# pangenome/impg

Hardware: AMD Instinct MI355X
Metric: projected ranges/sec, 1M-PAF 100k-BED -x depth 3; CPU coitrees baseline (higher is better)
Workload: dtype int32

## Files before the change

### impg_amd/csrc/capi.cpp

```cpp
#include <sys/stat.h>
#include <unistd.h>

#include <atomic>
#include <cerrno>
#include <functional>
#include <thread>
#include <chrono>
#include <cmath>
#include <cstdlib>
#include <memory>
#include <new>

#include "engine.hpp"
#include "partition.hpp"

namespace impg {
thread_local std::string g_error;
void set_error(const std::string &msg) { g_error = msg; }
void render_paf(const impg_gpu_results &res, const impg_gpu_index &ix, const char *const *range_names,
                const impg_gpu_params_t &p, int32_t merge_distance, bool bedpe, std::vector<std::string> &parts);
void render_bed(const impg_gpu_results &res, const impg_gpu_index &ix, const char *const *range_names,
                const impg_gpu_params_t &p, int32_t merge_distance, std::vector<std::string> &parts);
char *join_parts(std::vector<std::string> &parts, size_t *len);
}

using namespace impg;


namespace impg {
static void engine_options(impg_gpu_index &ix, Engine *e) {
  e->pair_budget = ix.opt_pair_budget;
  e->chunk_ranges = ix.opt_chunk_ranges;
  e->locality_min = ix.opt_locality_min;
  e->free_slots_allowed = ix.opt_free_slots;
  e->regroup_pairs = ix.opt_regroup;
  e->fuse_allowed = ix.opt_fuse_final;
  e->filter_covered = ix.opt_filter_covered;
  e->walk_allowed = ix.opt_walk != 0 && !getenv("IMPG_NO_WALK");
  e->walk_bfs = ix.opt_walk == 2;
  e->walk_members = ix.opt_walk_members;
  e->seg_group = ix.opt_seg_group;
  e->seg_parts_force = ix.opt_seg_parts;
  e->seg_stats = ix.seg_stats;
  e->proj_stats = ix.proj_stats;
  e->update_stats = ix.opt_update_stats;
  e->upd_stats = ix.upd_stats;
  e->wide_emit = WideEmit{ix.opt_wide_cap, ix.opt_wide_bins, ix.opt_lookup_stats};
  e->lk_stats = ix.lk_stats;
}
static Engine *take_or_create(impg_gpu_index &ix) {
  Engine *e = nullptr;
  if (!ix.eng_free.empty()) { e = ix.eng_free.back(); ix.eng_free.pop_back(); }
  else if ((int)ix.engines.size() < ix.max_engines) {
    ix.engines.emplace_back(new Engine(ix.device));
    e = ix.engines.back().get();
  } else return nullptr;
  engine_options(ix, e);
  return e;
}
EngineLease::EngineLease(impg_gpu_index &ix_) : ix(ix_) {
  std::unique_lock<std::mutex> lk(ix.eng_m);
  while (!(e = take_or_create(ix))) ix.eng_cv.wait(lk);
}
Engine *try_lease_engine(impg_gpu_index &ix) {
  std::unique_lock<std::mutex> lk(ix.eng_m);
  return take_or_create(ix);
}
void return_engine(impg_gpu_index &ix, Engine *e) {
  e->remote = nullptr;
  e->masked = false;
  e->subset_on = false;
  std::lock_guard<std::mutex> lk(ix.eng_m);
  ix.eng_free.push_back(e);
  ix.eng_cv.notify_one();
}
EngineLease::~EngineLease() { return_engine(ix, e); }
}

namespace impg {

void require_device(int device) {
  int n = 0;
  hipError_t e = hipGetDeviceCount(&n);
  if (e != hipSuccess || n <= 0)
    throw Error{IMPG_E_HIP, "no HIP device available (libimpg_gpu has no CPU fallback)"};
  if (device < 0 || device >= n) throw Error{IMPG_E_INVALID, "device ordinal out of range"};
}

std::unique_ptr<impg_gpu_index> make_index(const impg_gpu_record_t *records, size_t n_records, const uint32_t *ops,
                                           size_t n_ops, const int64_t *seq_len, uint32_t n_seq, int bidirectional,
                                           int order_policy, int device, uint32_t shard, uint32_t n_shards,
                                           const HostSeqIndex *seq, const std::vector<uint64_t> *file_first,
                                           const uint32_t *owner) {
  if ((!records && n_records) || (!ops && n_ops) || (!seq_len && n_seq)) throw Error{IMPG_E_INVALID, "null input array"};
  require_device(device);
  auto ix = std::make_unique<impg_gpu_index>();
  ix->device = device;
  if (seq) ix->seq = *seq;
  if (file_first) {
    if (file_first->size() < 2 || file_first->front() != 0 || file_first->back() != n_records ||
        !std::is_sorted(file_first->begin(), file_first->end()))
      throw Error{IMPG_E_INVALID, "file boundaries must start at 0, end at n_records and be ascending"};
    ix->file_first = *file_first;
  }
  build_index(*ix, records, n_records, ops, n_ops, seq_len, n_seq, bidirectional != 0, order_policy, shard, n_shards, owner);
  { EngineLease warm(*ix); }
  return ix;
}

}

namespace impg {
void assemble_results(Engine &E, const impg_gpu_range_t *h_ranges, uint32_t n, const impg_gpu_params_t &p,
                      std::vector<std::unique_ptr<LevelBufs>> &levels, DevBuf &self_dev, impg_gpu_results &res, uint64_t max_rows,
                      hipEvent_t kernels_done, const std::function<void()> &on_kernels_done) {
  hipStream_t s = E.stream;
  res.ranges.assign(h_ranges, h_ranges + n);
  res.has_cigar = p.store_cigar != 0;
  RowPlan pl;
  plan_rows(E, n, p, levels, self_dev, false, pl);
  const size_t nr = pl.n_rows;
  if (nr > max_rows && n > 1) throw SplitBatch{};
  DevBuf rows, clen, coff, cpool;
  for (DevBuf *b : {&rows, &clen, &coff, &cpool}) b->pool = &E.level_pool;
  rows.reserve(std::max<size_t>(nr * sizeof(impg_gpu_interval_t), 256));
  if (res.has_cigar) clen.reserve(std::max<size_t>(nr * 4, 256));
  scatter_rows(E, levels, pl, RowSinks{rows.as<impg_gpu_interval_t>(), nullptr, nullptr, nullptr, nullptr,
                                       res.has_cigar ? clen.as<uint32_t>() : nullptr});
  if (max_rows != ~0ull && nr * sizeof(impg_gpu_interval_t) > res.intervals.cap)
    res.intervals.reserve(std::max<size_t>(nr, (size_t)std::min<uint64_t>(max_rows, nr + nr / 4)), true);
  res.intervals.resize(nr, true);
  std::vector<uint32_t> off32((size_t)n + 1);
  IMPG_HIP(hipMemcpyAsync(off32.data(), pl.offsets.p, ((size_t)n + 1) * 4, hipMemcpyDeviceToHost, s));
  if (kernels_done && !res.has_cigar) IMPG_HIP(hipEventRecord(kernels_done, s));
  if (nr) IMPG_HIP(hipMemcpyAsync(res.intervals.data(), rows.p, nr * sizeof(impg_gpu_interval_t), hipMemcpyDeviceToHost, s));
  if (res.has_cigar) {
    const uint64_t n_ops = build_row_cigars(E, levels, pl, clen, coff, cpool);
    res.cigar_off.resize(nr + 1, true);
    res.cigar_ops.resize(n_ops, true);
    if (kernels_done) IMPG_HIP(hipEventRecord(kernels_done, s));
    IMPG_HIP(hipMemcpyAsync(res.cigar_off.data(), coff.p, (nr + 1) * 8, hipMemcpyDeviceToHost, s));
    if (n_ops) IMPG_HIP(hipMemcpyAsync(res.cigar_ops.data(), cpool.p, n_ops * 4, hipMemcpyDeviceToHost, s));
  }
  if (kernels_done) { IMPG_HIP(hipEventSynchronize(kernels_done)); if (on_kernels_done) on_kernels_done(); }
  IMPG_HIP(hipStreamSynchronize(s));
  levels.clear();
  res.offsets.resize((size_t)n + 1);
  for (size_t q = 0; q <= n; q++) res.offsets[q] = off32[q];
  res.projected = E.last_projected;
}

const impg_gpu_range_t *upload_ranges(DevBuf &dst, const impg_gpu_range_t *ranges, size_t n, const hipStream_t *async_on) {
  dst.reserve(std::max<size_t>(n * sizeof(impg_gpu_range_t), 256));
  if (n && async_on) IMPG_HIP(hipMemcpyAsync(dst.p, ranges, n * sizeof(impg_gpu_range_t), hipMemcpyHostToDevice, *async_on));
  else if (n) IMPG_HIP(hipMemcpy(dst.p, ranges, n * sizeof(impg_gpu_range_t), hipMemcpyHostToDevice));
  return dst.as<impg_gpu_range_t>();
}

StatSinks::StatSinks(DevBuf &cnt, DevBuf &ck, bool want_count, bool want_cksum, size_t n, const hipStream_t *async_on) {
  auto zeroed = [&](DevBuf &b) {
    b.reserve(std::max<size_t>(n * 8, 256));
    if (async_on) IMPG_HIP(hipMemsetAsync(b.p, 0, n * 8, *async_on));
    else IMPG_HIP(hipMemset(b.p, 0, std::max<size_t>(n * 8, 8)));
    return b.as<unsigned long long>();
  };
  if (want_count) count = zeroed(cnt);
  if (want_cksum) cksum = zeroed(ck);
}
void StatSinks::home(uint64_t *per_range_count, uint64_t *per_range_checksum, size_t n) const {
  if (per_range_count && n) IMPG_HIP(hipMemcpy(per_range_count, count, n * 8, hipMemcpyDeviceToHost));
  if (per_range_checksum && n) IMPG_HIP(hipMemcpy(per_range_checksum, cksum, n * 8, hipMemcpyDeviceToHost));
}

bool run_chunk_rows(const impg_gpu_index &ix, Engine &E, const impg_gpu_range_t *d_ranges, const impg_gpu_range_t *h_ranges, size_t b,
                    size_t e, const impg_gpu_params_t &p, impg_gpu_results &part, std::mutex *gpu_turn, uint64_t max_rows,
                    hipEvent_t kernels_done, const std::function<void()> &on_kernels_done) {
  std::vector<std::unique_ptr<LevelBufs>> levels;
  DevBuf self_dev;
  self_dev.pool = &E.level_pool;
  const auto c0 = std::chrono::steady_clock::now();
  {
    const auto turn = take_turn(gpu_turn);
    RunSpec rs(d_ranges + b, (uint32_t)(e - b), p);
    rs.keep = &levels;
    rs.self_out = &self_dev;
    E.run(ix, rs);
  }
  const auto c1 = std::chrono::steady_clock::now();
  if (e == b) return false;
  assemble_results(E, h_ranges + b, (uint32_t)(e - b), p, levels, self_dev, part, max_rows, kernels_done, on_kernels_done);
  part.approximate = ix.tp_mode;
  part.run_s = std::chrono::duration<double>(c1 - c0).count();
  part.assemble_s = std::chrono::duration<double>(std::chrono::steady_clock::now() - c1).count();
  return true;
}

bool run_chunk_bed(const impg_gpu_index &ix, Engine &E, const impg_gpu_range_t *d_ranges, const impg_gpu_range_t *h_ranges,
                   const char *const *range_names, size_t b, size_t e, const impg_gpu_params_t &p, int32_t merge_distance,
                   const std::function<void(const char *, size_t)> &sink, double *seconds3, std::mutex *gpu_turn) {
  std::vector<std::unique_ptr<LevelBufs>> levels;
  DevBuf self_dev, rows;
// ... 276 lines not shown
      struct stat st;
      if (stat(p.c_str(), &st) == 0) bytes += (uint64_t)st.st_size * ((p.size() > 3 && p.compare(p.size() - 3, 3, ".gz") == 0) ? 6 : 1);
    }
    size_t free_b = 0, total_b = 0;
    IMPG_HIP(hipSetDevice(device));
    IMPG_HIP(hipMemGetInfo(&free_b, &total_b));
    if (bytes * 8 > free_b) raw = false;
  }
  parse_paf_files(ps, pp, raw);
  lap(raw ? "parse PAF (lines, fields)" : "parse PAF", t0);
  std::vector<int64_t> lens = pp.seq.lens;
  if (raw) {
    const auto t1 = std::chrono::steady_clock::now();
    DevBuf d_ops;
    const uint64_t n_ops = tokenize_on_device(pp, device, d_ops);
    lap("CIGAR text -> ops (device)", t1);
    auto ix = std::make_unique<impg_gpu_index>();
    ix->device = device;
    ix->seq = pp.seq;
    if (pp.file_first.size() < 2 || pp.file_first.front() != 0 || pp.file_first.back() != pp.records.size())
      throw Error{IMPG_E_INVALID, "internal: bad file boundaries"};
    ix->file_first = pp.file_first;
    if (order_policy != IMPG_ORDER_COITREES && order_policy != IMPG_ORDER_SORTED) throw Error{IMPG_E_INVALID, "bad order policy"};
    if (build_index_device(*ix, pp.records.data(), pp.records.size(), nullptr, n_ops, lens.data(), (uint32_t)lens.size(), bidirectional != 0,
                           order_policy, 0, 1, nullptr, d_ops.as<uint32_t>())) {
      { EngineLease warm(*ix); }
      *out = ix.release();
      return IMPG_OK;
    }
    pp.ops.resize(n_ops);
    if (n_ops) IMPG_HIP(hipMemcpy(pp.ops.data(), d_ops.p, n_ops * 4, hipMemcpyDeviceToHost));
  }
  *out = make_index(pp.records.data(), pp.records.size(), pp.ops.data(), pp.ops.size(), lens.data(), (uint32_t)lens.size(),
                    bidirectional, order_policy, device, 0, 1, &pp.seq, &pp.file_first, nullptr).release();
  return IMPG_OK;
  IMPG_CATCH
}

int impg_gpu_parse_subsequence(const char *seq_name, char *base_out, size_t base_cap, int32_t *start_offset) {
  IMPG_TRY
  if (!seq_name || !base_out || !start_offset) throw Error{IMPG_E_INVALID, "null argument"};
  size_t base_len = 0;
  uint32_t off = 0;
  const std::string name(seq_name);
  if (!subsequence_origin(name, base_len, off)) return 0;
  if (base_len + 1 > base_cap) throw Error{IMPG_E_INVALID, "name buffer too small"};
  memcpy(base_out, name.data(), base_len);
  base_out[base_len] = '\0';
  *start_offset = (int32_t)off;
  return 1;
  IMPG_CATCH
}

int impg_gpu_subset_keep(const char *list_text, size_t len, const char *const *names, size_t n, uint8_t *keep_out,
                         size_t *n_entries) {
  IMPG_TRY
  if ((!list_text && len) || (n && (!names || !keep_out))) throw Error{IMPG_E_INVALID, "null argument"};
  const size_t e = subset_select(list_text, len, names, n, keep_out);
  if (n_entries) *n_entries = e;
  return IMPG_OK;
  IMPG_CATCH
}

int impg_gpu_index_save(const impg_gpu_index_t *ix, const char *path) {
  IMPG_TRY
  if (!ix || !path) throw Error{IMPG_E_INVALID, "null argument"};
  if (ix->shard || ix->cluster) save_sharded(*ix, path);
  else save_index(*ix, path);
  return IMPG_OK;
  IMPG_CATCH
}

int impg_gpu_index_load(const char *path, int device, impg_gpu_index_t **out) {
  IMPG_TRY
  if (!path || !out) throw Error{IMPG_E_INVALID, "null argument"};
  require_device(device);
  auto ix = std::make_unique<impg_gpu_index>();
  ix->device = device;
  load_index(*ix, path);
  { EngineLease warm(*ix); }
  *out = ix.release();
  return IMPG_OK;
  IMPG_CATCH
}

void impg_gpu_index_destroy(impg_gpu_index_t *ix) { delete ix; }

uint32_t impg_gpu_num_seqs(const impg_gpu_index_t *ix) { return (uint32_t)ix->seq.lens.size(); }
const char *impg_gpu_seq_name(const impg_gpu_index_t *ix, uint32_t id) {
  return id < ix->seq.names.size() ? ix->seq.names[id].c_str() : nullptr;
}
int64_t impg_gpu_seq_len(const impg_gpu_index_t *ix, uint32_t id) { return id < ix->seq.lens.size() ? ix->seq.lens[id] : -1; }
int64_t impg_gpu_seq_id(const impg_gpu_index_t *ix, const char *name) {
  auto it = ix->seq.name_to_id.find(name);
  return it == ix->seq.name_to_id.end() ? -1 : (int64_t)it->second;
}
size_t impg_gpu_num_targets(const impg_gpu_index_t *ix) { return ix->n_targets; }
size_t impg_gpu_target_ids(const impg_gpu_index_t *ix, uint32_t *out, size_t cap) {
  size_t k = 0;
  for (uint32_t s = 0; s + 1 < ix->h_tgt_off.size(); s++)
    if (ix->h_tgt_off[s + 1] != ix->h_tgt_off[s]) {
      if (out && k < cap) out[k] = s;
      k++;
    }
  return k;
}
size_t impg_gpu_num_entries(const impg_gpu_index_t *ix) { return ix->n_entries; }
size_t impg_gpu_num_records(const impg_gpu_index_t *ix) { return ix->n_records; }
size_t impg_gpu_device_bytes(const impg_gpu_index_t *ix) { return ix->device_bytes; }
int impg_gpu_index_approximate(const impg_gpu_index_t *ix) {
  return ix->tp_mode ? 1 : 0;
}

uint64_t impg_gpu_host_pool_trim(uint64_t keep_bytes) { return (uint64_t)impg::pinned_trim((size_t)keep_bytes); }

int impg_gpu_set_option(impg_gpu_index_t *ix, const char *key, int64_t value) {
  IMPG_TRY
  if (!ix || !key) throw Error{IMPG_E_INVALID, "null argument"};
  std::string k(key);
  if (k == "pair_budget") {
    if (value < 1024 || value >= 0xFFFFFFF0ll) throw Error{IMPG_E_INVALID, "pair_budget out of range"};
    ix->opt_pair_budget = (uint64_t)value;
  } else if (k == "chunk_ranges") {
    if (value < 0 || value >= (1ll << 31)) throw Error{IMPG_E_INVALID, "chunk_ranges out of range"};
    ix->opt_chunk_ranges = (uint32_t)value;
  } else if (k == "locality_min") {
    if (value < 0 || value >= (1ll << 31)) throw Error{IMPG_E_INVALID, "locality_min out of range"};
    ix->opt_locality_min = (uint32_t)value;
  } else if (k == "device_rows_pool_bytes") {
    if (value < 0) throw Error{IMPG_E_INVALID, "device_rows_pool_bytes must not be negative"};
    ix->opt_device_rows_pool = (uint64_t)value;
  } else if (k == "fuse_final_level") {
    ix->opt_fuse_final = value != 0;
  } else if (k == "regroup_entries") {
    ix->opt_regroup = value != 0;
  } else if (k == "walk_kernel") {
    if (value < 0 || value > 2) throw Error{IMPG_E_INVALID, "walk_kernel is 0, 1 or 2"};
    ix->opt_walk = (int)value;
  } else if (k == "segment_groups") {
    ix->opt_seg_group = value != 0;
  } else if (k == "segment_parts") {
    if (value < 0 || value > 4096) throw Error{IMPG_E_INVALID, "segment_parts is 0 .. 4096"};
    ix->opt_seg_parts = (uint32_t)value;
  } else if (k == "walk_members") {
    if (value < 0 || value > (long long)WALK_MAX_MEMBERS) throw Error{IMPG_E_INVALID, "walk_members is 0 .. 64"};
    ix->opt_walk_members = (uint32_t)value;
  } else if (k == "filter_covered") {
    if (value < 0 || value > 2) throw Error{IMPG_E_INVALID, "filter_covered is 0, 1 or 2"};
    ix->opt_filter_covered = (int)value;
  } else if (k == "update_stats") {
    ix->opt_update_stats = value != 0;
  } else if (k == "lookup_stats") {
    ix->opt_lookup_stats = value != 0;
  } else if (k == "wide_emit_cap") {
    if (value < 64 || value > (long long)WIDE_CAP) throw Error{IMPG_E_INVALID, "wide_emit_cap is 64 .. 4096"};
    ix->opt_wide_cap = (uint32_t)value;
  } else if (k == "wide_emit_bins") {
    if (value < 2 || value > (long long)WIDE_BINS) throw Error{IMPG_E_INVALID, "wide_emit_bins is 2 .. 1024"};
    ix->opt_wide_bins = (uint32_t)value;
  } else if (k == "approximate_cigar") {
    if (value != 0 && value != 1) throw Error{IMPG_E_INVALID, "approximate_cigar is 0 or 1"};
    ix->opt_approx_cigar = value != 0;
  } else if (k == "free_slot_order") {
    ix->opt_free_slots = value != 0;
  } else if (k == "debug_fail_owner" || k == "debug_fail_home") {
    if (value < 0 || value > 0xFFFFFFFFll) throw Error{IMPG_E_INVALID, "debug_fail_* out of range"};
    (k == "debug_fail_owner" ? ix->opt_debug_fail_owner : ix->opt_debug_fail_home) = (uint32_t)value;
  } else if (k == "lane_schedule") {
    if (value < 0) throw Error{IMPG_E_INVALID, "lane_schedule out of range"};
    ix->opt_lane_schedule = (uint64_t)value;
  } else if (k == "prewarm_result_bytes") {
    if (value < 0) throw Error{IMPG_E_INVALID, "prewarm_result_bytes is a size"};
    if (value) {
      size_t cap = 0;
      void *b = pinned_take((size_t)value, cap);
      pinned_give(b, cap);
    }
  } else if (k == "prewarm_walk") {
    if (value < 0 || value > 2) throw Error{IMPG_E_INVALID, "prewarm_walk is 0, 1 or 2"};
    if (value && !ix->shard && !ix->cluster) {
      IMPG_HIP(hipSetDevice(ix->device));
      EngineLease lease(*ix);
      lease->reserve_walk_slabs(*ix, value >= 2);
    }
  } else throw Error{IMPG_E_INVALID, "unknown option " + k};
  return IMPG_OK;
  IMPG_CATCH
}

int impg_gpu_get_counter(const impg_gpu_index_t *ix, const char *key, int64_t *value_out) {
  IMPG_TRY
  if (!ix || !key || !value_out) throw Error{IMPG_E_INVALID, "null argument"};
  const std::string k = key;
  if (k == "walk_launches") *value_out = (int64_t)ix->walk_launches.load();
  else if (k == "walk_fallbacks") *value_out = (int64_t)ix->walk_fallbacks.load();
  else if (k == "walk_members") *value_out = (int64_t)ix->walk_last_members.load();
  else if (k == "small_batches") *value_out = (int64_t)ix->small_batches.load();
  else if (k == "segment_sliced_levels") *value_out = (int64_t)ix->seg_stats[0].load();
  else if (k == "segment_retries") *value_out = (int64_t)ix->seg_stats[1].load();
  else if (k == "segment_library_levels") *value_out = (int64_t)ix->seg_stats[2].load();
  else if (k == "project_lane_levels") *value_out = (int64_t)ix->proj_stats[PROJ_ARM_LANE].load();
  else if (k == "project_staged_levels") *value_out = (int64_t)ix->proj_stats[PROJ_ARM_STAGED].load();
  else if (k == "project_staged_rows_levels") *value_out = (int64_t)ix->proj_stats[PROJ_ARM_STAGED_ROWS].load();
  else if (k == "project_entries_slots_levels") *value_out = (int64_t)ix->proj_stats[PROJ_ARM_ENTRIES_SLOTS].load();
  else if (k == "project_entries_qs_levels") *value_out = (int64_t)ix->proj_stats[PROJ_ARM_ENTRIES_QS].load();
  else if (k == "project_entries_rows_levels") *value_out = (int64_t)ix->proj_stats[PROJ_ARM_ENTRIES_ROWS].load();
  else if (k == "project_entries_ident_levels") *value_out = (int64_t)ix->proj_stats[PROJ_ARM_ENTRIES_IDENT].load();
  else if (k == "project_tp_levels") *value_out = (int64_t)ix->proj_stats[PROJ_ARM_TP].load();
  else if (k == "update_lane_groups") *value_out = (int64_t)ix->upd_stats[UPD_LANE].load();
  else if (k == "update_mid_groups") *value_out = (int64_t)ix->upd_stats[UPD_MID].load();
  else if (k == "update_wave_tiny_groups") *value_out = (int64_t)ix->upd_stats[UPD_WAVE_TINY].load();
  else if (k == "update_wave_small_groups") *value_out = (int64_t)ix->upd_stats[UPD_WAVE_SMALL].load();
  else if (k == "update_wave_large_groups") *value_out = (int64_t)ix->upd_stats[UPD_WAVE_LARGE].load();
  else if (k == "update_inplace_groups") *value_out = (int64_t)ix->upd_stats[UPD_INPLACE].load();
  else if (k == "update_tiled_sort_groups") *value_out = (int64_t)ix->upd_stats[UPD_TILED_SORT].load();
  else if (k == "update_lane_spill_groups") *value_out = (int64_t)ix->upd_stats[UPD_LANE_SPILL].load();
  else if (k == "lookup_wide_windows") *value_out = (int64_t)ix->lk_stats[LK_WIDE].load();
  else if (k == "lookup_wide_single") *value_out = (int64_t)ix->lk_stats[LK_SINGLE].load();
  else if (k == "lookup_wide_grouped") *value_out = (int64_t)ix->lk_stats[LK_GROUPED].load();
  else if (k == "lookup_wide_group_passes") *value_out = (int64_t)ix->lk_stats[LK_GROUP_PASSES].load();
  else if (k == "lookup_wide_overflow") *value_out = (int64_t)ix->lk_stats[LK_OVERFLOW].load();
  else throw Error{IMPG_E_INVALID, "unknown counter " + k};
  return IMPG_OK;
  IMPG_CATCH
}

int impg_gpu_visit_rank(uint32_t n, int order_policy, uint32_t *rank_out) {
  IMPG_TRY
  if (!rank_out && n) throw Error{IMPG_E_INVALID, "null argument"};
  if (order_policy == IMPG_ORDER_COITREES) coitrees_visit_rank(n, rank_out);
  else if (order_policy == IMPG_ORDER_SORTED) for (uint32_t i = 0; i < n; i++) rank_out[i] = i;
  else throw Error{IMPG_E_INVALID, "bad order policy"};
  return IMPG_OK;
  IMPG_CATCH
}

}
namespace impg {
void apply_mask(Engine &E, const impg_gpu_index &ix, const impg_gpu_mask_t *m, const impg_gpu_params_t &p) {
  if (!m) return;
  if (!p.transitive) throw Error{IMPG_E_INVALID, "masked_regions belong to the transitive queries"};
  const uint32_t n_seq = ix.view.n_seq;
  if (m->n_seqs && (!m->seq_id || !m->sequence_length || !m->range_off)) throw Error{IMPG_E_INVALID, "null mask array"};
  const uint64_t total = m->n_seqs ? m->range_off[m->n_seqs] : 0;
  if (total >= 0xFFFFFFF0ull) throw Error{IMPG_E_UNSUPPORTED, "mask exceeds 2^32 ranges"};
  if (total && !m->ranges) throw Error{IMPG_E_INVALID, "null mask array"};
  std::vector<uint32_t> off(n_seq + 1, 0);
  std::vector<int32_t> init_len(n_seq, 0), touch_len(n_seq, 0);
  bool has_empty = false;
  if (p.multi_impg) for (uint32_t s = 0; s < n_seq; s++) touch_len[s] = (int32_t)std::min<int64_t>(std::max<int64_t>(ix.seq.lens[s], 0), INT32_MAX);
  for (uint32_t i = 0; i < m->n_seqs; i++) {
    const uint32_t s = m->seq_id[i];
    if (s >= n_seq) throw Error{IMPG_E_INVALID, "mask names an unknown sequence id"};
    if (i && s <= m->seq_id[i - 1]) throw Error{IMPG_E_INVALID, "mask sequence ids must be strictly ascending"};
    if (m->range_off[i + 1] < m->range_off[i]) throw Error{IMPG_E_INVALID, "mask offsets must not decrease"};
    off[s + 1] = (uint32_t)(m->range_off[i + 1] - m->range_off[i]);
    init_len[s] = touch_len[s] = m->sequence_length[i];
    for (uint64_t k = m->range_off[i]; k < m->range_off[i + 1]; k++) {
      const int32_t a = m->ranges[2 * k], b = m->ranges[2 * k + 1];
      if (a > b || (k > m->range_off[i] && a <= m->ranges[2 * k - 1]))
        throw Error{IMPG_E_INVALID, "mask ranges must be sorted, disjoint and non-touching"};
      has_empty = has_empty || a == b;
    }
  }
  for (uint32_t s = 0; s < n_seq; s++) off[s + 1] += off[s];
  E.mask_off.reserve((size_t)(n_seq + 1) * 4);
  E.mask_ranges.reserve(std::max<size_t>(total * 8, 256));
  E.mask_init_len.reserve(std::max<size_t>((size_t)n_seq * 4, 256));
  E.mask_touch_len.reserve(std::max<size_t>((size_t)n_seq * 4, 256));
  IMPG_HIP(hipMemcpy(E.mask_off.p, off.data(), (size_t)(n_seq + 1) * 4, hipMemcpyHostToDevice));
  ix.mask_table_uploads++;
  if (total) { IMPG_HIP(hipMemcpy(E.mask_ranges.p, m->ranges, total * 8, hipMemcpyHostToDevice)); ix.mask_table_uploads++; }
  if (n_seq) {
    IMPG_HIP(hipMemcpy(E.mask_init_len.p, init_len.data(), (size_t)n_seq * 4, hipMemcpyHostToDevice));
    IMPG_HIP(hipMemcpy(E.mask_touch_len.p, touch_len.data(), (size_t)n_seq * 4, hipMemcpyHostToDevice));
    ix.mask_table_uploads += 2;
  }
  E.masked = true;
  E.mask_has_empty = has_empty;
  E.mask_ranges_total = total;
  E.mask_lists = m->n_seqs;
}
void apply_subset(Engine &E, const impg_gpu_index &ix, const uint8_t *subset_keep) {
  if (!subset_keep) return;
  const size_t ns = ix.view.n_seq;
  E.subset_keep.reserve(std::max<size_t>(ns, 256));
  if (ns) IMPG_HIP(hipMemcpy(E.subset_keep.p, subset_keep, ns, hipMemcpyHostToDevice));
  E.subset_on = true;
}
}
extern "C" {

int impg_gpu_query_batch(impg_gpu_index_t *ix, const impg_gpu_range_t *ranges, size_t n, const impg_gpu_params_t *params,
                         impg_gpu_results_t **out) {
  return impg_gpu_query_batch_masked(ix, ranges, n, params, nullptr, out);
}

int impg_gpu_query_batch_masked(impg_gpu_index_t *ix, const impg_gpu_range_t *ranges, size_t n,
                                const impg_gpu_params_t *params, const impg_gpu_mask_t *mask, impg_gpu_results_t **out) {
  return impg_gpu_query_batch_filtered(ix, ranges, n, params, mask, nullptr, out);
}

int impg_gpu_query_batch_filtered(impg_gpu_index_t *ix, const impg_gpu_range_t *ranges, size_t n,
                                  const impg_gpu_params_t *params, const impg_gpu_mask_t *mask, const uint8_t *subset_keep,
                                  impg_gpu_results_t **out) {
  IMPG_TRY
  if (!ix || !params || !out || (!ranges && n)) throw Error{IMPG_E_INVALID, "null argument"};
  check_ranges(ranges, n);
  Engine::check_params(*params);
  if (ix->shard || ix->cluster) return sharded_query_batch(*ix, ranges, n, *params, mask, subset_keep, out);
  IMPG_HIP(hipSetDevice(ix->device));
  EngineLease lease(*ix);
  Engine &E = *lease;
  apply_mask(E, *ix, mask, *params);
  apply_subset(E, *ix, subset_keep);
  auto res = std::make_unique<impg_gpu_results>();
  res->approximate = ix->tp_mode;
  if (n && n <= Engine::SMALL_RANGES && !params->transitive) {
    const auto c0 = std::chrono::steady_clock::now();
    if (E.run_small(*ix, ranges, (uint32_t)n, *params, *res)) {
      res->run_s = std::chrono::duration<double>(std::chrono::steady_clock::now() - c0).count();
      *out = res.release();
      return IMPG_OK;
    }
  }
  const impg_gpu_range_t *d_ranges = upload_ranges(E.ranges_dev, ranges, n, &E.stream);
  if (n < (1ull << 31) && E.walk_applicable(*ix, (uint32_t)n, *params)) {
    const auto c0 = std::chrono::steady_clock::now();
    if (walk_query(*ix, E, (uint32_t)n, *params, *res)) {
      res->run_s = std::chrono::duration<double>(std::chrono::steady_clock::now() - c0).count();
      res->ranges.assign(ranges, ranges + n);
      *out = res.release();
      return IMPG_OK;
    }
    res = std::make_unique<impg_gpu_results>();
  }
  res->offsets.assign(1, 0);
  for_chunks(E, n, [&](size_t b, size_t e) {
    impg_gpu_results part;
    run_chunk_rows(*ix, E, d_ranges, ranges, b, e, *params, part);
    ix->result_rows_to_host += part.intervals.size();
    append_results(*res, part);
  });
  res->ranges.assign(ranges, ranges + n);
  *out = res.release();
  return IMPG_OK;
  IMPG_CATCH
}

int impg_gpu_query(impg_gpu_index_t *ix, uint32_t target_id, int32_t start, int32_t end, const impg_gpu_params_t *params,
                   impg_gpu_results_t **out) {
  impg_gpu_range_t r{target_id, start, end};
  return impg_gpu_query_batch(ix, &r, 1, params, out);
}

int impg_gpu_query_batch_stream(impg_gpu_index_t *ix, const impg_gpu_range_t *ranges, size_t n, const impg_gpu_params_t *params,
                                const impg_gpu_mask_t *mask, const uint8_t *subset_keep, size_t chunk_ranges, size_t max_block_bytes,
                                impg_gpu_stream_cb cb, void *ctx, uint64_t *projected_out) {
  IMPG_TRY
  if (!ix) throw Error{IMPG_E_INVALID, "null argument"};
  const bool collective = ix->shard && !ix->cluster;
  std::exception_ptr refused;
  try {
    if (!params || !cb || (!ranges && n)) throw Error{IMPG_E_INVALID, "null argument"};
    check_ranges(ranges, n);
    Engine::check_params(*params);
  } catch (...) {
    if (!collective) throw;
    refused = std::current_exception();
// ... 538 lines not shown
```

### impg_amd/csrc/engine.cpp

```cpp
#include <cmath>
#include <cstdio>
#include <cstdlib>
#include <memory>

#include "engine.hpp"

namespace impg {

namespace {
inline unsigned bits_for(uint64_t n) {
  unsigned b = 0;
  while ((1ull << b) < n) b++;
  return b;
}
}

Engine::Engine(int device) {
  IMPG_HIP(hipSetDevice(device));
  IMPG_HIP(hipStreamCreateWithFlags(&stream, hipStreamNonBlocking));
  for (DevBuf *b : {&ord_offsets, &ord_rows}) b->pool = &level_pool;
  win_se.pool = &level_pool;
  counters.reserve(128);
  acc_slots.reserve(COUNT_BYTES);
  act_slots.reserve(COUNT_BYTES);
// ... 255 lines not shown
  for (uint32_t k = 0; k < COUNT_SLOTS; k++) t += h_slots[k * COUNT_STRIDE];
  return t;
}

uint64_t Engine::scan(const uint32_t *in, uint32_t *out, uint32_t n) {
  if (n == 0) return 0;
  scan_tmp.reserve(scan_scratch_bytes(n));
  launch_exclusive_scan(in, out, n, scan_tmp.as<unsigned long long>(), counters.as<unsigned long long>() + 3, stream);
  IMPG_HIP(hipMemcpyAsync(h_counters, counters.as<uint64_t>() + 3, 24, hipMemcpyDeviceToHost, stream));
  IMPG_HIP(hipStreamSynchronize(stream));
  if (h_counters[2]) throw Error{IMPG_E_INVALID, "query range must satisfy start < end"};
  return h_counters[0];
}

void Engine::scan2(const uint32_t *in_a, uint32_t *out_a, const uint32_t *in_b, uint32_t *out_b, uint32_t n, uint64_t &total_a, uint64_t &total_b,
                   const uint32_t *d_extra, uint32_t *h_extra, uint32_t n_extra) {
  total_a = total_b = 0;
  if (n) {
    scan_tmp.reserve(scan_scratch_bytes(n));
    scan_tmp2.reserve(scan_scratch_bytes(n));
    launch_exclusive_scan(in_a, out_a, n, scan_tmp.as<unsigned long long>(), counters.as<unsigned long long>() + 14, stream);
    launch_exclusive_scan(in_b, out_b, n, scan_tmp2.as<unsigned long long>(), counters.as<unsigned long long>() + 15, stream);
    IMPG_HIP(hipMemcpyAsync(h_counters, counters.as<uint64_t>() + 14, 16, hipMemcpyDeviceToHost, stream));
  }
  if (n_extra) IMPG_HIP(hipMemcpyAsync(h_counters + 2, d_extra, (size_t)n_extra * 4, hipMemcpyDeviceToHost, stream));
  IMPG_HIP(hipStreamSynchronize(stream));
  if (n) { total_a = h_counters[0]; total_b = h_counters[1]; }
  if (n_extra) memcpy(h_extra, h_counters + 2, (size_t)n_extra * 4);
}

static HitArrays hit_arrays(LevelBufs &L, uint32_t n_pairs) {
  size_t b = std::max<size_t>((size_t)n_pairs * 4, 256);
  L.qid.reserve(L.qs_interleaved ? 2 * b : b); L.coords.reserve(4 * b);
  return HitArrays{L.qid.as<uint32_t>(), L.coords.as<int4>()};
}

const uint32_t *Engine::lookup_order(const DeviceIndexView &v, const FrontierRec *fr, uint32_t n_fr, const RecordBlocks *blocks) {
  if (!locality_min || (n_fr < locality_min && !blocks)) { keys_for = nullptr; return nullptr; }
  const size_t nb = (size_t)n_fr * 4;
  lo_key.reserve(nb); lo_key2.reserve(nb); lo_idx.reserve(nb); lo_perm.reserve(nb);
  unsigned hi_bit = std::max(1u, bits_for((uint32_t)std::min<size_t>(v.n_entries, 0xFFFFFFFFull)));
  unsigned block_shift = 0;
  if (blocks) {
    const unsigned bb = std::max(1u, bits_for(blocks->n_blocks));
    if (hi_bit + bb > 32) return nullptr;
    block_shift = hi_bit;
    hi_bit += bb;
  }
  if (!blocks && keys_for && keys_for == (const void *)fr && keys_n == n_fr) {
  } else
    launch_order_keys(v, fr, n_fr, lo_key.as<uint32_t>(), lo_idx.as<uint32_t>(), stream, blocks ? blocks->d_bounds : nullptr,
                      blocks ? blocks->n_blocks : 0u, block_shift);
  keys_for = nullptr;
  static const bool lib_sort = getenv("IMPG_LIB_SORT") && atoi(getenv("IMPG_LIB_SORT")) != 0;
  if (lib_sort) {
    const size_t tb = sort_u32_scratch_bytes(n_fr);
    sort_tmp.reserve(tb);
    launch_sort_u32(sort_tmp.p, tb, lo_key.as<uint32_t>(), lo_key2.as<uint32_t>(), lo_idx.as<uint32_t>(), lo_perm.as<uint32_t>(), n_fr,
                    stream, 0, hi_bit);
  } else {
    sort_tmp.reserve(order_sort_scratch_bytes(n_fr));
    launch_order_sort(lo_key.as<uint32_t>(), lo_key2.as<uint32_t>(), lo_perm.as<uint32_t>(), lo_idx.as<uint32_t>(), n_fr, hi_bit, sort_tmp.p, stream);
  }
  return lo_perm.as<uint32_t>();
}
void Engine::projection_offsets(const uint32_t *d_perm, uint32_t n_fr, const uint32_t *d_cnt, uint64_t P, const uint32_t *&d_offp,
                                ProjList &pl) {
  d_offp = nullptr;
  pl = ProjList{nullptr, nullptr, nullptr};
  if (!d_perm || !P) return;
  const size_t nb = (size_t)n_fr * 4;
  lo_cnt.reserve(nb); lo_off.reserve(nb); lo_offp.reserve(nb);
  const size_t pb = std::max<size_t>(P * 4, 256);
  slot_of.reserve(pb); proj_range.reserve(pb); proj_entry.reserve(pb);
  launch_gather_u32(d_cnt, d_perm, n_fr, lo_cnt.as<uint32_t>(), stream);
  scan(lo_cnt.as<uint32_t>(), lo_off.as<uint32_t>(), n_fr);
  launch_scatter_u32(lo_off.as<uint32_t>(), d_perm, n_fr, lo_offp.as<uint32_t>(), stream);
  pl = ProjList{slot_of.as<uint32_t>(), proj_range.as<uint32_t>(), proj_entry.as<uint32_t>()};
  d_offp = lo_offp.as<uint32_t>();
}

void Engine::count_wide_paths(const DeviceIndexView &v, uint32_t n) {
  if (!(wide_emit.count_reach && lk_stats) || !n || !emit_by_lanes(v)) return;
  uint32_t w[LK_WORDS];
  IMPG_HIP(hipMemcpyAsync(w, wide_n.p, sizeof w, hipMemcpyDeviceToHost, stream));
  IMPG_HIP(hipStreamSynchronize(stream));
  const uint32_t *reach = w + LK_REACH_BASE;
  lk_stats[LK_WIDE] += w[0];
  lk_stats[LK_OVERFLOW] += w[1];
  lk_stats[LK_SINGLE] += reach[LK_REACH_SINGLE];
  lk_stats[LK_GROUPED] += reach[LK_REACH_GROUPED];
  lk_stats[LK_GROUP_PASSES] += reach[LK_REACH_PASSES];
}

uint64_t Engine::expand(const DeviceIndexView &v, const FrontierRec *fr, uint32_t n_fr, bool transitive, LevelBufs &L,
                        impg_gpu_stats_t *st, bool raw, const RecordBlocks *blocks) {
  hipEvent_t e0 = event(), e1 = event(), e2 = event();
  IMPG_HIP(hipEventRecord(e0, stream));
  cnt.reserve((size_t)n_fr * 4);
  win.reserve((size_t)n_fr * 16);
  pair_off.reserve((size_t)n_fr * 4);
  if (multi) transitive = false;
  wide_n.reserve(256);
  wide_list.reserve(std::max<size_t>((size_t)n_fr * 8, 256));
  const uint32_t *d_perm = lookup_order(v, fr, n_fr, blocks);
  const bool by_place = free_slot_order && (!raw || blocks) && !multi && !store_cigar && d_perm;
  last_by_place = by_place;
  last_range_places = false;
  L.qs_interleaved = false;
  L.placed = false;
  expand_n_fr = n_fr;
  bool fused = by_place && fuse_final && emit_by_lanes(v) && !v.tp_mode;
  const bool lk = wide_emit.count_reach && lk_stats;
  const WideEmit we{wide_emit.cap, wide_emit.bins, lk};
  if (by_place) win_se.reserve(std::max<size_t>((size_t)n_fr * sizeof(FrontierRec), 256));
  const bool ordered = run_modes.ordered_rows && !raw;
  if (ordered) { L.slot_ref.reserve(std::max<size_t>((size_t)n_fr * 4, 256)); ord_cnt.reserve(std::max<size_t>((size_t)n_fr * 4, 256)); }
  launch_lookup_count(v, fr, n_fr, transitive, d_perm, cnt.as<uint32_t>(), win.as<uint4>(), wide_n.as<uint32_t>(),
                      wide_list.as<uint32_t>(), stream, by_place, by_place ? win_se.as<FrontierRec>() : nullptr,
                      ordered && by_place ? ord_cnt.as<uint32_t>() : nullptr, lk);
  uint64_t P = scan(cnt.as<uint32_t>(), pair_off.as<uint32_t>(), n_fr);
  if (P > pair_budget || P >= 0xFFFFFFF0ull) {
    if (split_ok) throw SplitBatch{};
    if (P >= 0xFFFFFFF0ull) throw Error{IMPG_E_UNSUPPORTED, "more than 2^32 candidate pairs for a single range"};
  }
  L.n_pairs = (uint32_t)P;
  L.n_frontier = n_fr;
  bool direct = false;
  if (ordered) {
    ordered_level(fr, n_fr, L, !by_place, P);
    direct = fused && !store_cigar && !(min_identity == min_identity) && project_entry_major(v, P, min_identity);
    if (!direct) fused = false;
  }
  L.pair_range.reserve(std::max<size_t>(P * 4, 256));
  pair_entry.reserve(std::max<size_t>(P * 4, 256));
  ProjList pl{nullptr, nullptr, nullptr};
  WindowLists wlists{nullptr, nullptr, nullptr, nullptr, nullptr, 0u, nullptr, 0u, 0u};
  if (fused) {
    const bool staged = project_is_staged(v, P, !store_cigar && !(min_identity == min_identity));
    tile_first.reserve(((size_t)(P + 255) / 256 + 1) * 4);
    if (!staged) launch_tile_first(cnt.as<uint32_t>(), pair_off.as<uint32_t>(), n_fr, tile_first.as<uint32_t>(), stream);
    launch_lookup_emit(v, fr, n_fr, transitive, pair_off.as<uint32_t>(), win.as<uint4>(), L.pair_range.as<uint32_t>(),
                       pair_entry.as<uint32_t>(), d_perm, nullptr, pl, wide_n.as<uint32_t>(), wide_list.as<uint32_t>(), stream, true, true, we);
    wlists = WindowLists{tile_first.as<uint32_t>(), pair_off.as<uint32_t>(), win.as<uint4>(), win_se.as<FrontierRec>(), d_perm, n_fr,
                         fuse_need_ranges && !direct ? L.pair_range.as<uint32_t>() : nullptr, 1u, fuse_range_places ? 1u : 0u};
    last_range_places = fuse_need_ranges && fuse_range_places && !direct;
    if (project_entry_major(v, P, min_identity) && !store_cigar) {
      const uint32_t cap = project_entry_slice_cap(P), nb = project_entry_blocks(n_fr);
      ent_work.reserve(((size_t)cap + 1) * 4);
      ent_alloc.reserve(std::max<size_t>((size_t)nb * 4, 256));
      IMPG_HIP(hipMemsetAsync(ent_work.p, 0, 4, stream));
      IMPG_HIP(hipMemsetAsync(ent_alloc.p, 0, (size_t)nb * 4, stream));
      wlists.slice_work = ent_work.as<uint32_t>(); wlists.slice_alloc = ent_alloc.as<uint32_t>(); wlists.slice_cap = cap;
    }
    L.qs_interleaved = last_range_places && project_entry_major(v, P, min_identity) && !(min_identity == min_identity) && !store_cigar && !getenv("IMPG_NO_QS");
    if (L.qs_interleaved) { wlists.masks |= 4u; wlists.range_out = nullptr; }
    if (direct) {
      ordered_offsets();
      ord_dest.reserve(std::max<size_t>((size_t)n_fr * 4, 256));
      ord_vpos.reserve(std::max<size_t>(P + 256, 256));
      const bool by_visit = ordered_rows_by_visit();
      const OrdDestArgs od{win_se.as<FrontierRec>(), d_perm, L.slot_ref.as<uint32_t>(), ord_offsets.as<uint32_t>(), L.lvbase.as<uint32_t>(), ord_dest.as<uint32_t>()};
      launch_emit_vpos(v, n_fr, pair_off.as<uint32_t>(), win.as<uint4>(), ord_vpos.as<uint8_t>(), stream, by_visit, &od);
      wlists.ord = OrderedOut{ord_rows.as<impg_gpu_interval_t>(), ord_dest.as<uint32_t>(), ord_vpos.as<uint8_t>(), ord_min_len, by_visit ? 1u : 0u};
      L.placed = true;
    }
  } else if (by_place) {
    launch_lookup_emit(v, fr, n_fr, transitive, pair_off.as<uint32_t>(), win.as<uint4>(), L.pair_range.as<uint32_t>(),
                       pair_entry.as<uint32_t>(), d_perm, nullptr, pl, wide_n.as<uint32_t>(), wide_list.as<uint32_t>(), stream, true, false, we);
    wlists = WindowLists{nullptr, pair_off.as<uint32_t>(), win.as<uint4>(), win_se.as<FrontierRec>(), d_perm, n_fr, nullptr, 0u, 0u};
  } else {
    const uint32_t *d_offp = nullptr;
    projection_offsets(d_perm, n_fr, cnt.as<uint32_t>(), P, d_offp, pl);
    const bool entry_slots = store_cigar || multi || !pl.slot;
    launch_lookup_emit(v, fr, n_fr, transitive, pair_off.as<uint32_t>(), win.as<uint4>(), L.pair_range.as<uint32_t>(),
                       entry_slots ? pair_entry.as<uint32_t>() : nullptr, pl.slot ? d_perm : nullptr, d_offp, pl,
                       wide_n.as<uint32_t>(), wide_list.as<uint32_t>(), stream, false, false, we);
  }
  count_wide_paths(v, n_fr);
  IMPG_HIP(hipEventRecord(e1, stream));
  HitArrays h = direct ? HitArrays{nullptr, nullptr} : hit_arrays(L, L.n_pairs);
  SliceArrays sl{nullptr, nullptr, nullptr, nullptr};
  if (store_cigar) {
    size_t b = std::max<size_t>((size_t)L.n_pairs * 4, 256);
    L.sl_a.reserve(b); L.sl_n.reserve(b); L.sl_off.reserve(b); L.sl_rem.reserve(b);
    sl = SliceArrays{L.sl_a.as<uint32_t>(), L.sl_n.as<uint32_t>(), L.sl_off.as<int32_t>(), L.sl_rem.as<int32_t>()};
  }
  count_arm(launch_project(v, fr, L.pair_range.as<uint32_t>(), pair_entry.as<uint32_t>(), L.n_pairs, transitive, h,
                           acc_slots.as<unsigned long long>(), (uint32_t *)(counters.as<uint64_t>() + 2), min_identity,
                           store_cigar ? &sl : nullptr, pl, stream, nullptr, regroup_pairs, by_place ? &wlists : nullptr));
  if (!raw && !direct) {
    post_expand(fr, n_fr, L, pair_off.as<uint32_t>(), pair_entry.as<uint32_t>(), v.mrank, sl);
    h = HitArrays{L.qid.as<uint32_t>(), L.coords.as<int4>()};
    if (store_cigar) sl = SliceArrays{L.sl_a.as<uint32_t>(), L.sl_n.as<uint32_t>(), L.sl_off.as<int32_t>(), L.sl_rem.as<int32_t>()};
  }
  IMPG_HIP(hipEventRecord(e2, stream));
  if (store_cigar && L.n_pairs) {
    cnt.reserve((size_t)L.n_pairs * 4);
    L.slice_pos.reserve((size_t)L.n_pairs * 4);
    launch_slice_counts(h, sl, L.n_pairs, cnt.as<uint32_t>(), stream);
    L.slice_total = scan(cnt.as<uint32_t>(), L.slice_pos.as<uint32_t>(), L.n_pairs);
    if (L.slice_total >= 0xFFFFFFF0ull) {
      if (split_ok) throw SplitBatch{};
      throw Error{IMPG_E_UNSUPPORTED, "CIGAR slices of one level exceed 2^32 ops"};
    }
    L.slice_pool.reserve(std::max<size_t>(L.slice_total * 4, 256));
    launch_slice_write(v, pair_entry.as<uint32_t>(), h, sl, L.n_pairs, L.slice_pos.as<uint32_t>(), L.slice_pool.as<uint32_t>(), stream);
  } else {
    L.slice_total = 0;
  }
  timed.push_back({e0, e1, 0});
  timed.push_back({e1, e2, 1});
  if (st) {
    st->pairs += P;
    st->frontier_ranges += n_fr;
    if (P) st->project_launches += 1;
  }
  return P;
}

void Engine::post_expand(const FrontierRec *fr, uint32_t n_fr, LevelBufs &L, const uint32_t *d_pair_off, uint32_t *tie_idx,
                         const uint32_t *tie_rank, SliceArrays sl) {
  HitArrays h{L.qid.as<uint32_t>(), L.coords.as<int4>()};
  if (subset_on)
    launch_subset_filter(fr, L.pair_range.as<uint32_t>(), L.n_pairs, h.qid, subset_keep.as<uint8_t>(), cur_ranges, stream);
  if (multi && L.n_pairs) {
    const size_t b = std::max<size_t>((size_t)L.n_pairs * 4, 256);
    m_dest.reserve(b); m_qid.reserve(b); m_coords.reserve(4 * b); m_pe.reserve(b);
    launch_sort5(fr, n_fr, d_pair_off, L.n_pairs, h, tie_idx, tie_rank, m_dest.as<uint32_t>(), stream);
    HitArrays h2{m_qid.as<uint32_t>(), m_coords.as<int4>()};
    SliceArrays sl2{nullptr, nullptr, nullptr, nullptr};
    if (sl.a) {
      m_sa.reserve(b); m_sn.reserve(b); m_so.reserve(b); m_sr.reserve(b);
      sl2 = SliceArrays{m_sa.as<uint32_t>(), m_sn.as<uint32_t>(), m_so.as<int32_t>(), m_sr.as<int32_t>()};
    }
    launch_permute_slots(m_dest.as<uint32_t>(), L.n_pairs, h, h2, tie_idx, m_pe.as<uint32_t>(), sl, sl2, stream);
    L.qid.swap(m_qid); L.coords.swap(m_coords);
    if (tie_idx == pair_entry.as<uint32_t>()) pair_entry.swap(m_pe);
    if (sl.a) { L.sl_a.swap(m_sa); L.sl_n.swap(m_sn); L.sl_off.swap(m_so); L.sl_rem.swap(m_sr); }
  }
}

void Engine::ordered_level(const FrontierRec *fr, uint32_t n_fr, LevelBufs &L, bool counts_by_range, uint64_t P) {
  const uint64_t total = scan(counts_by_range ? cnt.as<uint32_t>() : ord_cnt.as<uint32_t>(), L.slot_ref.as<uint32_t>(), n_fr);
  if (total != P) throw Error{IMPG_E_INVALID, "internal: a level's slot counts disagree between its two orders"};
  L.lvbase.reserve(std::max<size_t>((size_t)ord_n * 4, 256));
  launch_ord_level_bases(fr, n_fr, L.slot_ref.as<uint32_t>(), (uint32_t)P, ord_n, ord_acc.as<uint32_t>(), L.lvbase.as<uint32_t>(), stream);
}
void Engine::ordered_offsets() {
  if (ord_offsets_done) return;
  ord_offsets.reserve(((size_t)ord_n + 1) * 4);
  ord_total = scan(ord_acc.as<uint32_t>(), ord_offsets.as<uint32_t>(), ord_n + 1u);
  if (ord_total >= 0xFFFFFFF0ull) { if (split_ok) throw SplitBatch{}; throw Error{IMPG_E_UNSUPPORTED, "more than 2^32 result rows in one chunk: use smaller chunks (chunk_ranges)"}; }
  ord_rows.reserve(std::max<size_t>(ord_total * sizeof(impg_gpu_interval_t), 256));
  ord_offsets_done = true;
}
void Engine::ordered_finish(std::vector<std::unique_ptr<LevelBufs>> &levels) {
  hipEvent_t p0 = event(), p1 = event();
  IMPG_HIP(hipEventRecord(p0, stream));
  ordered_offsets();
  launch_ord_self_rows(ord_self, ord_ranges, ord_n, ord_offsets.as<uint32_t>(), ord_rows.as<impg_gpu_interval_t>(), stream);
  for (auto &Lp : levels) {
    LevelBufs &L = *Lp;
    if (L.placed || !L.n_pairs) continue;
    L.run_start.reserve(std::max<size_t>((size_t)L.n_frontier * 4, 256));
    launch_ord_run_heads(L.pair_range.as<uint32_t>(), L.n_pairs, L.run_start.as<uint32_t>(), stream);
    HitArrays h{L.qid.as<uint32_t>(), L.coords.as<int4>()};
    launch_ord_level_rows(L.frontier.as<FrontierRec>(), L.pair_range.as<uint32_t>(), L.n_pairs, h, L.run_start.as<uint32_t>(), L.slot_ref.as<uint32_t>(),
                          ord_offsets.as<uint32_t>(), L.lvbase.as<uint32_t>(), ord_min_len, ord_rows.as<impg_gpu_interval_t>(), stream);
    L.placed = true;
  }
  IMPG_HIP(hipEventRecord(p1, stream));
  IMPG_HIP(hipStreamSynchronize(stream));
  float ms = 0;
  IMPG_HIP(hipEventElapsedTime(&ms, p0, p1));
  ms_place = ms;
}

HopResult Engine::hop(const DeviceIndexView &v, const FrontierRec *fr, uint32_t n_fr, bool transitive, LevelBufs &L,
                      impg_gpu_stats_t *st, bool need_hits, bool need_rows, bool alive) {
  if (remote) return remote->hop(*this, v, fr, n_fr, transitive, L, st, need_hits, need_rows, alive);
  if (!alive) { L.n_pairs = 0; return HopResult{0, true}; }
  if (!n_fr) { L.n_pairs = 0; return HopResult{0, false}; }
  return HopResult{expand(v, fr, n_fr, transitive, L, st), false};
}

uint32_t Engine::update(const DeviceIndexView &v, const FrontierRec *fr, LevelBufs &L, uint32_t n_queries,
                        const impg_gpu_params_t &p, DevBuf &next_frontier) {
  hipEvent_t e0 = event(), e1 = event();
  IMPG_HIP(hipEventRecord(e0, stream));
  const uint32_t P = L.n_pairs;
  uint32_t n_next = 0;
  HitArrays h{L.qid.as<uint32_t>(), L.coords.as<int4>()};
  if (P) {
    const uint32_t P_slots = P;
    const bool want_flags = filter_covered != 0;
    svals.reserve((size_t)P * 8);
    uint32_t seg_active = 0, seg_groups = 0;
    uint32_t *sg_run_start = nullptr, *sg_run_end = nullptr, *sg_q = nullptr, *sg_bins = nullptr;
    uint32_t seg_parts = seg_group && !want_flags && !multi && seg_group_fits(v.n_seq) && L.n_frontier > 0 ? seg_group_parts(P, n_queries, v.n_seq) : 0u;
    if (seg_parts_force && seg_parts) {
      seg_parts = std::max(1u, std::min(seg_parts_force, 4096u));
      while (seg_parts > 1 && ((uint64_t)n_queries * seg_parts >= (1ull << 31) || seg_group_bins_bytes(n_queries, v.n_seq, seg_parts) > (1ull << 30))) seg_parts >>= 1;
    }
    bool by_segments = seg_parts != 0;
    if (by_segments) {
      const uint32_t n_fr = L.n_frontier;
      seg_run.reserve(std::max<size_t>((size_t)n_fr * 8, 256));
      seg_q.reserve(std::max<size_t>((size_t)n_queries * 24 + 256, 512));
      sg_run_start = seg_run.as<uint32_t>(); sg_run_end = sg_run_start + n_fr;
      sg_q = seg_q.as<uint32_t>();
      uint32_t *qfirst = sg_q, *qlast = qfirst + n_queries, *qact = qlast + n_queries, *qdst = qact + n_queries, *qgrp = qdst + n_queries,
               *gdst = qgrp + n_queries, *unsorted = gdst + n_queries;
      const bool own_offsets = !remote && !store_cigar && L.n_frontier == expand_n_fr;
      launch_seg_bounds(fr, n_fr, n_queries, L.pair_range.as<uint32_t>(), P, sg_run_start, sg_run_end, qfirst, qlast, unsorted, stream,
                        own_offsets && last_by_place ? lo_perm.as<uint32_t>() : nullptr, own_offsets ? pair_off.as<uint32_t>() : nullptr,
                        own_offsets ? cnt.as<uint32_t>() : nullptr);
      for (int attempt = 0; attempt < 2 && by_segments; attempt++) {
        const size_t bb = seg_group_bins_bytes(n_queries, v.n_seq, seg_parts);
        sg_bins = nullptr;
        if (seg_parts > 1 || bb <= (512ull << 20)) { seg_bins.reserve(std::max<size_t>(bb, 256)); sg_bins = seg_bins.as<uint32_t>(); }
        if (seg_parts > 1) seg_tot.reserve(std::max<size_t>(seg_group_bins_bytes(n_queries, v.n_seq, 1), 256));
        launch_seg_group(true, fr, qfirst, qlast, sg_run_start, sg_run_end, h, n_queries, v.n_seq, qact, qdst, qgrp, gdst, nullptr, nullptr, nullptr, sg_bins,
                         stream, seg_parts, seg_tot.as<uint32_t>());
        uint64_t ta = 0, tg = 0;
        uint32_t bad[2] = {0, 0};
        scan2(qact, qdst, qgrp, gdst, n_queries, ta, tg, unsorted, bad, 2);
        seg_active = (uint32_t)ta;
        if (bad[0]) by_segments = false;
        else if (bad[1]) {
          const uint32_t again = seg_parts == 1 && attempt == 0 ? seg_group_parts(P, n_queries, v.n_seq, bad[1]) : 0u;
          if (again > 1) { seg_parts = again; IMPG_HIP(hipMemsetAsync(unsorted, 0, 8, stream)); if (seg_stats) seg_stats[1]++; }
          else by_segments = false;
        } else { seg_groups = (uint32_t)tg; break; }
      }
      if (by_segments && seg_parts > 1 && seg_stats) seg_stats[0]++;
    }
    if (!by_segments) {
      if (seg_stats) seg_stats[2]++;
      keys.reserve((size_t)P * 8); skeys.reserve((size_t)P * 8); vals.reserve((size_t)P * 8);
      IMPG_HIP(hipMemsetAsync(act_slots.p, 0, COUNT_BYTES, stream));
      launch_update_keys(fr, L.pair_range.as<uint32_t>(), P, h, keys.as<unsigned long long>(), vals.as<unsigned long long>(),
                         act_slots.as<unsigned long long>(), stream);
// ... 546 lines not shown
```

### impg_amd/csrc/engine.hpp

```cpp
#pragma once
#include <atomic>
#include <functional>
#include <memory>
#include <string>
#include <vector>

#include "kernels.hpp"

namespace impg {

struct LevelBufs {
  DevBuf frontier, pair_range, qid, coords;
  DevBuf sl_a, sl_n, sl_off, sl_rem, slice_pos, slice_pool;
  uint64_t slice_total = 0;
  uint32_t n_frontier = 0, n_pairs = 0;
  DevBuf slot_ref, lvbase, run_start;
  bool qs_interleaved = false;
  bool placed = false;
  LevelBufs() = default;
  explicit LevelBufs(BufPool *pool) {
    for (DevBuf *b : {&frontier, &pair_range, &qid, &coords, &sl_a, &sl_n, &sl_off, &sl_rem, &slice_pos, &slice_pool, &slot_ref, &lvbase, &run_start}) b->pool = pool;
  }
};
struct VisitedStore {
  DevBuf keys, off, len, ranges, qoff;
  uint32_t n_groups = 0;
  explicit VisitedStore(BufPool *pool) { keys.pool = off.pool = len.pool = ranges.pool = qoff.pool = pool; }
};

struct SplitBatch {};

struct HopResult {
  uint64_t pairs;
  bool all_dead;
};
struct Engine;
struct Expander {
  virtual ~Expander() {}
  virtual HopResult hop(Engine &home, const DeviceIndexView &v, const FrontierRec *fr, uint32_t n_fr, bool transitive,
                        LevelBufs &L, impg_gpu_stats_t *st, bool need_hits, bool need_rows, bool alive) = 0;
};

struct RemoteRows {
  std::vector<std::unique_ptr<LevelBufs>> *parts;
  BufPool *pool;
  uint64_t range_base;
  uint32_t level;
};
struct RunModes {
  bool keep_any_order = false;
  bool ordered_rows = false;
  RemoteRows *remote_rows = nullptr;
};
struct RunSpec : RunModes {
  const impg_gpu_range_t *d_ranges;
  uint32_t n;
  const impg_gpu_params_t &p;
  std::vector<std::unique_ptr<LevelBufs>> *keep = nullptr;
  unsigned long long *d_count = nullptr, *d_cksum = nullptr;
  impg_gpu_stats_t *stats = nullptr;
  DevBuf *self_out = nullptr;
  RunSpec(const impg_gpu_range_t *d_ranges_, uint32_t n_, const impg_gpu_params_t &p_) : d_ranges(d_ranges_), n(n_), p(p_) {}
};

struct Engine {
  BufPool table_pool;
  BufPool level_pool;
  hipStream_t stream = nullptr;
  DevBuf counters;
  DevBuf acc_slots, act_slots;
  uint64_t *h_slots = nullptr;
  uint64_t read_slots(DevBuf &b);
  uint64_t *h_counters = nullptr;
  std::vector<hipEvent_t> ev_pool;
  size_t ev_next = 0;
  struct Timed { hipEvent_t a, b; int kind; };
  std::vector<Timed> timed;
  DevBuf big_list;
  DevBuf cnt, win, pair_off, pair_entry, scan_tmp, scan_tmp2, keys, skeys, vals, svals, sort_tmp, head, gid, gstart, glen, old_src,
      cap, pcap, poff, pieces, n_pieces, foff, frontier_a, frontier_b, self_scratch, ranges_dev, stat_count,
      stat_cksum, stage_off;
  LevelBufs level_scratch;
  std::vector<std::unique_ptr<VisitedStore>> tables;
  uint32_t table_queries = 0;
  void index_table(VisitedStore &t);
  uint64_t last_projected = 0;
  uint64_t pair_budget = 1ull << 28;
  uint32_t chunk_ranges = 0;
  bool split_ok = false;
  double min_identity = __builtin_nan("");
  bool store_cigar = false;
  bool multi = false;
  bool free_slot_order = false;
  bool free_slots_allowed = true;
  bool regroup_pairs = true;
  bool fuse_allowed = true;
  bool fuse_final = false, fuse_need_ranges = false, fuse_range_places = false;
  bool last_range_places = false;
  DevBuf ord_acc, ord_offsets, ord_rows, ord_dest, ord_vpos, ord_cnt;
  uint64_t ord_total = 0;
  bool ord_offsets_done = false;
  uint32_t ord_n = 0;
  int32_t ord_min_len = -1;
  const FrontierRec *ord_self = nullptr;
  const impg_gpu_range_t *ord_ranges = nullptr;
  void ordered_level(const FrontierRec *fr, uint32_t n_fr, LevelBufs &L, bool counts_by_range, uint64_t P);
  void ordered_offsets();
  void ordered_finish(std::vector<std::unique_ptr<LevelBufs>> &levels);
  float ms_place = 0;
  DevBuf ent_work, ent_alloc;
  DevBuf win_se, tile_first;
  int filter_covered = 0;
  uint64_t covered_dropped = 0;
  bool update_stats = false;
  DevBuf m_dest, m_qid, m_coords, m_pe, m_sa, m_sn, m_so, m_sr;
  DevBuf wide_n, wide_list;
  WideEmit wide_emit;
  std::atomic<uint64_t> *lk_stats = nullptr;
  void count_wide_paths(const DeviceIndexView &v, uint32_t n);
  DevBuf lo_key, lo_key2, lo_idx, lo_perm, lo_cnt, lo_off, lo_offp, slot_of;
  uint32_t locality_min = 4096;
  const uint32_t *stage_perm = nullptr;
  uint32_t stage_n = 0;

  explicit Engine(int device);
  ~Engine();
  hipEvent_t event();
  uint64_t read_counter(int k);
  uint64_t scan(const uint32_t *in, uint32_t *out, uint32_t n);
  void scan2(const uint32_t *in_a, uint32_t *out_a, const uint32_t *in_b, uint32_t *out_b, uint32_t n, uint64_t &total_a, uint64_t &total_b,
             const uint32_t *d_extra = nullptr, uint32_t *h_extra = nullptr, uint32_t n_extra = 0);
  struct RecordBlocks { const uint32_t *d_bounds; uint32_t n_blocks; };
  const uint32_t *lookup_order(const DeviceIndexView &v, const FrontierRec *fr, uint32_t n_fr, const RecordBlocks *blocks = nullptr);
  void projection_offsets(const uint32_t *d_perm, uint32_t n_fr, const uint32_t *d_cnt, uint64_t P, const uint32_t *&d_offp,
                          ProjList &pl);
  DevBuf proj_range, proj_entry;
  uint64_t expand(const DeviceIndexView &v, const FrontierRec *fr, uint32_t n_fr, bool transitive, LevelBufs &L,
                  impg_gpu_stats_t *st, bool raw = false, const RecordBlocks *blocks = nullptr);
  const void *keys_for = nullptr;
  uint32_t keys_n = 0;
  uint32_t expand_n_fr = 0;
  bool last_by_place = false;
  void post_expand(const FrontierRec *fr, uint32_t n_fr, LevelBufs &L, const uint32_t *d_pair_off, uint32_t *tie_idx,
                   const uint32_t *tie_rank, SliceArrays sl);
  Expander *remote = nullptr;
  const RunModes &modes() const { return run_modes; }
  HopResult hop(const DeviceIndexView &v, const FrontierRec *fr, uint32_t n_fr, bool transitive, LevelBufs &L,
                impg_gpu_stats_t *st, bool need_hits, bool need_rows, bool alive);
  uint32_t update(const DeviceIndexView &v, const FrontierRec *fr, LevelBufs &L, uint32_t n_queries,
                  const impg_gpu_params_t &p, DevBuf &next_frontier);
  VisitedTables tables_view() const;
  void compact_tables();
  DevBuf dk_a, dk_b, ds_a, ds_b, de_a, de_b, dd_a, dd_b, d_flag2, d_pos2, d_popdepth, d_popsel, d_perm, d_perm2, d_k32, d_k32b,
      d_src, d_src2, d_ckey, d_ckey2;
  void run_dfs(const impg_gpu_index &ix, const RunSpec &spec);
  void finish_run(impg_gpu_stats_t *st, hipEvent_t t0, hipEvent_t t1);
  static void check_params(const impg_gpu_params_t &p);
  uint32_t begin_transitive(const DeviceIndexView &v, const impg_gpu_range_t *d_ranges, uint32_t n,
                            const impg_gpu_params_t &p, FrontierRec *d_self, DevBuf &frontier_out);
  DevBuf subset_keep;
  bool subset_on = false;
  const impg_gpu_range_t *cur_ranges = nullptr;
  bool masked = false;
  DevBuf mask_off, mask_ranges, mask_init_len, mask_touch_len;
  bool mask_has_empty = false;
  uint64_t mask_ranges_total = 0, mask_lists = 0;
  DevBuf self_off;
  uint64_t n_self = 0;
  uint32_t begin_transitive_masked(const DeviceIndexView &v, const impg_gpu_range_t *d_ranges, uint32_t n,
                                   const impg_gpu_params_t &p, DevBuf &self, DevBuf &frontier_out);
  float stage_ms[3] = {0, 0, 0};
  uint64_t stage_launches = 0;
  DevBuf stage_next;
  uint32_t stage_next_n = 0, stage_queries = 0;
  void run(const impg_gpu_index &ix, const RunSpec &spec);
  static constexpr uint32_t SMALL_RANGES = 64, SMALL_PAIRS = 1u << 18;
  bool run_small(const impg_gpu_index &ix, const impg_gpu_range_t *h_ranges, uint32_t n, const impg_gpu_params_t &p,
                 impg_gpu_results &res);
  struct WalkRows {
    DevBuf rows, base, cap, n_rows;
    std::vector<uint32_t> h_n_rows;
    std::vector<unsigned long long> h_base;
  };
  bool walk_allowed = true, walk_bfs = false;
  bool walk_applicable(const impg_gpu_index &ix, uint32_t n, const impg_gpu_params_t &p) const;
  static void walk_caps(bool wide, WalkArgs &a);
  static uint64_t walk_workgroups(const impg_gpu_index &ix, bool wide);
  void reserve_walk_slabs(const impg_gpu_index &ix, bool dfs_too);
  bool run_walk(const impg_gpu_index &ix, const impg_gpu_range_t *d_ranges, uint32_t n, const impg_gpu_params_t &p,
                unsigned long long *d_count, unsigned long long *d_cksum, impg_gpu_stats_t *st, WalkRows *rows, uint32_t *h_n_rows = nullptr);
  DevBuf walk_slabs, walk_ctr, walk_ctl;
  DevBuf rstat;
  DevBuf seg_run, seg_q, seg_bins, seg_tot;
  std::atomic<uint64_t> *seg_stats = nullptr;
  std::atomic<uint64_t> *proj_stats = nullptr;
  std::atomic<uint64_t> *upd_stats = nullptr;
  void count_arm(int arm) { if (proj_stats && arm >= 0 && arm < PROJ_ARMS) proj_stats[arm]++; }
  uint32_t seg_parts_force = 0;
  bool seg_group = true;
  uint32_t walk_members = 0;
  uint32_t walk_group_size(const impg_gpu_index &ix, uint32_t n, const impg_gpu_params_t &p) const;
  char *small_in = nullptr;
  char *small_out = nullptr;
  void *small_out_dev = nullptr;
  size_t small_out_cap = 0;

 private:
  RunModes run_modes;
};

void build_index(impg_gpu_index &ix, const impg_gpu_record_t *records, size_t n_records, const uint32_t *cigar_ops,
                 size_t n_ops, const int64_t *seq_len, uint32_t n_seq, bool bidirectional, int order_policy,
                 uint32_t shard, uint32_t n_shards, const uint32_t *owner, const TpInput *tp = nullptr,
                 const EntryPlan *plan = nullptr);

struct EngineLease {
  impg_gpu_index &ix;
  Engine *e = nullptr;
  explicit EngineLease(impg_gpu_index &ix);
  ~EngineLease();
  EngineLease(const EngineLease &) = delete;
  Engine &operator*() { return *e; }
  Engine *operator->() { return e; }
};

#define IMPG_TRY try {
#define IMPG_CATCH                                          \
  }                                                         \
  catch (const impg::Error &e) {                            \
    impg::set_error(e.msg);                                 \
    return e.code;                                          \
  }                                                         \
  catch (const std::bad_alloc &) {                          \
    impg::set_error("host out of memory");                  \
    return IMPG_E_OOM;                                      \
  }                                                         \
  catch (const std::exception &e) {                         \
    impg::set_error(std::string("internal: ") + e.what());  \
    return IMPG_E_INVALID;                                  \
  }
void require_device(int device);
std::unique_ptr<impg_gpu_index> make_index(const impg_gpu_record_t *records, size_t n_records, const uint32_t *ops,
                                           size_t n_ops, const int64_t *seq_len, uint32_t n_seq, int bidirectional,
                                           int order_policy, int device, uint32_t shard, uint32_t n_shards,
                                           const HostSeqIndex *seq, const std::vector<uint64_t> *file_first,
                                           const uint32_t *owner);
void assemble_results(Engine &E, const impg_gpu_range_t *h_ranges, uint32_t n, const impg_gpu_params_t &p,
                      std::vector<std::unique_ptr<LevelBufs>> &levels, DevBuf &self_dev, impg_gpu_results &res,
                      uint64_t max_rows = ~0ull, hipEvent_t kernels_done = nullptr,
                      const std::function<void()> &on_kernels_done = nullptr);
const impg_gpu_range_t *upload_ranges(DevBuf &dst, const impg_gpu_range_t *ranges, size_t n, const hipStream_t *async_on);
inline void add_stats(impg_gpu_stats_t &tot, const impg_gpu_stats_t &st) {
  tot.projected += st.projected; tot.pairs += st.pairs; tot.frontier_ranges += st.frontier_ranges;
  tot.levels = std::max(tot.levels, st.levels);
  tot.ms_total += st.ms_total; tot.ms_lookup += st.ms_lookup; tot.ms_project += st.ms_project; tot.ms_update += st.ms_update;
  tot.project_launches += st.project_launches;
  tot.ms_exchange += st.ms_exchange;
}
struct StatSinks {
  unsigned long long *count = nullptr, *cksum = nullptr;
  StatSinks(DevBuf &cnt, DevBuf &ck, bool want_count, bool want_cksum, size_t n, const hipStream_t *async_on);
  void aim(RunSpec &rs, size_t b) const { rs.d_count = count ? count + b : nullptr; rs.d_cksum = cksum ? cksum + b : nullptr; }
  void home(uint64_t *per_range_count, uint64_t *per_range_checksum, size_t n) const;
};
inline std::unique_lock<std::mutex> take_turn(std::mutex *gpu_turn) {
  return gpu_turn ? std::unique_lock<std::mutex>(*gpu_turn) : std::unique_lock<std::mutex>();
}
bool run_chunk_rows(const impg_gpu_index &ix, Engine &E, const impg_gpu_range_t *d_ranges, const impg_gpu_range_t *h_ranges, size_t b,
                    size_t e, const impg_gpu_params_t &p, impg_gpu_results &part, std::mutex *gpu_turn = nullptr,
                    uint64_t max_rows = ~0ull, hipEvent_t kernels_done = nullptr,
                    const std::function<void()> &on_kernels_done = nullptr);
// ... 67 lines not shown
```

### impg_amd/csrc/impg_internal.hpp

```cpp
#pragma once
#include <atomic>
#include <chrono>
#include <exception>
#include <vector>
#include <hip/hip_runtime.h>

#include <algorithm>
#include <condition_variable>
#include <cstdlib>
#include <new>
#include <cstdint>
#include <cstring>
#include <memory>
#include <mutex>
#include <string>
#include <unordered_map>
#include <vector>

#include "../../include/impg_gpu.h"

namespace impg {

void set_error(const std::string &msg);
inline uint64_t error_clock() {
// ... 170 lines not shown
    const bool pin = want_pinned && bytes >= PINNED_MIN_BYTES;
    if (pin) np = static_cast<T *>(pinned_take(bytes, ncap));
    else {
      ncap = std::max<size_t>(bytes, 64);
      np = static_cast<T *>(malloc(ncap));
      if (!np) throw std::bad_alloc();
    }
    if (n) memcpy(np, p, n * sizeof(T));
    const size_t keep = n;
    release();
    p = np; cap = ncap; pinned = pin; n = keep;
  }
  void resize(size_t count, bool want_pinned = false) { reserve(count, want_pinned); n = count; }
  void push_back(const T &v) {
    if ((n + 1) * sizeof(T) > cap) reserve(std::max<size_t>(2 * n, 16));
    p[n++] = v;
  }
  void assign(const T *b, const T *e) { n = 0; resize((size_t)(e - b)); if (e > b) memcpy(p, b, (size_t)(e - b) * sizeof(T)); }
  void assign(size_t count, const T &v) { n = 0; resize(count); for (size_t i = 0; i < count; i++) p[i] = v; }
  void clear() { n = 0; }
  void swap(HostArr &o) { std::swap(p, o.p); std::swap(n, o.n); std::swap(cap, o.cap); std::swap(pinned, o.pinned); }
  size_t size() const { return n; }
  bool empty() const { return n == 0; }
  T *data() { return p; }
  const T *data() const { return p; }
  T *begin() { return p; }
  T *end() { return p + n; }
  const T *begin() const { return p; }
  const T *end() const { return p + n; }
  T &operator[](size_t i) { return p[i]; }
  const T &operator[](size_t i) const { return p[i]; }
  T &back() { return p[n - 1]; }
};
void parallel_memcpy(void *dst, const void *src, size_t bytes);

struct ParsedPaf {
  HostSeqIndex seq;
  std::vector<impg_gpu_record_t> records;
  std::vector<uint32_t> ops;
  std::vector<uint64_t> file_first;
  bool raw = false;
  struct Text { const char *p; size_t n; uint64_t base; };
  std::vector<Text> texts;
  std::vector<std::shared_ptr<void>> holders;
};
void parse_paf_files(const std::vector<std::string> &paths, ParsedPaf &out, bool raw = false);
void parse_paf_text(const char *text, size_t len, ParsedPaf &out, bool raw = false, uint64_t text_base = 0);
uint64_t tokenize_on_device(ParsedPaf &pp, int device, DevBuf &d_ops);
long parse_cigar(const char *s, size_t n, uint32_t *out, size_t cap);

struct TpInput {
  const impg_gpu_tp_record_t *records;
  const int32_t *tracepoints, *query_deltas, *diffs;
  size_t n_segs_total;
  impg_gpu_tp_mode_t mode;
};

struct EntryPlan {
  std::vector<std::vector<uint64_t>> per_target;
};

bool build_index_device(impg_gpu_index &ix, const impg_gpu_record_t *records, size_t n_records, const uint32_t *cigar_ops, size_t n_ops,
                        const int64_t *seq_len, uint32_t n_seq, bool bidirectional, int order_policy, uint32_t shard, uint32_t n_shards,
                        const uint32_t *owner, const uint32_t *d_cigar_ops = nullptr );
void coitrees_visit_rank(uint32_t n, uint32_t *rank_out);

struct ShardInfo {
  uint32_t world = 0, rank = 0;
  std::vector<uint32_t> owner;
  bool front = false;
};
void save_index(const impg_gpu_index &ix, const char *path, const ShardInfo *shard = nullptr, bool front = false);
void load_index(impg_gpu_index &ix, const char *path, ShardInfo *shard = nullptr);
void save_sharded(const impg_gpu_index &ix, const char *path);

size_t subset_select(const char *text, size_t len, const char *const *names, size_t n, uint8_t *keep);

inline bool subsequence_origin(const std::string &name, size_t &base_len, uint32_t &offset) {
  const size_t colon = name.rfind(':');
  if (colon == std::string::npos) return false;
  const size_t dash = name.find('-', colon + 1);
  if (dash == std::string::npos) return false;
  size_t i = colon + 1;
  if (i < dash && name[i] == '+') i++;
  if (i >= dash) return false;
  uint64_t v = 0;
  for (; i < dash; i++) {
    if (name[i] < '0' || name[i] > '9') return false;
    v = v * 10 + (uint64_t)(name[i] - '0');
    if (v > 2147483647ull) return false;
  }
  base_len = colon;
  offset = (uint32_t)v;
  return true;
}
inline uint32_t put_original_name(std::string &s, const std::string &name, bool original) {
  size_t base_len = 0;
  uint32_t off = 0;
  if (original && subsequence_origin(name, base_len, off)) {
    s.append(name, 0, base_len);
    return off;
  }
  s += name;
  return 0;
}

size_t bed_merge(impg_gpu_interval_t *iv, size_t n, int32_t merge_distance, bool merge_strands);

struct Engine;
struct ShardCtx;
struct Cluster;

}

struct impg_gpu_index {
  int device = 0;
  hipStream_t stream = nullptr;
  impg::HostSeqIndex seq;
  size_t n_records = 0, n_entries = 0, n_tiles = 0, n_targets = 0;
  std::vector<uint32_t> h_tgt_off;
  std::vector<uint64_t> file_first;
  impg::DevBuf d_seg, d_starts, d_ends, d_ends_t, d_pmax, d_starts_lvl, d_pmax_lvl, d_rank, d_mrank, d_entries, d_ops, d_ext_cp, d_idp, d_seq_len, d_pfx;
  impg::DeviceIndexView view{};
  static constexpr int N_BLOBS = 15;
  impg::DevBuf *blob(int k);
  size_t blob_bytes[N_BLOBS] = {};
  bool multi_file = false;
  bool tp_mode = false;
  void bind_view(uint32_t n_seq, uint32_t sorted_order);
  std::atomic<size_t> device_bytes{0};
  std::mutex idl_m;
  void ensure_identity_lines();
  std::atomic<bool> has_identity_lines{false};
  bool lacks_identity_lines() const {
    return !tp_mode && n_tiles && blob_bytes[14] && !has_identity_lines.load(std::memory_order_acquire);
  }
  std::vector<std::unique_ptr<impg::Engine>> engines;
  std::vector<impg::Engine *> eng_free;
  std::mutex eng_m;
  std::condition_variable eng_cv;
  int max_engines = 4;
  uint64_t opt_pair_budget = 1ull << 28;
  uint32_t opt_chunk_ranges = 0, opt_locality_min = 4096;
  uint32_t opt_debug_fail_owner = 0, opt_debug_fail_home = 0;
  uint64_t opt_lane_schedule = 0;
  uint64_t opt_device_rows_pool = 160ull << 30;
  struct RowsPool : impg::BufPool { RowsPool() { shared = true; } } rows_pool;
  bool opt_free_slots = true;
  bool opt_regroup = true;
  bool opt_fuse_final = true;
  int opt_filter_covered = 0;
  bool opt_update_stats = false;
  bool opt_lookup_stats = false;
  bool opt_approx_cigar = false;
  uint32_t opt_wide_cap = 4096, opt_wide_bins = 1024;
  int opt_walk = 1;
  uint32_t opt_walk_members = 0;
  bool opt_seg_group = true;
  uint32_t opt_seg_parts = 0;
  mutable std::atomic<uint64_t> walk_launches{0}, walk_fallbacks{0}, walk_last_members{1};
  mutable std::atomic<uint64_t> small_batches{0};
  mutable std::atomic<uint64_t> mask_table_uploads{0}, result_rows_to_host{0};
  mutable std::atomic<uint64_t> seg_stats[3] = {};
  mutable std::atomic<uint64_t> proj_stats[8] = {};
  mutable std::atomic<uint64_t> upd_stats[8] = {};
  mutable std::atomic<uint64_t> lk_stats[5] = {};
  impg::ShardCtx *shard = nullptr;
  impg::Cluster *cluster = nullptr;
  impg_gpu_index();
  ~impg_gpu_index();
};

struct impg_gpu_results {
  std::vector<uint64_t> offsets;
  impg::HostArr<impg_gpu_interval_t> intervals;
  std::vector<impg_gpu_range_t> ranges;
  bool has_cigar = false;
  bool approximate = false;
  impg::HostArr<uint64_t> cigar_off;
  impg::HostArr<uint32_t> cigar_ops;
  uint64_t projected = 0;
  double run_s = 0, assemble_s = 0;
};
```

### impg_amd/csrc/kernels.hip

```cpp
#include <hip/hip_runtime.h>

#include <cstring>

#include "device_prims.hpp"
#include "impg_internal.hpp"
#include "kernels.hpp"

namespace impg {

__device__ __forceinline__ unsigned lane_id() { return threadIdx.x & 63u; }
__device__ __forceinline__ unsigned long long lanemask_lt() { return (1ull << lane_id()) - 1ull; }

template <int CTRL, int ROW_MASK>
__device__ __forceinline__ uint32_t dpp_or0(uint32_t x) {
  return (uint32_t)__builtin_amdgcn_update_dpp(0, (int)x, CTRL, ROW_MASK, 0xF, false);
}
__device__ __forceinline__ uint32_t wave_incl_scan(uint32_t x) {
  x += dpp_or0<0x111, 0xF>(x);
  x += dpp_or0<0x112, 0xF>(x);
  x += dpp_or0<0x114, 0xF>(x);
  x += dpp_or0<0x118, 0xF>(x);
  x += dpp_or0<0x142, 0xA>(x);
  x += dpp_or0<0x143, 0xC>(x);
  return x;
// ... 1020 lines not shown

template <int MODE>
__device__ __forceinline__ TileScan walk_tiles(const PairCtx &c, uint32_t A, uint32_t B, IdentScan &id) {
  TileScan s;
  s.found = s.any = false;
  s.pqs = s.pts = s.pqe = s.pte = -1;
  ident_reset(id);
  int32_t T, Qn;
  tile_start(c, A, T, Qn);
  const int stepj = c.flip ? -1 : 1;
  for (int64_t j = A;; j += stepj) {
    const uint32_t *tp = c.ops + (size_t)j * TILE_WORDS + 6;
    for (int u = 0; u < (int)TILE_OPS && T <= c.last_tp; u++) {
      const int w = c.flip ? (int)TILE_OPS - 1 - u : u;
      op_step<MODE>(tp[w], c, T, Qn, s, id, (uint32_t)j * TILE_OPS + (uint32_t)w);
    }
    if (T > c.last_tp || j == (int64_t)B) break;
  }
  return s;
}

typedef uint32_t u32x4_u __attribute__((ext_vector_type(4), aligned(4)));
typedef uint32_t u32x2_u __attribute__((ext_vector_type(2), aligned(4)));
struct PfxTile {
  int32_t bT, bQ;
  uint32_t tsh, qsh;
};
__device__ __forceinline__ bool pfx_eval(const PairCtx &c, const PfxTile &t, uint32_t ea, uint32_t eb, bool first_form,
                                         int32_t &oq, int32_t &ot, int32_t &adj) {
  const int32_t xa = (int32_t)__builtin_amdgcn_ubfe(ea, t.tsh, 16u), xb = (int32_t)__builtin_amdgcn_ubfe(eb, t.tsh, 16u);
  const int32_t ya = (int32_t)__builtin_amdgcn_ubfe(ea, t.qsh, 16u), yb = (int32_t)__builtin_amdgcn_ubfe(eb, t.qsh, 16u);
  const int32_t td = xb - xa, qa = yb - ya;
  const int32_t T = c.flip ? t.bT - xb : t.bT + xa;
  const int32_t Qn = c.flip ? t.bQ - yb : t.bQ + ya;
  const bool qzero = qa == 0;
  const int32_t lim = qzero ? c.last_tp : c.R1;
  const int32_t os = max(T, c.R0);
  const int32_t oe = min(T + td, lim);
  const int32_t slack = 1 - min(td, 1);
  const bool pass = (T <= c.last_tp) & (os < oe + slack);
  const int32_t fq = Qn + (qzero ? 0 : os - T);
  const int32_t lq = Qn + (((td == 0) | qzero) ? qa : oe - T);
  oq = first_form ? fq : lq;
  ot = first_form ? os : oe;
  adj = td == 0 ? 0 : first_form ? os - T : oe - (T + td);
  return pass;
}
struct PfxOp { uint32_t j, k; int32_t adj; };
template <bool NEXT, uint32_t LINE_STRIDE = TILE_WORDS>
__device__ __forceinline__ bool pfx_end(const PairCtx &c, const uint32_t *__restrict__ pfx_rec, uint32_t n_ops, uint32_t j,
                                        int32_t thr_abs, bool first_form, int32_t &oq, int32_t &ot, PfxOp &which, uint4 h0) {
  for (bool fresh = true;; fresh = false) {
    const uint32_t *line = pfx_rec + (size_t)j * LINE_STRIDE;
    uint4 h = h0;
    if (!fresh) h = *reinterpret_cast<const uint4 *>(line);
    asm volatile("" : "+v"(h.x), "+v"(h.y), "+v"(h.z), "+v"(h.w));
    const bool wide = (h.x >> 31) != 0u;
    const uint32_t cnt = min(TILE_OPS, n_ops - j * TILE_OPS);
    PfxTile t;
    t.tsh = c.swp ? 16u : 0u;
    t.qsh = 16u - t.tsh;
    const int32_t X0 = (int32_t)(c.swp ? h.y : h.x), Y0 = (int32_t)(c.swp ? h.x : h.y);
    t.bT = c.flip ? c.ts + (int32_t)c.totT - X0 : c.ts + X0;
    t.bQ = c.flip ? (int32_t)c.totQ - Y0 : Y0;
    const int32_t thr = thr_abs - X0;
    uint32_t s = ((int32_t)__builtin_amdgcn_ubfe(h.z, t.tsh, 16u) < thr ? 1u : 0u) + ((int32_t)__builtin_amdgcn_ubfe(h.w, t.tsh, 16u) < thr ? 1u : 0u);
    s = min(s, (cnt - 1u) / PFX_STEP);
    const uint32_t lb = PFX_STEP * s;
    constexpr int D = NEXT ? 0 : 1;
    const uint32_t *q = line + PFX_E0 + lb - (uint32_t)D;
    u32x4_u r0 = *reinterpret_cast<const u32x4_u *>(q), r1 = *reinterpret_cast<const u32x4_u *>(q + 4),
            r2 = *reinterpret_cast<const u32x4_u *>(q + 8);
    asm volatile("" : "+v"(r0), "+v"(r1), "+v"(r2));
    const uint32_t r[12] = {r0.x, r0.y, r0.z, r0.w, r1.x, r1.y, r1.z, r1.w, r2.x, r2.y, r2.z, r2.w};
    const bool b2 = (int32_t)__builtin_amdgcn_ubfe(r[4 + D], t.tsh, 16u) < thr;
    const uint32_t uu[6] = {b2 ? r[4] : r[0], b2 ? r[5] : r[1], b2 ? r[6] : r[2], b2 ? r[7] : r[3], b2 ? r[8] : r[4], b2 ? r[9] : r[5]};
    const bool b1 = (int32_t)__builtin_amdgcn_ubfe(uu[2 + D], t.tsh, 16u) < thr;
    const uint32_t vv[4] = {b1 ? uu[2] : uu[0], b1 ? uu[3] : uu[1], b1 ? uu[4] : uu[2], b1 ? uu[5] : uu[3]};
    const bool b0 = (int32_t)__builtin_amdgcn_ubfe(vv[1 + D], t.tsh, 16u) < thr;
    const bool b3 = (int32_t)__builtin_amdgcn_ubfe(r[8 + D], t.tsh, 16u) < thr;
    uint32_t w0 = b3 ? r[8] : b0 ? vv[1] : vv[0], w1 = b3 ? r[9] : b0 ? vv[2] : vv[1], w2 = b3 ? r[10] : b0 ? vv[3] : vv[2];
    uint32_t k = lb + (b3 ? 8u : (b2 ? 4u : 0u) + (b1 ? 2u : 0u) + (b0 ? 1u : 0u));
    if (wide) return false;
    if (k >= cnt) {
      if (NEXT) return false;
      k = cnt - 1u;
      w0 = line[PFX_E0 + k - 1u]; w1 = line[PFX_E0 + k]; w2 = line[PFX_E0 + k + 1u];
    }
    which.j = j; which.k = k;
    if (pfx_eval(c, t, NEXT ? w0 : w1, NEXT ? w1 : w2, first_form, oq, ot, which.adj)) return true;
    if (NEXT) {
      which.k = k + 1u;
      if (k + 1u < cnt) return pfx_eval(c, t, w1, w2, first_form, oq, ot, which.adj);
      if (j + 1u >= c.m) return false;
      j += 1u;
    } else {
      which.k = k - 1u;
      if (k > 0u) return pfx_eval(c, t, w0, w1, first_form, oq, ot, which.adj);
      if (j == 0u) return false;
      j -= 1u;
    }
  }
}

#ifndef IMPG_PROJ_BLOCK
#define IMPG_PROJ_BLOCK 256
#endif
#ifdef IMPG_PHASE_CLOCKS
__device__ unsigned long long g_phase_clk[16];
#define PHASE_MARK(i) do { asm volatile("s_waitcnt vmcnt(0) lgkmcnt(0)" ::: "memory"); phase_t[i] = __builtin_readcyclecounter(); } while (0)
#define PHASE_MARK_NW(i) do { phase_t[i] = __builtin_readcyclecounter(); } while (0)
#define PHASE_ARG , unsigned long long *phase_t
#define PHASE_PASS , phase_t
#else
#define PHASE_MARK(i) do { } while (0)
#define PHASE_MARK_NW(i) do { } while (0)
#define PHASE_ARG
#define PHASE_PASS
#endif
constexpr uint32_t PROJ_BLOCK = IMPG_PROJ_BLOCK, PROJ_WAVES = PROJ_BLOCK / 64u;
constexpr uint32_t STG_ENT_STRIDE = 20u;
constexpr uint32_t STG_LINE_STRIDE = TILE_WORDS + 4u;
constexpr uint32_t STG_REC_STRIDE = INLINE_TILES * STG_LINE_STRIDE + 4u;
constexpr uint32_t ENT_CP_OFF = INLINE_TILES * STG_LINE_STRIDE;
template <bool TRANSITIVE, int MODE, bool STAGED, int ORIENT>
__device__ __forceinline__ void project_core(const DeviceIndexView &v, uint4 e0, uint4 e1, uint4 e2, uint4 e3, int32_t f_start, int32_t f_end,
                                             uint32_t p, double min_identity, uint32_t *__restrict__ err_flag, const SliceArrays &sl,
                                             unsigned long long *__restrict__ accepted, bool &ok, uint32_t &qid, TileScan &res PHASE_ARG,
                                             const uint32_t *st_pfx);
template <bool TRANSITIVE, int MODE, bool STAGED = false>
__device__ __forceinline__ void project_pair(const DeviceIndexView &v, uint32_t eidx, int32_t f_start, int32_t f_end, uint32_t p,
                                             double min_identity, uint32_t *__restrict__ err_flag, const SliceArrays &sl,
                                             unsigned long long *__restrict__ accepted, bool &ok, uint32_t &qid, TileScan &res PHASE_ARG,
                                             const uint4 *st_entry = nullptr, const uint32_t *st_pfx = nullptr) {
  const uint4 *ep = STAGED ? st_entry : reinterpret_cast<const uint4 *>(v.entries + eidx);
  uint4 e0 = ep[0], e1 = ep[1], e2 = ep[2], e3 = ep[3];
  asm volatile("" : "+v"(e0.x), "+v"(e1.z), "+v"(e2.x), "+v"(e3.x));
  PHASE_MARK(3);
  project_core<TRANSITIVE, MODE, STAGED, -1>(v, e0, e1, e2, e3, f_start, f_end, p, min_identity, err_flag, sl, accepted, ok, qid, res PHASE_PASS, st_pfx);
}
template <bool TRANSITIVE, int MODE, bool STAGED, int ORIENT>
__device__ __forceinline__ void project_core(const DeviceIndexView &v, uint4 e0, uint4 e1, uint4 e2, uint4 e3, int32_t f_start, int32_t f_end,
                                             uint32_t p, double min_identity, uint32_t *__restrict__ err_flag, const SliceArrays &sl,
                                             unsigned long long *__restrict__ accepted, bool &ok, uint32_t &qid, TileScan &res PHASE_ARG,
                                             const uint32_t *st_pfx) {
  constexpr bool IDENT = (MODE & MODE_IDENT) != 0;
  constexpr bool CIGAR = (MODE & MODE_CIGAR) != 0;
  static_assert(!STAGED || MODE == 0 || MODE == MODE_IDENT, "on staged lines: the plain projection, or the one under the identity filter (its identity lines are read from the index)");
  (void)accepted;
  {
    FrontierRec f;
    f.start = f_start; f.end = f_end;
    const int32_t en_ts = (int32_t)e0.x, en_te = (int32_t)e0.y, en_qs = (int32_t)e0.z, en_qe = (int32_t)e0.w;
    const uint32_t nops_flags = e1.z;
    const uint32_t n = nops_flags & OP_LEN_MASK;
    const bool rev = (nops_flags & EF_STRAND) != 0;
    PairCtx c;
    c.swp = ORIENT < 0 ? (nops_flags & EF_REVERSED) != 0 : ORIENT >= 1;
    c.flip = ORIENT < 0 ? c.swp && rev : ORIENT == 2;
    c.zt = c.swp ? 3u : 2u;
    c.zq = c.swp ? 2u : 3u;
    c.ts = en_ts;
    const int32_t qbase = rev ? en_qe : en_qs;
    c.R0 = f.start;
    c.R1 = f.end;
    if (TRANSITIVE) {
      c.R0 = max(c.R0, en_ts);
      c.R1 = min(c.R1, en_te);
    }
    c.last_tp = min(en_te, c.R1);
    c.m = (n + TILE_OPS - 1) / TILE_OPS;
    c.totT = e1.w;
    c.totQ = e2.x;
    if (STAGED && ORIENT >= 0) {
      c.totT = st_pfx[ENT_CP_OFF + 3u];
      c.totQ = st_pfx[ENT_CP_OFF + 4u];
    }
    c.ops = v.ops + (size_t)e1.y * TILE_WORDS;
    if (n == 0) {
      atomicOr(err_flag, 1u);
    } else {
      constexpr bool ON_LINES = !(MODE & (MODE_WALK | MODE_CIGAR));
      const bool start_cov = ON_LINES && c.R0 <= c.ts && c.last_tp > c.ts;
      const bool end_cov = ON_LINES && c.R1 >= en_te && c.R0 < en_te && (int32_t)c.totT == en_te - c.ts;
      const int32_t xa = c.R0 - c.ts, xb = c.last_tp - c.ts;
      const int32_t xbc = ON_LINES ? xb + 1 : xb;
      uint32_t cA = 0, cB = 0;
      if (ORIENT >= 0 || c.m <= INLINE_TILES) {
        uint4 p2 = e2, p3 = e3;
        if (STAGED && ORIENT >= 0) {
          const uint4 *cp = reinterpret_cast<const uint4 *>(__builtin_assume_aligned(st_pfx, 16)) + ENT_CP_OFF / 4u;
          p2 = cp[1];
          p3 = cp[2];
          asm volatile("" : "+v"(p2.x), "+v"(p2.y), "+v"(p2.z), "+v"(p2.w), "+v"(p3.x), "+v"(p3.y), "+v"(p3.z), "+v"(p3.w));
        }
        const int32_t P[8] = {(int32_t)p2.y, (int32_t)p2.z, (int32_t)p2.w, (int32_t)p3.x, (int32_t)p3.y, (int32_t)p3.z, (int32_t)p3.w,
                              c.m == INLINE_TILES ? (int32_t)c.totT : 0x7FFFFFFF};
        cB = 0 < xbc ? 1u : 0u;
#pragma unroll
        for (uint32_t i = 0; i < 8; i++) {
          cA += P[i] < xa ? 1u : 0u;
          cB += P[i] < xbc ? 1u : 0u;
        }
        cB = min(cB, c.m);
      } else {
        const uint32_t *P = v.ext_cp + e2.y;
        uint32_t la = 1, ha = c.m + 1, lb = 0, hb = c.m;
        while (la < ha || lb < hb) {
          const uint32_t wa = ha - la, wb = hb - lb;
          const uint32_t a1 = la + (wa >> 2), a2 = la + (wa >> 1), a3 = la + (wa >> 1) + (wa >> 2);
          const uint32_t b1 = lb + (wb >> 2), b2 = lb + (wb >> 1), b3 = lb + (wb >> 1) + (wb >> 2);
          const bool ga = wa != 0, gb = wb != 0;
          const int32_t pa1 = ga ? (int32_t)P[a1] : 0, pa2 = ga ? (int32_t)P[a2] : 0, pa3 = ga ? (int32_t)P[a3] : 0;
          const int32_t pb1 = gb ? (int32_t)P[b1] : 0, pb2 = gb ? (int32_t)P[b2] : 0, pb3 = gb ? (int32_t)P[b3] : 0;
          if (ga) {
            if (pa1 >= xa) ha = a1; else if (pa2 >= xa) { la = a1 + 1; ha = a2; } else if (pa3 >= xa) { la = a2 + 1; ha = a3; } else la = a3 + 1;
          }
          if (gb) {
            if (pb1 >= xbc) hb = b1; else if (pb2 >= xbc) { lb = b1 + 1; hb = b2; } else if (pb3 >= xbc) { lb = b2 + 1; hb = b3; } else lb = b3 + 1;
          }
        }
        cA = la - 1;
        cB = lb;
      }
      if (cA < c.m) {
        const uint32_t kA = cA, kB = max(cB, 1u) - 1u;
        TileScan sa;
        sa.found = sa.any = false;
        sa.pqs = sa.pts = sa.pqe = sa.pte = -1;
        IdentScan ia, ib;
        ident_reset(ia);
        ident_reset(ib);
        bool walked = false, joined = false, need_walk = false;
        constexpr int PA = MODE == 0 ? PART_FIRST : PART_BOTH, PB = MODE == 0 ? PART_LAST : PART_BOTH;
        uint32_t ipa = 0, ipb = 0;
        int32_t lineM = 0, lineX = 0, lineG = 0;
        if (CIGAR) {
          res = walk_tiles<MODE>(c, orig_tile(c, kA), c.flip ? 0u : c.m - 1u, ia);
          walked = true;
        } else if (!(MODE & MODE_WALK)) {
          const uint32_t *pfx_rec = STAGED ? st_pfx : v.pfx + (size_t)e1.y * TILE_WORDS;
          bool lit = cB == 0u;
          const uint32_t kL = cB ? cB - 1u : 0u;
          int32_t fq = 0, ft = c.ts, lq = (int32_t)c.totQ, lt = en_te;
          const bool do_first = !start_cov, do_last = !end_cov;
          PfxOp lo_op{0u, 0u, 0}, hi_op{c.m - 1u, n - (c.m - 1u) * TILE_OPS - 1u, 0};
          const bool lo_edge = c.flip ? !do_last : !do_first;
          const bool run1 = !lit && (c.flip ? do_last : do_first), run2 = !lit && (c.flip ? do_first : do_last);
          const uint32_t j1 = orig_tile(c, c.flip ? kL : kA), j2 = orig_tile(c, c.flip ? kA : kL);
          uint4 hd1 = make_uint4(0u, 0u, 0u, 0u), hd2 = make_uint4(0u, 0u, 0u, 0u);
          constexpr uint32_t LSTRIDE = STAGED ? STG_LINE_STRIDE : TILE_WORDS;
          if (run1) hd1 = *reinterpret_cast<const uint4 *>(pfx_rec + (size_t)j1 * LSTRIDE);
          if (run2) hd2 = *reinterpret_cast<const uint4 *>(pfx_rec + (size_t)j2 * LSTRIDE);
          asm volatile("" : "+v"(hd1.x), "+v"(hd1.y), "+v"(hd1.z), "+v"(hd1.w), "+v"(hd2.x), "+v"(hd2.y), "+v"(hd2.z), "+v"(hd2.w));
          PHASE_MARK(4);
          if (run1) {
            int32_t oq, ot;
            const bool okc = pfx_end<true, LSTRIDE>(c, pfx_rec, n, j1, c.flip ? (int32_t)c.totT - xb : xa, !c.flip, oq, ot, lo_op, hd1);
            lit = !okc;
            if (c.flip) { lq = oq; lt = ot; } else { fq = oq; ft = ot; }
          }
          PHASE_MARK(5);
          if (run2 && !lit) {
            int32_t oq, ot;
            const bool okc = pfx_end<false, LSTRIDE>(c, pfx_rec, n, j2, (c.flip ? (int32_t)c.totT - xa : xb) + 1, c.flip, oq, ot, hi_op, hd2);
            lit = !okc;
            if (c.flip) { fq = oq; ft = ot; } else { lq = oq; lt = ot; }
          }
          PHASE_MARK(6);
          if (IDENT && !lit && (c.flip ? !do_first : !do_last)) {
            lit = (pfx_rec[(size_t)(c.m - 1u) * LSTRIDE] >> 31) != 0u;
          }
          if (IDENT && !lit) {
            const uint32_t *idl = reinterpret_cast<const uint32_t *>(v.idp) + (size_t)e1.y * IDL_WORDS;
            const uint32_t *la = idl + (size_t)lo_op.j * IDL_WORDS, *lb = idl + (size_t)hi_op.j * IDL_WORDS;
            uint4 ha = make_uint4(0u, 0u, 0u, 0u), hb = *reinterpret_cast<const uint4 *>(lb);
            u32x2_u ea = {0u, 0u}, eb = *reinterpret_cast<const u32x2_u *>(lb + IDL_E0 + hi_op.k);
            if (!lo_edge) {
              ha = *reinterpret_cast<const uint4 *>(la);
              ea = *reinterpret_cast<const u32x2_u *>(la + IDL_E0 + lo_op.k);
            }
            asm volatile("" : "+v"(ha.x), "+v"(hb.x), "+v"(ea), "+v"(eb));
            const int32_t am0 = (int32_t)(ea.x & 0xFFFFu), ax0 = (int32_t)(ea.x >> 16), am1 = (int32_t)(ea.y & 0xFFFFu), ax1 = (int32_t)(ea.y >> 16);
            const int32_t bm0 = (int32_t)(eb.x & 0xFFFFu), bx0 = (int32_t)(eb.x >> 16), bm1 = (int32_t)(eb.y & 0xFFFFu), bx1 = (int32_t)(eb.y >> 16);
            lineM = (int32_t)(hb.x - ha.x) + (bm1 - am0);
            lineX = (int32_t)(hb.y - ha.y) + (bx1 - ax0);
            lineG = (int32_t)(hb.z - ha.z) + (__popc(hb.w & ((2u << hi_op.k) - 1u)) - __popc(ha.w & ((1u << lo_op.k) - 1u)));
            const int32_t lo_adj = c.flip ? lo_op.adj : -lo_op.adj, hi_adj = c.flip ? -hi_op.adj : hi_op.adj;
            lineM += (am1 != am0 ? lo_adj : 0) + (bm1 != bm0 ? hi_adj : 0);
            lineX += (ax1 != ax0 ? lo_adj : 0) + (bx1 != bx0 ? hi_adj : 0);
          }
          if (lit) {
            res = walk_tiles<MODE>(c, orig_tile(c, kA), c.flip ? 0u : c.m - 1u, ia);
            walked = true;
          } else {
            res.found = true;
            res.pqs = fq; res.pts = ft; res.pqe = lq; res.pte = lt;
          }
        } else {
        Cursor cur;
        cur.k = 0xFFFFFFFFu; cur.he = 0; cur.T = 0; cur.Qn = 0;
        if (start_cov) {
          sa.found = true;
          sa.pqs = 0;
          sa.pts = c.ts;
        } else {
          const TileHdr hd = tile_header(c, orig_tile(c, kA));
          const uint32_t nsub = tile_subs(n, orig_tile(c, kA));
          uint32_t he;
          if (!c.flip) {
            const int32_t y = xa - (int32_t)hd.t0;
            he = ((int32_t)hd.bt1 < y ? 1u : 0u) + ((int32_t)hd.bt2 < y ? 1u : 0u) + ((int32_t)hd.bt3 < y ? 1u : 0u);
            he = min(he, nsub - 1u);
          } else {
            const int32_t z = (int32_t)(c.totT - hd.t0) - xa;
            he = ((int32_t)hd.bt3 > z ? 1u : 0u) + ((int32_t)hd.bt2 > z ? 1u : 0u) + ((int32_t)hd.bt1 > z ? 1u : 0u);
            he = max(he, TILE_SUBS - nsub);
          }
          place(c, n, hd, kA, he, cur);
          const uint32_t ipa0 = TILE_SUBS * (e1.y + orig_tile(c, cur.k)) + orig_sub(c, cur.he);
          for (;;) {
            scan_cur<MODE, PA>(c, cur, sa, ia);
            if (sa.found || cur.T > c.last_tp) break;
            if (!advance(c, n, cur)) break;
          }
          ipa = c.flip ? TILE_SUBS * (e1.y + orig_tile(c, cur.k)) + orig_sub(c, cur.he) : ipa0;
        }
        if (sa.found && end_cov) {
          sa.pqe = (int32_t)c.totQ;
          sa.pte = en_te;
        } else if (sa.found) {
          const TileHdr hd = tile_header(c, orig_tile(c, kB));
          const uint32_t nsub = tile_subs(n, orig_tile(c, kB));
          uint32_t he;
          if (!c.flip) {
            const int32_t y = xb - (int32_t)hd.t0;
            he = ((int32_t)hd.bt1 < y ? 1u : 0u) + ((int32_t)hd.bt2 < y ? 1u : 0u) + ((int32_t)hd.bt3 < y ? 1u : 0u);
            he = min(he, nsub - 1u);
          } else {
            const int32_t z = (int32_t)(c.totT - hd.t0) - xb;
            he = ((int32_t)hd.bt3 > z ? 1u : 0u) + ((int32_t)hd.bt2 > z ? 1u : 0u) + ((int32_t)hd.bt1 > z ? 1u : 0u);
            he = max(he, TILE_SUBS - nsub);
          }
          if (hd.wide) he = c.flip ? TILE_SUBS - nsub : 0u;
          joined = !start_cov && (kB < cur.k || (kB == cur.k && he <= cur.he));
          bool go;
          if (joined && MODE == 0) {
            const uint32_t ka = cur.k, ha = cur.he;
            if (ka == kB) place(c, n, hd, ka, ha, cur);
            else place(c, n, tile_header(c, orig_tile(c, ka)), ka, ha, cur);
            go = true;
            sa.any = false;
          } else if (joined) {
            ib = ia;
            go = cur.T <= c.last_tp && advance(c, n, cur);
          } else {
            place(c, n, hd, kB, he, cur);
            ipb = TILE_SUBS * (e1.y + orig_tile(c, cur.k)) + orig_sub(c, cur.he);
            go = true;
            sa.any = false;
          }
          while (go) {
            scan_cur<MODE, PB>(c, cur, sa, ib);
            go = cur.T <= c.last_tp && advance(c, n, cur);
          }
          if (c.flip) ipb = TILE_SUBS * (e1.y + orig_tile(c, cur.k)) + orig_sub(c, cur.he);
          need_walk = (MODE == 0 || !joined) && !sa.any;
        }
        if (need_walk) {
          res = walk_tiles<MODE>(c, orig_tile(c, kA), c.flip ? 0u : c.m - 1u, ia);
          walked = true;
        } else {
          res = sa;
        }
        }
#ifdef IMPG_DEBUG_WALK
        if (walked) atomicAdd(&accepted[(blockIdx.x % COUNT_SLOTS) * COUNT_STRIDE], 1ull << 40);
#endif
        if (CIGAR) {
          sl.a[p] = ia.first_oi;
          sl.n[p] = (ia.first_oi > ia.last_oi ? ia.first_oi - ia.last_oi : ia.last_oi - ia.first_oi) + 1u;
          sl.off[p] = ia.first_off;
          sl.rem[p] = ia.last_rem;
        }
        if (IDENT && res.found) {
          int64_t M, X, G;
          if (!walked && !(MODE & MODE_WALK)) {
            M = lineM; X = lineX; G = lineG;
          } else if (walked || joined) {
            const IdentScan &w = walked ? ia : ib;
            M = (int64_t)w.lm - w.fm; X = (int64_t)w.lx - w.fx; G = (int64_t)w.lg - w.fg;
            M += -(int64_t)w.first_adj_m + w.last_adj_m;
            X += -(int64_t)w.first_adj_x + w.last_adj_x;
          } else {
            const uint4 pa = v.idp[ipa], pb = v.idp[ipb];
            if (!c.flip) {
              M = ((int64_t)pb.x + ib.lm) - ((int64_t)pa.x + ia.fm);
              X = ((int64_t)pb.y + ib.lx) - ((int64_t)pa.y + ia.fx);
              G = ((int64_t)pb.z + ib.lg) - ((int64_t)pa.z + ia.fg);
            } else {
              M = ((int64_t)pa.x + ia.rm - ia.fm) - ((int64_t)pb.x + ib.rm - ib.lm);
              X = ((int64_t)pa.y + ia.rx - ia.fx) - ((int64_t)pb.y + ib.rx - ib.lx);
              G = ((int64_t)pa.z + ia.rg - ia.fg) - ((int64_t)pb.z + ib.rg - ib.lg);
            }
            M += -(int64_t)ia.first_adj_m + ib.last_adj_m;
            X += -(int64_t)ia.first_adj_x + ib.last_adj_x;
          }
          const int32_t total = (int32_t)(M + X + G);
          const double dm = (double)(int32_t)M, dt = (double)total, prod = min_identity * dt;
          bool drop;
          if (dm < prod * (1.0 - 0x1p-50)) drop = true;
          else if (dm > prod * (1.0 + 0x1p-50)) drop = false;
          else drop = (total == 0 ? 0.0 : dm / dt) < min_identity;
          if (drop) res.found = false;
        }
      }
      ok = res.found && res.pqs != res.pqe && res.pts != res.pte;
      if (ok) qid = e1.x;
      res.pqs = qbase + (rev ? -res.pqs : res.pqs);
      res.pqe = qbase + (rev ? -res.pqe : res.pqe);
    }
  }
}

__device__ __forceinline__ uint32_t select_bit64(uint32_t lo, uint32_t hi, uint32_t k) {
  uint32_t c = (uint32_t)__popc(lo), w = lo, base = 0;
  if (k >= c) { k -= c; w = hi; base = 32u; }
  c = (uint32_t)__popc(w & 0xFFFFu); if (k >= c) { k -= c; w >>= 16; base += 16u; }
  c = (uint32_t)__popc(w & 0xFFu);   if (k >= c) { k -= c; w >>= 8; base += 8u; }
  c = (uint32_t)__popc(w & 0xFu);    if (k >= c) { k -= c; w >>= 4; base += 4u; }
  c = (uint32_t)__popc(w & 0x3u);    if (k >= c) { k -= c; w >>= 2; base += 2u; }
  return base + (k >= (w & 1u) ? 1u : 0u);
}
__device__ __forceinline__ void put_ordered_row(const OrderedOut &o, uint32_t d, uint32_t qid, uint32_t tid, bool ok, int32_t qs, int32_t qe,
                                                int32_t ts, int32_t te) {
  const bool on = ok && !(o.min_output_length >= 0 && abs(qe - qs) < o.min_output_length);
  uint32_t *p = reinterpret_cast<uint32_t *>(o.rows) + 6ull * d;
  const uint4 a = make_uint4(on ? qid : HIT_NONE, on ? (uint32_t)qs : 0u, on ? (uint32_t)qe : 0u, tid);
  const uint2 b = make_uint2(on ? (uint32_t)ts : 0u, on ? (uint32_t)te : 0u);
  __builtin_memcpy(p, &a, 16);
  __builtin_memcpy(p + 4, &b, 8);
}
struct PairIn {
  uint32_t eidx, p;
  int32_t f_start, f_end;
  uint32_t live;
};
constexpr uint32_t PROJ_WL_WORDS = 65u + 3u;
constexpr uint32_t PROJ_RG_WORDS = PROJ_BLOCK + 4u * PROJ_BLOCK + PROJ_WAVES + (4u - PROJ_WAVES % 4u) % 4u;
__device__ __forceinline__ PairIn pair_of_place(uint32_t pp, uint32_t lblock, uint32_t n_pairs, const FrontierRec *__restrict__ fr,
                                                const uint32_t *__restrict__ pair_range, const uint32_t *__restrict__ pair_entry,
                                                const ProjList &pl, const WindowLists &wl, uint32_t *wl_off ) {
  PairIn x;
  x.live = pp < n_pairs;
  x.p = pp; x.eidx = 0xFFFFFFFFu; x.f_start = 0; x.f_end = 0;
  uint32_t r = 0;
  if (wl.tile_first && lblock * PROJ_BLOCK >= n_pairs) {
  } else if (wl.tile_first) {
    const uint32_t pp_last = min(lblock * PROJ_BLOCK + PROJ_BLOCK, n_pairs) - 1u;
    uint32_t base_i = wl.tile_first[lblock], ri = 0, k = 0;
    bool found = !x.live;
    for (;;) {
      if (threadIdx.x < 65u) wl_off[threadIdx.x] = base_i + threadIdx.x < wl.n_fr ? wl.pair_off[base_i + threadIdx.x] : 0xFFFFFFFFu;
      __syncthreads();
      const uint32_t lim = wl_off[64];
      if (!found && pp < lim) {
        uint32_t j = 0;
#pragma unroll
        for (uint32_t st = 32u; st > 0u; st >>= 1) j += wl_off[j + st] <= pp ? st : 0u;
        ri = base_i + j;
        k = pp - wl_off[j];
        found = true;
      }
      __syncthreads();
      if (lim > pp_last) break;
      base_i += 64u;
    }
    if (x.live) {
      const uint4 w = wl.win[ri];
      const FrontierRec sf = wl.se[ri];
      const int2 se = make_int2(sf.start, sf.end);
      x.f_start = se.x; x.f_end = se.y;
      if (w.y - (w.x & ~3u) > 64u) x.eidx = pair_entry[pp];
      else x.eidx = w.x + select_bit64(w.z, w.w, k);
      if (wl.range_out) wl.range_out[pp] = wl.range_places ? ri : wl.perm[ri];
    }
  } else if (x.live) {
    if (pl.slot) { x.p = pl.slot[pp]; r = pl.range[pp]; x.eidx = pl.entry[pp]; }
    else { r = pair_range[pp]; x.eidx = pair_entry[pp]; }
    asm volatile("" : "+v"(r), "+v"(x.eidx));
    const FrontierRec f = fr[r];
    x.f_start = f.start; x.f_end = f.end;
  }
  return x;
}
template <uint32_t NB>
__device__ __forceinline__ void regroup_by_entry(PairIn &x, uint32_t *scratch ) {
  uint4 *rg_pay = reinterpret_cast<uint4 *>(scratch);
  uint32_t *rg_hist = scratch + 4u * NB, *rg_ws = rg_hist + NB;
  rg_hist[threadIdx.x] = 0u;
  __syncthreads();
  const uint32_t bin = x.eidx & (NB - 1u);
  const uint32_t pos = atomicAdd(&rg_hist[bin], 1u);
  __syncthreads();
  {
    const uint32_t cnt = rg_hist[threadIdx.x], inc = wave_incl_scan(cnt);
    if (lane_id() == 63u) rg_ws[threadIdx.x >> 6] = inc;
    __syncthreads();
    uint32_t base = 0;
#pragma unroll
    for (uint32_t k = 0; k + 1u < NB / 64u; k++) base += k < (threadIdx.x >> 6) ? rg_ws[k] : 0u;
    rg_hist[threadIdx.x] = base + inc - cnt;
  }
  __syncthreads();
  rg_pay[rg_hist[bin] + pos] = make_uint4(x.eidx, x.p, (uint32_t)x.f_start, (uint32_t)x.f_end);
  __syncthreads();
  const uint4 mine = rg_pay[threadIdx.x];
  x.eidx = mine.x; x.p = mine.y; x.f_start = (int32_t)mine.z; x.f_end = (int32_t)mine.w;
  x.live = x.eidx != 0xFFFFFFFFu;
}
template <uint32_t NW>
__device__ __forceinline__ void count_accepted(uint32_t mine, unsigned long long *__restrict__ accepted, uint32_t *wcnt ) {
  uint32_t w = mine;
#pragma unroll
  for (int o = 32; o > 0; o >>= 1) w += __shfl_xor(w, o);
  if (lane_id() == 0) wcnt[threadIdx.x >> 6] = w;
  __syncthreads();
  if (threadIdx.x == 0) {
    uint32_t tot = 0;
#pragma unroll
    for (uint32_t k = 0; k < NW; k++) tot += wcnt[k];
    if (tot) atomicAdd(&accepted[(blockIdx.x % COUNT_SLOTS) * COUNT_STRIDE], (unsigned long long)tot);
  }
}
template <bool TRANSITIVE, int MODE>
__global__ __launch_bounds__(PROJ_BLOCK) void project_kernel(DeviceIndexView v, const FrontierRec *__restrict__ fr,
                                                      const uint32_t *__restrict__ pair_range,
                                                      const uint32_t *__restrict__ pair_entry, uint32_t n_pairs,
                                                      HitArrays h, unsigned long long *__restrict__ accepted,
                                                      uint32_t *__restrict__ err_flag, double min_identity,
                                                      SliceArrays sl, ProjList pl, int xcd_map,
                                                      const uint32_t *__restrict__ n_pairs_dev, int regroup, WindowLists wl) {
  if (n_pairs_dev) n_pairs = *n_pairs_dev;
  const uint32_t per_xcd = gridDim.x >> 3;
  const uint32_t lblock = xcd_map ? (blockIdx.x & 7u) * per_xcd + (blockIdx.x >> 3) : blockIdx.x;
  const uint32_t pp = lblock * PROJ_BLOCK + threadIdx.x;
#ifdef IMPG_PHASE_CLOCKS
  unsigned long long phase_t[10];
  for (int i = 0; i < 10; i++) phase_t[i] = 0;
  PHASE_MARK(0);
#endif
  bool ok = false;
  TileScan res;
  res.found = res.any = false;
  res.pqs = res.pts = res.pqe = res.pte = -1;
  uint32_t qid = HIT_NONE;
  __shared__ uint32_t wl_off[PROJ_WL_WORDS];
  __shared__ uint4 rg_scratch[PROJ_RG_WORDS / 4u];
  __shared__ uint32_t wcnt[PROJ_WAVES];
  PairIn x = pair_of_place(pp, lblock, n_pairs, fr, pair_range, pair_entry, pl, wl, wl_off);
  PHASE_MARK(1);
  if (regroup) regroup_by_entry<PROJ_BLOCK>(x, reinterpret_cast<uint32_t *>(rg_scratch));
  PHASE_MARK(2);
  if (x.live) {
    project_pair<TRANSITIVE, MODE>(v, x.eidx, x.f_start, x.f_end, x.p, min_identity, err_flag, sl, accepted, ok, qid, res PHASE_PASS);
    h.qid[x.p] = qid;
    if (ok) {
      h.c[x.p] = make_int4(res.pqs, res.pqe, res.pts, res.pte);
    }
  }
  PHASE_MARK(7);
  count_accepted<PROJ_WAVES>(ok ? 1u : 0u, accepted, wcnt);
#ifdef IMPG_PHASE_CLOCKS
// ... 70 lines not shown
      }
    }
    if (!MASKS) {
      e_next = 0xFFFFFFFFu;
      if ((unsigned long long)pp + NT < P1) e_next = pair_entry[pp + NT];
    }
    if (by_visit) {
      v_next = 0u;
      if ((unsigned long long)pp + NT < P1) v_next = wl.ord.vpos[pp + NT];
    }
    if (regroup_all) regroup_by_entry<NT>(y, reinterpret_cast<uint32_t *>(st_line));
    if (y.live) {
      bool ok = false;
      TileScan res;
      res.found = res.any = false;
      res.pqs = res.pts = res.pqe = res.pte = -1;
      uint32_t qid = HIT_NONE;
      const uint32_t slot = y.eidx - emin;
      const uint4 *se = st_ent + min(slot, STG_ECAP - 1u) * (STG_ENT_STRIDE / 4u);
      if (CAN_STAGE && slot < n_e && (se[1].z & OP_LEN_MASK) <= INLINE_TILES * TILE_OPS)
        project_pair<TRANSITIVE, MODE, true>(v, y.eidx, y.f_start, y.f_end, y.p, min_identity, err_flag, no_sl, accepted, ok, qid, res PHASE_PASS, se,
                                             reinterpret_cast<const uint32_t *>(st_line + slot * (STG_REC_STRIDE / 4u)));
      else
        project_pair<TRANSITIVE, MODE>(v, y.eidx, y.f_start, y.f_end, y.p, min_identity, err_flag, no_sl, accepted, ok, qid, res PHASE_PASS);
      if (ordered) put_ordered_row(wl.ord, o_dest, qid, o_tid, ok, res.pqs, res.pqe, res.pts, res.pte);
      else {
        if (qs) reinterpret_cast<uint2 *>(h.qid)[y.p] = make_uint2(qid, o_tid);
        else h.qid[y.p] = qid;
        if (ok) h.c[y.p] = make_int4(res.pqs, res.pqe, res.pts, res.pte);
      }
      n_ok += ok ? 1u : 0u;
    }
    if (regroup_all) __syncthreads();
  }
  return n_ok;
}
template <bool TRANSITIVE, bool MASKS, int OUT = OUT_SLOTS>
__global__ __launch_bounds__(STG_THREADS) void project_staged_kernel(DeviceIndexView v, const uint32_t *__restrict__ pair_entry,
                                                      uint32_t n_pairs, HitArrays h, unsigned long long *__restrict__ accepted,
                                                      uint32_t *__restrict__ err_flag, int regroup, WindowLists wl) {
  const uint32_t per_xcd = gridDim.x >> 3;
  const uint32_t sblock = (blockIdx.x & 7u) * per_xcd + (blockIdx.x >> 3);
  __shared__ uint4 st_ent[STG_ENT_V4];
  __shared__ uint4 st_line[STG_LINE_V4];
  __shared__ uint4 st_win[STG_RANGES];
  __shared__ int2 st_se[STG_RANGES];
  __shared__ uint32_t st_off[STG_RANGES + 4u];
  __shared__ uint32_t st_dest[OUT == OUT_ROWS ? STG_RANGES : 1u], st_tid[OUT == OUT_ROWS ? STG_RANGES : 1u];
  __shared__ uint32_t wred[2u * STG_WAVES];
  __shared__ uint32_t wcnt[STG_WAVES];
  const uint32_t r0 = sblock * STG_RANGES;
  if (r0 >= wl.n_fr) return;
  const uint32_t nr = min(STG_RANGES, wl.n_fr - r0);
  if (OUT == OUT_ROWS && threadIdx.x < nr) st_dest[threadIdx.x] = wl.ord.dest[r0 + threadIdx.x];
#ifdef IMPG_PHASE_CLOCKS
  unsigned long long stg_t[8], phase_t[10];
#define STG_MARK(i) do { asm volatile("s_waitcnt vmcnt(0) lgkmcnt(0)" ::: "memory"); stg_t[i] = __builtin_readcyclecounter(); } while (0)
#else
#define STG_MARK(i) do { } while (0)
#endif
  STG_MARK(0);
  uint32_t emin = 0xFFFFFFFFu, emax = 0u;
  if (threadIdx.x <= STG_RANGES) {
    uint32_t o = 0xFFFFFFFFu;
    if (threadIdx.x < nr) o = wl.pair_off[r0 + threadIdx.x];
    else if (threadIdx.x == nr) o = r0 + nr < wl.n_fr ? wl.pair_off[r0 + nr] : n_pairs;
    st_off[threadIdx.x] = o;
    if (threadIdx.x < nr) {
      const uint4 w = wl.win[r0 + threadIdx.x];
      st_win[threadIdx.x] = w;
      { const FrontierRec sf = wl.se[r0 + threadIdx.x]; st_se[threadIdx.x] = make_int2(sf.start, sf.end); if (OUT == OUT_ROWS) st_tid[threadIdx.x] = sf.target_id; }
      if (w.y - (w.x & ~3u) > 64u) { emin = w.x; emax = w.y - 1u; }
      else if (w.z | w.w) {
        emin = w.x + (w.z ? (uint32_t)__builtin_ctz(w.z) : 32u + (uint32_t)__builtin_ctz(w.w));
        emax = w.x + (w.w ? 63u - (uint32_t)__builtin_clz(w.w) : 31u - (uint32_t)__builtin_clz(w.z));
      }
    }
  }
  {
#pragma unroll
    for (int o = 32; o > 0; o >>= 1) {
      emin = min(emin, (uint32_t)__shfl_xor((int)emin, o));
      emax = max(emax, (uint32_t)__shfl_xor((int)emax, o));
    }
    if (lane_id() == 0) { wred[threadIdx.x >> 6] = emin; wred[STG_WAVES + (threadIdx.x >> 6)] = emax; }
    __syncthreads();
#pragma unroll
    for (uint32_t k = 0; k < STG_WAVES; k++) { emin = min(emin, wred[k]); emax = max(emax, wred[STG_WAVES + k]); }
  }
  const uint32_t P0 = st_off[0], P1 = st_off[nr];
  uint32_t n_ok = 0;
  STG_MARK(1);
  const bool sparse = emin <= emax && emax - emin >= 4u * STG_ECAP;
  uint32_t n_e = 0;
  if (emin <= emax && !sparse) {
    n_e = min(STG_ECAP, emax - emin + 1u);
    if (threadIdx.x < n_e * 4u) st_ent[(threadIdx.x >> 2) * (STG_ENT_STRIDE / 4u) + (threadIdx.x & 3u)] = reinterpret_cast<const uint4 *>(v.entries + emin)[threadIdx.x];
    __syncthreads();
    const uint32_t w = threadIdx.x >> 6, l = lane_id();
    constexpr uint32_t TURNS = (STG_ECAP + STG_WAVES - 1u) / STG_WAVES;
    uint4 buf[TURNS];
#pragma unroll
    for (uint32_t k = 0; k < TURNS; k++) {
      const uint32_t i = w + k * STG_WAVES;
      buf[k] = make_uint4(0u, 0u, 0u, 0u);
      if (i < n_e) {
        const uint4 e1 = st_ent[i * (STG_ENT_STRIDE / 4u) + 1u];
        const uint32_t n = e1.z & OP_LEN_MASK, m = (n + TILE_OPS - 1u) / TILE_OPS;
        if (m <= INLINE_TILES && (l >> 3) < m) buf[k] = reinterpret_cast<const uint4 *>(v.pfx + (size_t)e1.y * TILE_WORDS)[l];
      }
    }
#pragma unroll
    for (uint32_t k = 0; k < TURNS; k++) {
      const uint32_t i = w + k * STG_WAVES;
      if (i < n_e) st_line[i * (STG_REC_STRIDE / 4u) + (l >> 3) * (STG_LINE_STRIDE / 4u) + (l & 7u)] = buf[k];
    }
    __syncthreads();
  }
  STG_MARK(2);
  n_ok = project_places<TRANSITIVE, MASKS, true, STG_RANGES, STG_THREADS, 0, OUT>(v, pair_entry, h, accepted, err_flag, wl, r0, P0, P1, emin, n_e,
                                                                                  sparse && regroup != 0, st_off, st_win, st_se, st_ent, st_line PHASE_PASS,
                                                                                  0.0, st_dest, OUT == OUT_ROWS ? st_tid : nullptr);
#ifdef IMPG_PHASE_CLOCKS
  STG_MARK(3);
  if ((blockIdx.x & 15u) == 0u && threadIdx.x == 0u) {
    if (sparse) {
      atomicAdd(&g_phase_clk[13], stg_t[3] - stg_t[0]);
      atomicAdd(&g_phase_clk[14], 1ull);
      atomicAdd(&g_phase_clk[12], (unsigned long long)(emax - emin));
    } else {
      for (int i = 0; i < 3; i++) atomicAdd(&g_phase_clk[i], stg_t[i + 1] - stg_t[i]);
      atomicAdd(&g_phase_clk[9], (unsigned long long)(P1 - P0));
      atomicAdd(&g_phase_clk[10], emin <= emax && emax - emin >= STG_ECAP ? 1ull : 0ull);
      atomicAdd(&g_phase_clk[15], 1ull);
      atomicAdd(&g_phase_clk[11], emin <= emax ? (unsigned long long)(emax - emin + 1u) : 0ull);
    }
  }
#endif
  count_accepted<STG_WAVES>(n_ok, accepted, wcnt);
}
#undef STG_MARK

#ifndef IMPG_ENT_RANGES
#define IMPG_ENT_RANGES 512
#endif
#ifndef IMPG_ENT_THREADS
#define IMPG_ENT_THREADS 256
#endif
constexpr uint32_t ENT_RANGES = IMPG_ENT_RANGES;
constexpr uint32_t ENT_THREADS = IMPG_ENT_THREADS, ENT_WAVES = ENT_THREADS / 64u;
constexpr uint32_t ENT_REC_STRIDE = ENT_CP_OFF + 16u;
static_assert((ENT_RANGES & (ENT_RANGES - 1u)) == 0u && ENT_RANGES % ENT_THREADS == 0 && ENT_THREADS % 64u == 0, "whole turns of the block over its ranges");
constexpr uint32_t ENT_REC_V4 = ENT_WAVES * ENT_REC_STRIDE / 4u, ENT_LIST_V4 = ENT_WAVES * ENT_RANGES * 2u / 16u;
static_assert((ENT_REC_V4 + ENT_LIST_V4) * 4u >= 5u * ENT_THREADS + ENT_WAVES, "the unstaged path's scratch overlays the waves' records and lists");
#ifndef IMPG_ENT_WAVES
#define IMPG_ENT_WAVES 6
#endif
template <bool TRANSITIVE, int ORIENT, int MODE, int OUT>
__device__ __forceinline__ void project_entry_chunk(const DeviceIndexView &v, uint4 e0, uint4 e1, uint4 e2, uint4 e3, uint32_t eidx, bool live,
                                                    int32_t f_start, int32_t f_end, uint32_t p, const uint32_t *rec, const HitArrays &h,
                                                    unsigned long long *__restrict__ accepted, uint32_t *__restrict__ err_flag,
                                                    uint32_t &n_ok PHASE_ARG, double min_identity, const OrderedOut &ord, uint32_t tid) {
  const SliceArrays no_sl{nullptr, nullptr, nullptr, nullptr};
  if (live) {
    bool ok = false;
    TileScan res;
    res.found = res.any = false;
    res.pqs = res.pts = res.pqe = res.pte = -1;
    uint32_t qid = HIT_NONE;
    if (ORIENT >= 0) {
      e0 = reinterpret_cast<const uint4 *>(__builtin_assume_aligned(rec, 16))[ENT_CP_OFF / 4u + 3u];
      asm volatile("" : "+v"(e0.x), "+v"(e0.y), "+v"(e0.z), "+v"(e0.w));
    }
    if (ORIENT >= 0)
      project_core<TRANSITIVE, MODE, true, ORIENT>(v, e0, e1, e2, e3, f_start, f_end, p, min_identity, err_flag, no_sl, accepted, ok, qid, res PHASE_PASS, rec);
    else
      project_pair<TRANSITIVE, MODE>(v, eidx, f_start, f_end, p, min_identity, err_flag, no_sl, accepted, ok, qid, res PHASE_PASS);
    if (OUT == OUT_ROWS) put_ordered_row(ord, p, qid, tid, ok, res.pqs, res.pqe, res.pts, res.pte);
    else {
      if (OUT == OUT_QS) reinterpret_cast<uint2 *>(h.qid)[p] = make_uint2(qid, tid);
      else h.qid[p] = qid;
      if (ok) h.c[p] = make_int4(res.pqs, res.pqe, res.pts, res.pte);
    }
    n_ok += ok ? 1u : 0u;
  }
}
#ifndef IMPG_ENT_SLICE_PAIRS
#define IMPG_ENT_SLICE_PAIRS 32768
#endif
constexpr uint32_t ENT_SLICE_PAIRS = IMPG_ENT_SLICE_PAIRS, ENT_MAX_SLICES = 64u;
#ifndef IMPG_ENT_SPARSE
#define IMPG_ENT_SPARSE 4
#endif
constexpr uint32_t ENT_SPARSE = IMPG_ENT_SPARSE;
struct EntSlices {
  uint32_t *work;
  uint32_t *alloc;
  uint32_t cap;
  int phase;
};
template <bool TRANSITIVE, int MODE, int OUT>
__global__ __launch_bounds__(ENT_THREADS) __attribute__((amdgpu_waves_per_eu(IMPG_ENT_WAVES, IMPG_ENT_WAVES)))
void project_entries_kernel(DeviceIndexView v, const uint32_t *__restrict__ pair_entry, uint32_t n_pairs,
                                                      HitArrays h, unsigned long long *__restrict__ accepted,
                                                      uint32_t *__restrict__ err_flag, int regroup, WindowLists wl, double min_identity, EntSlices sl) {
  const uint32_t per_xcd = gridDim.x >> 3;
  uint32_t sblock = (blockIdx.x & 7u) * per_xcd + (blockIdx.x >> 3);
  uint32_t slice = 0u, n_slices = 1u;
  if (sl.phase) {
    if (blockIdx.x >= min(sl.work[0], sl.cap)) return;
    const uint32_t item = sl.work[1u + blockIdx.x];
    sblock = item >> 12; slice = (item >> 6) & 63u; n_slices = (item & 63u) + 1u;
  }
  __shared__ uint4 st_work[ENT_REC_V4 + ENT_LIST_V4];
  uint4 (*st_rec)[ENT_REC_STRIDE / 4u] = reinterpret_cast<uint4 (*)[ENT_REC_STRIDE / 4u]>(st_work);
  uint16_t (*st_list)[ENT_RANGES] = reinterpret_cast<uint16_t (*)[ENT_RANGES]>(st_work + ENT_REC_V4);
  __shared__ uint4 st_win[ENT_RANGES];
  __shared__ int2 st_se[ENT_RANGES];
  __shared__ uint32_t st_off[ENT_RANGES + 4u];
  __shared__ uint16_t st_wide[ENT_RANGES];
  __shared__ uint32_t st_dest[OUT == OUT_ROWS ? ENT_RANGES : 1u];
  constexpr bool ordered = OUT == OUT_ROWS;
  constexpr bool qs = OUT == OUT_QS;
  constexpr bool WIDE_LISTED = ordered;
  __shared__ uint32_t st_nwide, st_alloc, st_next;
  __shared__ uint32_t wred[2u * ENT_WAVES];
  __shared__ uint32_t wcnt[ENT_WAVES];
  const uint32_t r0 = sblock * ENT_RANGES;
  if (r0 >= wl.n_fr) return;
  const uint32_t nr = min(ENT_RANGES, wl.n_fr - r0);
  const uint32_t wv = (uint32_t)__builtin_amdgcn_readfirstlane((int)(threadIdx.x >> 6)), l = lane_id();
#ifdef IMPG_PHASE_CLOCKS
  unsigned long long stg_t[8], phase_t[10];
#define STG_MARK(i) do { asm volatile("s_waitcnt vmcnt(0) lgkmcnt(0)" ::: "memory"); stg_t[i] = __builtin_readcyclecounter(); } while (0)
#else
#define STG_MARK(i) do { } while (0)
#endif
  STG_MARK(0);
  if (threadIdx.x == 0) { st_nwide = 0u; st_alloc = 0u; st_next = 0u; }
  __syncthreads();
  uint32_t emin = 0xFFFFFFFFu, emax = 0u;
#pragma unroll
  for (uint32_t t = threadIdx.x; t < ENT_RANGES; t += ENT_THREADS) {
    if (t < nr) st_off[t] = wl.pair_off[r0 + t];
    else st_off[t + 1u] = 0xFFFFFFFFu;
    if (t == 0) st_off[nr] = r0 + nr < wl.n_fr ? wl.pair_off[r0 + nr] : n_pairs;
    uint32_t glo = 0xFFFFFFFFu, ghi = 0u;
    if (t < nr) {
      const uint4 w = wl.win[r0 + t];
      st_win[t] = w;
      { const FrontierRec sf = wl.se[r0 + t]; st_se[t] = make_int2(sf.start, sf.end); }
      if (ordered) st_dest[t] = wl.ord.dest[r0 + t];
      if (w.y - (w.x & ~3u) > 64u) {
        if (WIDE_LISTED) st_wide[atomicAdd(&st_nwide, 1u)] = (uint16_t)t;
        else if (w.x < w.y) { glo = w.x; ghi = w.y - 1u; emin = min(emin, glo); emax = max(emax, ghi); }
      } else if (w.z | w.w) {
        glo = w.x + (w.z ? (uint32_t)__builtin_ctz(w.z) : 32u + (uint32_t)__builtin_ctz(w.w));
        ghi = w.x + (w.w ? 63u - (uint32_t)__builtin_clz(w.w) : 31u - (uint32_t)__builtin_clz(w.z));
        emin = min(emin, glo);
        emax = max(emax, ghi);
      }
    }
  }
  {
#pragma unroll
    for (int o = 32; o > 0; o >>= 1) {
      emin = min(emin, (uint32_t)__shfl_xor((int)emin, o));
      emax = max(emax, (uint32_t)__shfl_xor((int)emax, o));
    }
    if (l == 0) { wred[wv] = emin; wred[ENT_WAVES + wv] = emax; }
    __syncthreads();
#pragma unroll
    for (uint32_t k = 0; k < ENT_WAVES; k++) { emin = min(emin, wred[k]); emax = max(emax, wred[ENT_WAVES + k]); }
    emin = (uint32_t)__builtin_amdgcn_readfirstlane((int)emin);
    emax = (uint32_t)__builtin_amdgcn_readfirstlane((int)emax);
  }
  const uint32_t P0 = st_off[0], P1 = st_off[nr];
  const bool compact = !ordered;
  uint32_t n_ok = 0;
  STG_MARK(1);
  const bool sparse = emin <= emax && (unsigned long long)(P1 - P0) < (unsigned long long)ENT_SPARSE * (emax - emin + 1u);
  if (!sl.phase && sl.work && !sparse && emin <= emax && P1 - P0 > ENT_SLICE_PAIRS && (uint32_t)__builtin_amdgcn_readfirstlane((int)st_nwide) == 0u) {
    n_slices = min(ENT_MAX_SLICES, (P1 - P0 + ENT_SLICE_PAIRS - 1u) / ENT_SLICE_PAIRS);
    if (threadIdx.x == 0) {
      const uint32_t at = atomicAdd(&sl.work[0], n_slices - 1u);
      for (uint32_t k = 1; k < n_slices; k++)
        if (at + k - 1u < sl.cap) sl.work[1u + at + k - 1u] = sblock << 12 | k << 6 | (n_slices - 1u);
    }
  }
  if (sparse) {
    n_ok = project_places<TRANSITIVE, true, false, ENT_RANGES, ENT_THREADS, MODE, OUT>(v, pair_entry, h, accepted, err_flag, wl, r0, P0, P1, emin, 0u, regroup != 0, st_off, st_win,
                                                               st_se, nullptr, st_work PHASE_PASS, min_identity, st_dest);
  } else if (emin <= emax) {
    const uint4 *ents = reinterpret_cast<const uint4 *>(v.entries);
    const uint4 zero4 = make_uint4(0u, 0u, 0u, 0u);
    const uint32_t n_span = emax - emin + 1u;
    auto take = [&]() -> uint32_t {
      uint32_t i = 0;
      if (l == 0) i = atomicAdd(&st_next, 1u);
      i = (uint32_t)__builtin_amdgcn_readfirstlane((int)i);
      return n_slices > 1u ? min(n_span, slice + i * n_slices) : i;
    };
    uint32_t ic = take(), in = take();
    uint4 cq = zero4, nq = zero4, lc = zero4;
    auto fetch_entry = [&](uint32_t i) -> uint4 {
      uint4 q = zero4;
      if (i < n_span && l < 4u) q = ents[(size_t)(emin + i) * 4u + l];
      return q;
    };
#define IMPG_RDL(x, j) (uint32_t)__builtin_amdgcn_readlane((int)(x), j)
    auto fetch_record = [&](const uint4 &q) -> uint4 {
      uint4 r = zero4;
      const uint32_t nz = IMPG_RDL(q.z, 1), ny = IMPG_RDL(q.y, 1);
      const uint32_t m = ((nz & OP_LEN_MASK) + TILE_OPS - 1u) / TILE_OPS;
      if (m <= INLINE_TILES && (l >> 3) < m) r = reinterpret_cast<const uint4 *>(v.pfx + (size_t)ny * TILE_WORDS)[l];
      return r;
    };
    cq = fetch_entry(ic);
    nq = fetch_entry(in);
    if (ic < n_span) lc = fetch_record(cq);
#pragma unroll 1
    while (ic < n_span) {
      const uint32_t eidx = emin + ic;
      __builtin_amdgcn_wave_barrier();
      st_rec[wv][(l >> 3) * (STG_LINE_STRIDE / 4u) + (l & 7u)] = lc;
      if (l < 4u) st_rec[wv][ENT_CP_OFF / 4u + ((l + 3u) & 3u)] = cq;
      uint4 e0, e1, e2, e3;
      e0.x = IMPG_RDL(cq.x, 0); e0.y = IMPG_RDL(cq.y, 0); e0.z = IMPG_RDL(cq.z, 0); e0.w = IMPG_RDL(cq.w, 0);
      e1.x = IMPG_RDL(cq.x, 1); e1.y = IMPG_RDL(cq.y, 1); e1.z = IMPG_RDL(cq.z, 1); e1.w = IMPG_RDL(cq.w, 1);
      e2.x = IMPG_RDL(cq.x, 2); e2.y = IMPG_RDL(cq.y, 2); e2.z = IMPG_RDL(cq.z, 2); e2.w = IMPG_RDL(cq.w, 2);
      e3.x = IMPG_RDL(cq.x, 3); e3.y = IMPG_RDL(cq.y, 3); e3.z = IMPG_RDL(cq.z, 3); e3.w = IMPG_RDL(cq.w, 3);
      ic = in;
      cq = nq;
      lc = zero4;
      if (ic < n_span) {
        lc = fetch_record(cq);
        in = take();
        nq = fetch_entry(in);
      }
      uint32_t cnt = 0;
      const int32_t e_end = TRANSITIVE ? ((int32_t)e0.x < (int32_t)e0.y ? (int32_t)e0.y : (-2147483647 - 1)) : (int32_t)e0.y;
#pragma unroll
      for (uint32_t q = 0; q < ENT_RANGES / 64u; q++) {
        const uint32_t r = q * 64u + l;
        bool hit = false;
        if (r < nr) {
          const uint4 w = st_win[r];
          const uint32_t d = eidx - w.x;
          if (w.y - (w.x & ~3u) <= 64u) hit = d < 64u && (((d < 32u ? w.z >> d : w.w >> (d - 32u)) & 1u) != 0u);
          else if (!WIDE_LISTED) hit = eidx >= w.x && eidx < w.y && window_hit<TRANSITIVE>(e_end, st_se[r].x);
        }
        const unsigned long long b = __ballot(hit);
        if (hit) st_list[wv][cnt + (uint32_t)__popcll(b & lanemask_lt())] = (uint16_t)r;
        cnt += (uint32_t)__popcll(b);
      }
      uint32_t run = 0;
      if (compact) {
        if (l == 0) run = n_slices > 1u ? atomicAdd(&sl.alloc[sblock], cnt) : atomicAdd(&st_alloc, cnt);
        run = P0 + (uint32_t)__builtin_amdgcn_readfirstlane((int)run);
      }
      asm volatile("s_waitcnt lgkmcnt(0)" ::: "memory");
      __builtin_amdgcn_wave_barrier();
      const uint32_t *rec = reinterpret_cast<const uint32_t *>(&st_rec[wv][0]);
      const int orient = (e1.z & OP_LEN_MASK) > INLINE_TILES * TILE_OPS ? -1 : !(e1.z & EF_REVERSED) ? 0 : (e1.z & EF_STRAND) ? 2 : 1;
      uint32_t tid = 0;
      if (ordered && cnt) tid = wl.se[r0 + (uint32_t)__builtin_amdgcn_readfirstlane((int)st_list[wv][0])].target_id;
#pragma unroll 1
      for (uint32_t k0 = 0; k0 < cnt; k0 += 64u) {
        const bool live = k0 + l < cnt;
        const uint32_t r = live ? (uint32_t)st_list[wv][k0 + l] : 0u;
        const int2 se = st_se[r];
        uint32_t p = run + k0 + l;
        if (!compact) {
          const uint4 w = st_win[r];
          const uint32_t d = eidx - w.x;
          const uint32_t below = d < 32u ? (uint32_t)__popc(w.z & ((1u << d) - 1u))
                                         : (uint32_t)__popc(w.z) + (uint32_t)__popc(w.w & ((1u << (d - 32u)) - 1u));
          p = st_off[r] + below;
        }
        if (ordered) {
          if (live) p = st_dest[r] + (uint32_t)wl.ord.vpos[p];
        } else if (qs) tid = r0 + r;
        else if (live && wl.range_out) wl.range_out[p] = wl.range_places ? r0 + r : wl.perm[r0 + r];
        if (orient == 0) project_entry_chunk<TRANSITIVE, 0, MODE, OUT>(v, e0, e1, e2, e3, eidx, live, se.x, se.y, p, rec, h, accepted, err_flag, n_ok PHASE_PASS, min_identity, wl.ord, tid);
        else if (orient == 1) project_entry_chunk<TRANSITIVE, 1, MODE, OUT>(v, e0, e1, e2, e3, eidx, live, se.x, se.y, p, rec, h, accepted, err_flag, n_ok PHASE_PASS, min_identity, wl.ord, tid);
        else if (orient == 2) project_entry_chunk<TRANSITIVE, 2, MODE, OUT>(v, e0, e1, e2, e3, eidx, live, se.x, se.y, p, rec, h, accepted, err_flag, n_ok PHASE_PASS, min_identity, wl.ord, tid);
        else project_entry_chunk<TRANSITIVE, -1, MODE, OUT>(v, e0, e1, e2, e3, eidx, live, se.x, se.y, p, rec, h, accepted, err_flag, n_ok PHASE_PASS, min_identity, wl.ord, tid);
      }
    }
#undef IMPG_RDL
#ifdef IMPG_PHASE_CLOCKS
    STG_MARK(2);
    if ((blockIdx.x & 15u) == 0u && threadIdx.x == 0u) {
      atomicAdd(&g_phase_clk[0], stg_t[1] - stg_t[0]);
      atomicAdd(&g_phase_clk[2], stg_t[2] - stg_t[1]);
      atomicAdd(&g_phase_clk[9], (unsigned long long)(P1 - P0));
      atomicAdd(&g_phase_clk[15], 1ull);
      atomicAdd(&g_phase_clk[11], (unsigned long long)(emax - emin + 1u));
    }
#endif
  }
  if (!sparse) {
    const SliceArrays no_sl{nullptr, nullptr, nullptr, nullptr};
    const uint32_t nw = st_nwide;
#pragma unroll 1
    for (uint32_t k = 0; k < nw; k++) {
      const uint32_t r = st_wide[k];
      const uint32_t a = st_off[r], b = st_off[r + 1u];
      const int2 se = st_se[r];
#pragma unroll 1
      for (uint32_t pp = a + threadIdx.x; pp < b; pp += ENT_THREADS) {
        bool ok = false;
        TileScan res;
        res.found = res.any = false;
        res.pqs = res.pts = res.pqe = res.pte = -1;
        uint32_t qid = HIT_NONE;
        project_pair<TRANSITIVE, MODE>(v, pair_entry[pp], se.x, se.y, pp, min_identity, err_flag, no_sl, accepted, ok, qid, res PHASE_PASS);
        if (ordered)
          put_ordered_row(wl.ord, st_dest[r] + (pp - a), qid, wl.se[r0 + r].target_id, ok, res.pqs, res.pqe, res.pts, res.pte);
        else {
          if (qs) reinterpret_cast<uint2 *>(h.qid)[pp] = make_uint2(qid, r0 + r);
          else h.qid[pp] = qid;
          if (ok) h.c[pp] = make_int4(res.pqs, res.pqe, res.pts, res.pte);
        }
        n_ok += ok ? 1u : 0u;
        if (wl.range_out && !ordered && !qs) wl.range_out[pp] = wl.range_places ? r0 + r : wl.perm[r0 + r];
      }
    }
  }
#ifdef IMPG_PHASE_CLOCKS
  if (sparse && (blockIdx.x & 15u) == 0u && threadIdx.x == 0u) {
    STG_MARK(3);
    atomicAdd(&g_phase_clk[13], stg_t[3] - stg_t[0]);
    atomicAdd(&g_phase_clk[14], 1ull);
    atomicAdd(&g_phase_clk[12], (unsigned long long)(emax - emin));
  }
#endif
  count_accepted<ENT_WAVES>(n_ok, accepted, wcnt);
}
#undef STG_MARK
#ifdef IMPG_PHASE_CLOCKS
extern "C" void impg_gpu_debug_phase_clocks(unsigned long long *out) {
  unsigned long long z[16] = {};
  (void)hipDeviceSynchronize();
  (void)hipMemcpyFromSymbol(out, HIP_SYMBOL(g_phase_clk), sizeof(z));
  (void)hipMemcpyToSymbol(HIP_SYMBOL(g_phase_clk), z, sizeof(z));
}
#endif

__device__ __forceinline__ int32_t tp_refine(int32_t query_pos, int32_t query_delta, int32_t seg_start, int32_t overlap_pos,
                                             int32_t abs_target_delta, bool first, int32_t lo, int32_t hi) {
  int32_t refined;
  if (abs_target_delta == 0) {
    refined = first ? query_pos : query_pos + query_delta;
  } else {
    const double target_fraction = (double)(overlap_pos - seg_start) / (double)abs_target_delta;
    const double indel_ratio = (double)query_delta / (double)abs_target_delta;
    const double query_advance = target_fraction * (double)abs_target_delta * indel_ratio;
    const double r = round(query_advance);
    const int32_t adv = r >= 2147483647.0 ? 2147483647 : r <= -2147483648.0 ? (-2147483647 - 1) : (int32_t)r;
    refined = (int32_t)((uint32_t)query_pos + (uint32_t)adv);
  }
  return min(max(refined, lo), hi);
}
template <bool TRANSITIVE, bool CIGAR = false>
__global__ __launch_bounds__(256) void project_tp_kernel(DeviceIndexView v, const FrontierRec *__restrict__ fr,
                                                         const uint32_t *__restrict__ pair_range,
                                                         const uint32_t *__restrict__ pair_entry, uint32_t n_pairs,
                                                         HitArrays h, unsigned long long *__restrict__ accepted,
                                                         uint32_t *__restrict__ err_flag, double min_identity, int use_ident,
                                                         ProjList pl, const uint32_t *__restrict__ n_pairs_dev,
                                                         SliceArrays sl = SliceArrays{nullptr, nullptr, nullptr, nullptr}) {
  if (n_pairs_dev) n_pairs = *n_pairs_dev;
  const uint32_t per_xcd = gridDim.x >> 3;
  const uint32_t lblock = (blockIdx.x & 7u) * per_xcd + (blockIdx.x >> 3);
  const uint32_t pp = lblock * 256u + threadIdx.x;
  bool ok = false;
  if (pp < n_pairs) {
    const uint32_t p = pl.slot ? pl.slot[pp] : pp;
    const uint32_t r = pl.slot ? pl.range[pp] : pair_range[p];
    const FrontierRec f = fr[r];
    const uint4 *ep = reinterpret_cast<const uint4 *>(v.entries + (pl.slot ? pl.entry[pp] : pair_entry[p]));
    const uint4 e0 = ep[0], e1 = ep[1];
    const int32_t m_ts = (int32_t)e0.x, m_te = (int32_t)e0.y, m_qs = (int32_t)e0.z, m_qe = (int32_t)e0.w;
    const uint32_t n = e1.z & OP_LEN_MASK;
    const bool is_reverse = (e1.z & EF_STRAND) != 0, reversed_entry = (e1.z & EF_REVERSED) != 0;
    int32_t rs = f.start, re = f.end;
    if (TRANSITIVE) { rs = max(rs, m_ts); re = min(re, m_te); }
    uint32_t qid = HIT_NONE;
    int4 out = make_int4(0, 0, 0, 0);
    if (!(m_ts >= re || m_te <= rs) && n) {
      const uint4 *B = reinterpret_cast<const uint4 *>(v.ops) + e1.y;
      const int sdir = reversed_entry ? 1 : (is_reverse ? -1 : 1);
      const int pdir = reversed_entry ? (is_reverse ? -1 : 1) : 1;
      const int32_t s0 = reversed_entry ? m_ts : (is_reverse ? m_te : m_ts);
      const int32_t p0 = reversed_entry ? (is_reverse ? m_qe : m_qs) : m_qs;
      const int64_t x_lo = sdir > 0 ? (int64_t)rs - s0 : (int64_t)s0 - re, x_hi = sdir > 0 ? (int64_t)re - s0 : (int64_t)s0 - rs;
      auto S = [&](uint32_t k) -> int64_t { const uint4 b = B[k]; return (int64_t)(reversed_entry ? b.y : b.x); };
      uint32_t lo = 1, hi = n + 1;
      while (lo < hi) { const uint32_t mid = (lo + hi) >> 1; if (S(mid) <= x_lo) lo = mid + 1; else hi = mid; }
      const uint32_t first = lo - 1;
      lo = 0; hi = n;
      while (lo < hi) { const uint32_t mid = (lo + hi) >> 1; if (S(mid) < x_hi) lo = mid + 1; else hi = mid; }
      if (first < n && lo > 0 && first <= lo - 1) {
        const uint32_t last = lo - 1;
        const uint4 bf0 = B[first], bf1 = B[first + 1], bl0 = B[last], bl1 = B[last + 1];
        auto seg = [&](const uint4 &a, const uint4 &b, int32_t &ppos, int32_t &pdelta, int32_t &sstart, int32_t &send, int32_t &asd) {
          const int32_t sa = (int32_t)(reversed_entry ? a.y : a.x), sb = (int32_t)(reversed_entry ? b.y : b.x);
          const int32_t ja = (int32_t)(reversed_entry ? a.x : a.y), jb = (int32_t)(reversed_entry ? b.x : b.y);
          const int32_t pa = s0 + sdir * sa, pb = s0 + sdir * sb;
          sstart = min(pa, pb); send = max(pa, pb); asd = sb - sa;
          ppos = p0 + pdir * ja; pdelta = pdir * (jb - ja);
        };
        const int32_t qlo = min(m_qs, m_qe), qhi = max(m_qs, m_qe);
        int32_t ppos, pdelta, sstart, send, asd;
        seg(bf0, bf1, ppos, pdelta, sstart, send, asd);
        const int32_t refined_first = tp_refine(ppos, pdelta, sstart, max(sstart, rs), asd, true, qlo, qhi);
        seg(bl0, bl1, ppos, pdelta, sstart, send, asd);
        const int32_t refined_last = tp_refine(ppos, pdelta, sstart, min(send, re), asd, false, qlo, qhi);
        bool keep = true;
        int64_t mm = 0, xx = 0;
        if (CIGAR || use_ident) { mm = (int64_t)bl1.z - bf0.z; xx = (int64_t)bl1.w - bf0.w; }
        if (use_ident) {
          const int64_t total = mm + xx;
          const double ident = total == 0 ? 0.0 : (double)mm / (double)total;
          keep = !(ident < min_identity);
        }
        if (keep) {
          if (refined_first < 0 || refined_last < 0) atomicOr(err_flag, 2u);
          const bool swap_q = is_reverse && !reversed_entry;
          out = make_int4(swap_q ? refined_last : refined_first, swap_q ? refined_first : refined_last, rs, re);
          qid = e1.x;
          ok = true;
          if (CIGAR) {
            const bool fits = mm <= (int64_t)OP_LEN_MASK && xx <= (int64_t)OP_LEN_MASK;
            if (!fits) atomicOr(err_flag, 4u);
            sl.a[p] = (uint32_t)mm;
            sl.off[p] = (int32_t)xx;
            sl.n[p] = fits ? (mm > 0 ? 1u : 0u) + (xx > 0 ? 1u : 0u) : 0u;
            sl.rem[p] = 0;
          }
        }
      }
    }
    h.qid[p] = qid;
    if (ok) h.c[p] = out;
  }
  __shared__ uint32_t wcnt[4];
  unsigned long long m = __ballot(ok);
  if (lane_id() == 0) wcnt[threadIdx.x >> 6] = __popcll(m);
  __syncthreads();
  if (threadIdx.x == 0) {
    uint32_t tot = wcnt[0] + wcnt[1] + wcnt[2] + wcnt[3];
    if (tot) atomicAdd(&accepted[(blockIdx.x % COUNT_SLOTS) * COUNT_STRIDE], (unsigned long long)tot);
  }
// ... 2786 lines not shown
```

### impg_amd/csrc/kernels.hpp

```cpp
#pragma once
#include <hip/hip_runtime.h>

#include <cstdint>

#include "impg_internal.hpp"

namespace impg {

struct FrontierRec {
  uint32_t target_id;
  int32_t start, end;
  uint32_t qidx;
};

struct HitArrays {
  uint32_t *qid;
  int4 *c;
};

struct SliceArrays {
  uint32_t *a;
  uint32_t *n;
  int32_t *off;
  int32_t *rem;
};

struct VisitedTable {
  const unsigned long long *keys;
  const uint32_t *off, *len;
  const int2 *ranges;
  const uint32_t *qoff;
  uint32_t n_groups;
};
constexpr int MAX_VISITED_TABLES = 48;
constexpr uint32_t COUNT_SLOTS = 64, COUNT_STRIDE = 16;
constexpr size_t COUNT_BYTES = (size_t)COUNT_SLOTS * COUNT_STRIDE * 8;
struct VisitedTables {
  VisitedTable t[MAX_VISITED_TABLES];
  uint32_t n_tables;
  const uint32_t *mask_off;
  const int2 *mask_ranges;
};

constexpr uint32_t LK_WORDS = 8, LK_REACH_BASE = 2, LK_REACH_SINGLE = 0, LK_REACH_GROUPED = 1, LK_REACH_PASSES = 2;
constexpr uint32_t WIDE_CAP = 4096, WIDE_BINS = 1024;
struct WideEmit { uint32_t cap = WIDE_CAP, bins = WIDE_BINS; bool count_reach = false; };
enum LookupStat { LK_WIDE = 0, LK_SINGLE, LK_GROUPED, LK_GROUP_PASSES, LK_OVERFLOW, LK_STATS };
static_assert(LK_STATS == sizeof(impg_gpu_index::lk_stats) / sizeof(impg_gpu_index::lk_stats[0]), "one counter per path");
void launch_lookup_count(const DeviceIndexView &v, const FrontierRec *fr, uint32_t n, bool transitive, const uint32_t *perm,
                         uint32_t *cnt, uint4 *win, uint32_t *wide_n, uint32_t *wide_list, hipStream_t s, bool by_place = false,
                         FrontierRec *se = nullptr ,
                         uint32_t *cnt_ref = nullptr ,
                         bool count_reach = false );
struct OrdDestArgs { const FrontierRec *frp; const uint32_t *perm, *slot_ref, *offsets, *lvbase; uint32_t *dest; };
void launch_emit_vpos(const DeviceIndexView &v, uint32_t n, const uint32_t *pair_off, const uint4 *win, uint8_t *vpos, hipStream_t s, bool by_visit = false,
                      const OrdDestArgs *dest = nullptr);
void launch_ord_self_count(const FrontierRec *self, const impg_gpu_range_t *ranges, uint32_t n, uint32_t *acc, hipStream_t s);
void launch_ord_level_bases(const FrontierRec *fr, uint32_t n_fr, const uint32_t *slot_ref, uint32_t total, uint32_t n_queries, uint32_t *acc,
                            uint32_t *lvbase, hipStream_t s);
void launch_ord_self_rows(const FrontierRec *self, const impg_gpu_range_t *ranges, uint32_t n, const uint32_t *offsets, impg_gpu_interval_t *rows,
                          hipStream_t s);
void launch_ord_run_heads(const uint32_t *pair_range, uint32_t n_pairs, uint32_t *run_start, hipStream_t s);
void launch_ord_level_rows(const FrontierRec *fr, const uint32_t *pair_range, uint32_t n_pairs, HitArrays h, const uint32_t *run_start,
                           const uint32_t *slot_ref, const uint32_t *offsets, const uint32_t *lvbase, int32_t min_output_length,
                           impg_gpu_interval_t *rows, hipStream_t s);
struct OrderedOut {
  impg_gpu_interval_t *rows;
  const uint32_t *dest;
  const uint8_t *vpos;
  int32_t min_output_length;
  uint32_t by_visit;
};
bool ordered_rows_by_visit();
struct WindowLists {
  const uint32_t *tile_first;
  const uint32_t *pair_off;
  const uint4 *win;
  const FrontierRec *se;
  const uint32_t *perm;
  uint32_t n_fr;
  uint32_t *range_out;
  uint32_t masks;
  uint32_t range_places;
  uint32_t *slice_work, *slice_alloc;
  uint32_t slice_cap;
  OrderedOut ord;
};
bool project_is_staged(const DeviceIndexView &v, uint64_t n_pairs, bool plain);
bool project_entry_major(const DeviceIndexView &v, uint64_t n_pairs, double min_identity);
uint32_t project_entry_blocks(uint32_t n_fr);
uint32_t project_entry_slice_cap(uint64_t n_pairs);
void launch_tile_first(const uint32_t *cnt, const uint32_t *pair_off, uint32_t n_fr, uint32_t *tile_first, hipStream_t s);
bool emit_by_lanes(const DeviceIndexView &v);
struct ProjList {
  uint32_t *slot, *range, *entry;
};
void launch_lookup_emit(const DeviceIndexView &v, const FrontierRec *fr, uint32_t n, bool transitive,
                        const uint32_t *pair_off, const uint4 *win, uint32_t *pair_range, uint32_t *pair_entry,
                        const uint32_t *perm, const uint32_t *offp, ProjList pl, const uint32_t *wide_n,
                        const uint32_t *wide_list, hipStream_t s, bool by_place = false, bool wide_only = false, WideEmit we = WideEmit{});
constexpr uint32_t ROUTE_WORLD_MAX = 1024;
void launch_route_keys(const FrontierRec *fr, uint32_t n, uint32_t world, const uint32_t *owner, uint32_t n_seq, uint32_t *key,
                       uint32_t *idx, unsigned long long *hist, hipStream_t s);
void launch_hits_pack(const FrontierRec *fr, const uint32_t *pair_range, uint32_t n_pairs, HitArrays h, const uint32_t *pair_entry,
                      const uint32_t *mrank, uint32_t words, void *out, hipStream_t s, const uint32_t *slice_n = nullptr);
void launch_hits_slice_n(const void *in, uint32_t n, uint32_t *cnt, hipStream_t s);
void launch_hits_unpack(const void *in, uint32_t n, uint32_t words, uint32_t n_front, const uint32_t *run_start, const uint32_t *off,
                        uint32_t *pair_range, HitArrays h, uint32_t *mslot, hipStream_t s, const uint32_t *slice_at = nullptr,
                        uint32_t *slice_pos = nullptr, uint32_t *slice_n = nullptr);
void launch_route_gather(const FrontierRec *fr, const uint32_t *perm, uint32_t n, FrontierRec *out, hipStream_t s);
void launch_route_gather_ranges(const FrontierRec *fr, const uint32_t *perm, uint32_t n, uint32_t range_base, FrontierRec *out, hipStream_t s);
void launch_partial_stats_add(const unsigned long long *in, uint32_t blocks, uint32_t n, unsigned long long *out, hipStream_t s);
void launch_frontier_gather(const FrontierRec *fr, const uint32_t *perm, uint32_t n, FrontierRec *out, hipStream_t s);
void launch_reorder_runs(const uint32_t *hits, uint32_t n, uint32_t words, uint32_t n_front, uint32_t *run_start,
                         uint32_t *run_len, uint32_t *err, hipStream_t s);
void launch_order_keys(const DeviceIndexView &v, const FrontierRec *fr, uint32_t n, uint32_t *key, uint32_t *idx, hipStream_t s,
                       const uint32_t *bounds = nullptr, uint32_t n_blocks = 0, uint32_t block_shift = 0);
void launch_scatter_u32(const uint32_t *in, const uint32_t *perm, uint32_t n, uint32_t *out, hipStream_t s);
void launch_exclusive_scan(const uint32_t *d_in, uint32_t *d_out, uint32_t n, unsigned long long *d_bsum,
                           unsigned long long *d_total, hipStream_t s);
size_t scan_scratch_bytes(uint32_t n);
enum ProjArm : int {
  PROJ_ARM_NONE = -1,
  PROJ_ARM_LANE = 0,
  PROJ_ARM_STAGED,
  PROJ_ARM_STAGED_ROWS,
  PROJ_ARM_ENTRIES_SLOTS,
  PROJ_ARM_ENTRIES_QS,
  PROJ_ARM_ENTRIES_ROWS,
  PROJ_ARM_ENTRIES_IDENT,
  PROJ_ARM_TP,
  PROJ_ARMS
};
static_assert(PROJ_ARMS == sizeof(impg_gpu_index::proj_stats) / sizeof(impg_gpu_index::proj_stats[0]), "one counter per arm");
enum UpdStat {
  UPD_LANE = 0, UPD_MID, UPD_WAVE_TINY, UPD_WAVE_SMALL, UPD_WAVE_LARGE,
  UPD_INPLACE,
  UPD_TILED_SORT,
  UPD_LANE_SPILL,
  UPD_STATS
};
static_assert(UPD_STATS == sizeof(impg_gpu_index::upd_stats) / sizeof(impg_gpu_index::upd_stats[0]), "one counter per path");
int launch_project(const DeviceIndexView &v, const FrontierRec *fr, const uint32_t *pair_range,
                   const uint32_t *pair_entry, uint32_t n_pairs, bool transitive, HitArrays h,
                   unsigned long long *accepted, uint32_t *err_flag, double min_identity, const SliceArrays *slices,
                   ProjList pl, hipStream_t s, const uint32_t *n_pairs_dev = nullptr, bool regroup = false,
                   const WindowLists *wl = nullptr);
constexpr uint32_t SMALL_HEADER_BYTES = 64;
void launch_small_scan(const uint32_t *cnt, uint32_t n, uint32_t *off, uint32_t *total, hipStream_t s);
void launch_small_pack(const FrontierRec *fr, const uint32_t *pair_range, const uint32_t *n_pairs_dev, uint32_t pairs_bound, HitArrays h,
                       const uint32_t *err_flag, const unsigned long long *accepted, void *hdr, impg_gpu_interval_t *rows,
                       uint32_t *row_range, hipStream_t s);
void launch_slice_counts(HitArrays h, SliceArrays sl, uint32_t n_pairs, uint32_t *cnt, hipStream_t s);
void launch_slice_write(const DeviceIndexView &v, const uint32_t *pair_entry, HitArrays h, SliceArrays sl, uint32_t n_pairs,
                        const uint32_t *off, uint32_t *out, hipStream_t s);
void launch_hit_stats(const FrontierRec *fr, uint32_t n_fr, const uint32_t *pair_range, uint32_t n_pairs, HitArrays h,
                      int32_t min_output_length, bool skip_same_target, unsigned long long *rstat, unsigned long long *count,
                      unsigned long long *cksum, hipStream_t s, uint32_t stride = 1 );
void launch_sort5(const FrontierRec *fr, uint32_t n, const uint32_t *pair_off, uint32_t n_pairs, HitArrays h,
                  const uint32_t *pair_entry, const uint32_t *mrank, uint32_t *dest, hipStream_t s);
void launch_permute_slots(const uint32_t *dest, uint32_t n_pairs, HitArrays in, HitArrays out, const uint32_t *pe_in,
                          uint32_t *pe_out, SliceArrays sin, SliceArrays sout, hipStream_t s);
void launch_update_keys(const FrontierRec *fr, const uint32_t *pair_range, uint32_t n_pairs, HitArrays h,
                        unsigned long long *keys, unsigned long long *vals, unsigned long long *n_active, hipStream_t s);
size_t sort_pairs_scratch_bytes(uint32_t n);
void launch_sort_pairs(void *tmp, size_t tmp_bytes, const unsigned long long *kin, unsigned long long *kout,
                       const uint32_t *vin, uint32_t *vout, uint32_t n, unsigned end_bit, hipStream_t s);
uint32_t group_tiles(uint32_t n);
void launch_group_count(const unsigned long long *skeys, uint32_t n, uint32_t *tile_heads, hipStream_t s);
void launch_group_fill(const unsigned long long *skeys, uint32_t n, const uint32_t *tile_base, uint32_t *gstart, unsigned long long *gkey, hipStream_t s);
void launch_group_heads(const unsigned long long *skeys, uint32_t n, uint32_t *head, hipStream_t s);
void launch_group_scatter(const unsigned long long *skeys, uint32_t n, const uint32_t *head, const uint32_t *gid,
                          uint32_t *gstart, unsigned long long *gkey, hipStream_t s);
void launch_table_qoff(const unsigned long long *keys, uint32_t n_groups, uint32_t n_queries, uint32_t *qoff, hipStream_t s);
void launch_group_prepare(const VisitedTables &vt, const unsigned long long *gkey, const uint32_t *gstart,
                          uint32_t n_groups, uint32_t n_active, uint32_t *glen, const int2 **old_src,
                          uint32_t *cap, uint32_t *pcap, hipStream_t s);
constexpr uint32_t VU_NBIG_WORDS = 12, VU_REACH_BASE = 8, VU_REACH_INPLACE = 0, VU_REACH_TILED_SORT = 1, VU_REACH_LANE_SPILL = 2;
void launch_visited_update(const unsigned long long *svals, const int32_t *seq_len,
                           const unsigned long long *gkey, const uint32_t *gstart, const uint32_t *glen,
                           const int2 *const *old_src, const uint32_t *noff, const uint32_t *poff,
                           uint32_t n_groups, int32_t min_transitive_len, int32_t mdbr, int2 *new_ranges,
                           uint32_t *new_len, int2 *pieces, uint32_t *n_pieces, const uint32_t *cap, const uint32_t *pcap,
                           uint32_t *big_list, uint32_t *n_big, bool count_reach, hipStream_t s);
void launch_covered_flags(const unsigned long long *svals, const uint32_t *head, const uint32_t *gid,
                          const unsigned long long *gkey, const int2 *const *old_src, const uint32_t *cap, const uint32_t *glen,
                          const int32_t *seq_len, uint32_t n_active, uint32_t *keep, hipStream_t s);
void launch_covered_compact(const unsigned long long *svals, const uint32_t *keep, const uint32_t *kpos, uint32_t n_active,
                            unsigned long long *out, uint32_t n_kept, uint32_t n_groups, uint32_t *gstart, uint32_t *glen, uint32_t *cap,
                            uint32_t *pcap, hipStream_t s);
void launch_frontier_emit(const unsigned long long *gkey, const uint32_t *poff, const uint32_t *n_pieces,
                          const uint32_t *foff, uint32_t n_groups, const int2 *pieces, FrontierRec *out, hipStream_t s,
                          const DeviceIndexView *v = nullptr, uint32_t *key = nullptr, uint32_t *idx = nullptr);
void launch_subset_filter(const FrontierRec *fr, const uint32_t *pair_range, uint32_t n_pairs, uint32_t *qid,
                          const uint8_t *keep, const impg_gpu_range_t *ranges, hipStream_t s);
void launch_mask_caps(const impg_gpu_range_t *ranges, uint32_t n, const uint32_t *mask_off, uint32_t n_seq, uint32_t *cap,
                      hipStream_t s);
void launch_visited_init_masked(const impg_gpu_range_t *ranges, uint32_t n, const int32_t *init_len, uint32_t n_seq,
                                const uint32_t *mask_off, const int2 *mask_ranges, int32_t min_transitive_len,
                                const uint32_t *loff, unsigned long long *keys, uint32_t *len, int2 *rng, int2 *pieces,
                                uint32_t *n_self, uint32_t *n_front, hipStream_t s);
void launch_masked_self_emit(const impg_gpu_range_t *ranges, uint32_t n, const uint32_t *loff, const uint32_t *n_self,
                             const uint32_t *self_off, const uint32_t *front_off, int32_t min_transitive_len,
                             const int2 *pieces, FrontierRec *self_out, FrontierRec *frontier_out, hipStream_t s);
void launch_visited_init(const impg_gpu_range_t *ranges, uint32_t n, const int32_t *seq_len, uint32_t n_seq,
                         int32_t min_transitive_len, unsigned long long *keys, uint32_t *off, uint32_t *len, int2 *rng,
                         FrontierRec *self_iv, uint32_t *in_frontier, hipStream_t s);
void launch_compact_frontier(const FrontierRec *in, const uint32_t *flag, const uint32_t *pos, uint32_t n,
                             FrontierRec *out, hipStream_t s);
void launch_ranges_to_frontier(const impg_gpu_range_t *ranges, uint32_t n, FrontierRec *out, uint32_t *bad, hipStream_t s);

void launch_frontier_to_stack(const FrontierRec *fr, uint32_t n, const uint32_t *pop_depth, bool use_depth,
                              unsigned long long *key, int32_t *st, int32_t *en, uint32_t *depth, hipStream_t s);
void launch_dfs_pop_flags(const unsigned long long *key, const uint32_t *depth, uint32_t n, uint32_t max_depth,
                          bool pop_front, uint32_t *fr_flag, uint32_t *keep_flag, uint32_t *pop_depth, uint32_t *pop_sel ,
                          uint32_t n_queries, hipStream_t s);
void launch_dfs_pop_scatter(const unsigned long long *key, const int32_t *st, const int32_t *en, const uint32_t *depth,
                            uint32_t n, const uint32_t *fr_flag, const uint32_t *fr_pos, const uint32_t *keep_flag,
                            const uint32_t *keep_pos, FrontierRec *fr_out, unsigned long long *key_out, int32_t *st_out,
                            int32_t *en_out, uint32_t *depth_out, hipStream_t s);
void launch_iota(uint32_t *v, uint32_t n, hipStream_t s);
void launch_gather_u32(const uint32_t *src, const uint32_t *idx, uint32_t n, uint32_t *dst, hipStream_t s);
void launch_gather_u64(const unsigned long long *src, const uint32_t *idx, uint32_t n, unsigned long long *dst, hipStream_t s);
void launch_run_heads(const unsigned long long *skeys, uint32_t n, uint32_t *head, hipStream_t s);
void launch_run_starts(const uint32_t *head, const uint32_t *gid, uint32_t n, uint32_t *gstart, hipStream_t s);
void launch_dfs_merge(const uint32_t *gstart, uint32_t n_groups, uint32_t n, const uint32_t *perm, const int32_t *st,
                      const int32_t *en, const uint32_t *depth, int32_t *st_m, int32_t *en_m, uint32_t *depth_m,
                      uint32_t *cnt, hipStream_t s);
void launch_dfs_compact(const uint32_t *gstart, const uint32_t *cnt, const uint32_t *off, uint32_t n_groups,
                        const unsigned long long *skeys, const int32_t *st_m, const int32_t *en_m, const uint32_t *depth_m,
                        unsigned long long *key_out, int32_t *st_out, int32_t *en_out, uint32_t *depth_out, hipStream_t s);
size_t sort_u32_scratch_bytes(uint32_t n);
void launch_sort_u32(void *tmp, size_t tmp_bytes, const uint32_t *kin, uint32_t *kout, const uint32_t *vin, uint32_t *vout,
                     uint32_t n, hipStream_t s, unsigned begin_bit = 0, unsigned end_bit = 32);
size_t order_sort_scratch_bytes(uint32_t n);
void launch_order_sort(uint32_t *keys, uint32_t *key_tmp, uint32_t *perm_out, uint32_t *perm_tmp, uint32_t n, unsigned end_bit, void *scratch,
                       hipStream_t s);
#ifdef IMPG_OS_CLOCKS
// ... 75 lines not shown
```

Before: 71.24 billion.

## Carry partial-wave tails across same-class entries in entry-major projection

In the compact (non-ordered) entry-major projection kernel, entries in a block are reordered by orientation class through a per-block ballot sort. When consecutive entries share a class, the leftover ranges of one entry (fewer than a full wave) are stored in the record's padding and processed together with the next entry's first chunk. This needs two record buffers per wave, and entry fields are read from the staged record instead of register broadcasts. The goal is fewer partially filled 64-lane passes, at the cost of more shared memory, extra synchronisation and a reordering prologue.

```diff
diff --git a/impg_amd/csrc/capi.cpp b/impg_amd/csrc/capi.cpp
--- a/impg_amd/csrc/capi.cpp
+++ b/impg_amd/csrc/capi.cpp
@@ -47,6 +47,9 @@
   e->upd_stats = ix.upd_stats;
   e->wide_emit = WideEmit{ix.opt_wide_cap, ix.opt_wide_bins, ix.opt_lookup_stats};
   e->lk_stats = ix.lk_stats;
+  e->tail_carry = ix.opt_tail_carry;
+  e->tail_stats = ix.opt_tail_stats;
+  e->tail_joins = &ix.tail_joins;
 }
 static Engine *take_or_create(impg_gpu_index &ix) {
   Engine *e = nullptr;
@@ -629,6 +632,10 @@
     ix->opt_update_stats = value != 0;
   } else if (k == "lookup_stats") {
     ix->opt_lookup_stats = value != 0;
+  } else if (k == "entries_tail_carry") {
+    ix->opt_tail_carry = value != 0;
+  } else if (k == "entries_tail_stats") {
+    ix->opt_tail_stats = value != 0;
   } else if (k == "wide_emit_cap") {
     if (value < 64 || value > (long long)WIDE_CAP) throw Error{IMPG_E_INVALID, "wide_emit_cap is 64 .. 4096"};
     ix->opt_wide_cap = (uint32_t)value;
@@ -692,6 +699,7 @@
   else if (k == "update_inplace_groups") *value_out = (int64_t)ix->upd_stats[UPD_INPLACE].load();
   else if (k == "update_tiled_sort_groups") *value_out = (int64_t)ix->upd_stats[UPD_TILED_SORT].load();
   else if (k == "update_lane_spill_groups") *value_out = (int64_t)ix->upd_stats[UPD_LANE_SPILL].load();
+  else if (k == "entries_tail_joins") *value_out = (int64_t)ix->tail_joins.load();
   else if (k == "lookup_wide_windows") *value_out = (int64_t)ix->lk_stats[LK_WIDE].load();
   else if (k == "lookup_wide_single") *value_out = (int64_t)ix->lk_stats[LK_SINGLE].load();
   else if (k == "lookup_wide_grouped") *value_out = (int64_t)ix->lk_stats[LK_GROUPED].load();
diff --git a/impg_amd/csrc/engine.cpp b/impg_amd/csrc/engine.cpp
--- a/impg_amd/csrc/engine.cpp
+++ b/impg_amd/csrc/engine.cpp
@@ -431,6 +431,12 @@
       IMPG_HIP(hipMemsetAsync(ent_work.p, 0, 4, stream));
       IMPG_HIP(hipMemsetAsync(ent_alloc.p, 0, (size_t)nb * 4, stream));
       wlists.slice_work = ent_work.as<uint32_t>(); wlists.slice_alloc = ent_alloc.as<uint32_t>(); wlists.slice_cap = cap;
+      wlists.tail_carry = tail_carry ? 1u : 0u;
+      if (tail_stats && tail_joins) {
+        ent_joins.reserve(256);
+        IMPG_HIP(hipMemsetAsync(ent_joins.p, 0, 4, stream));
+        wlists.tail_joins = ent_joins.as<uint32_t>();
+      }
     }
     L.qs_interleaved = last_range_places && project_entry_major(v, P, min_identity) && !(min_identity == min_identity) && !store_cigar && !getenv("IMPG_NO_QS");
     if (L.qs_interleaved) { wlists.masks |= 4u; wlists.range_out = nullptr; }
@@ -468,6 +474,12 @@
   count_arm(launch_project(v, fr, L.pair_range.as<uint32_t>(), pair_entry.as<uint32_t>(), L.n_pairs, transitive, h,
                            acc_slots.as<unsigned long long>(), (uint32_t *)(counters.as<uint64_t>() + 2), min_identity,
                            store_cigar ? &sl : nullptr, pl, stream, nullptr, regroup_pairs, by_place ? &wlists : nullptr));
+  if (wlists.tail_joins) {
+    uint32_t n = 0;
+    IMPG_HIP(hipMemcpyAsync(&n, wlists.tail_joins, 4, hipMemcpyDeviceToHost, stream));
+    IMPG_HIP(hipStreamSynchronize(stream));
+    *tail_joins += n;
+  }
   if (!raw && !direct) {
     post_expand(fr, n_fr, L, pair_off.as<uint32_t>(), pair_entry.as<uint32_t>(), v.mrank, sl);
     h = HitArrays{L.qid.as<uint32_t>(), L.coords.as<int4>()};
diff --git a/impg_amd/csrc/engine.hpp b/impg_amd/csrc/engine.hpp
--- a/impg_amd/csrc/engine.hpp
+++ b/impg_amd/csrc/engine.hpp
@@ -117,6 +117,10 @@
   DevBuf wide_n, wide_list;
   WideEmit wide_emit;
   std::atomic<uint64_t> *lk_stats = nullptr;
+  bool tail_carry = true;
+  bool tail_stats = false;
+  std::atomic<uint64_t> *tail_joins = nullptr;
+  DevBuf ent_joins;
   void count_wide_paths(const DeviceIndexView &v, uint32_t n);
   DevBuf lo_key, lo_key2, lo_idx, lo_perm, lo_cnt, lo_off, lo_offp, slot_of;
   uint32_t locality_min = 4096;
diff --git a/impg_amd/csrc/impg_internal.hpp b/impg_amd/csrc/impg_internal.hpp
--- a/impg_amd/csrc/impg_internal.hpp
+++ b/impg_amd/csrc/impg_internal.hpp
@@ -346,6 +346,8 @@
   int opt_filter_covered = 0;
   bool opt_update_stats = false;
   bool opt_lookup_stats = false;
+  bool opt_tail_carry = true;
+  bool opt_tail_stats = false;
   bool opt_approx_cigar = false;
   uint32_t opt_wide_cap = 4096, opt_wide_bins = 1024;
   int opt_walk = 1;
@@ -359,6 +361,7 @@
   mutable std::atomic<uint64_t> proj_stats[8] = {};
   mutable std::atomic<uint64_t> upd_stats[8] = {};
   mutable std::atomic<uint64_t> lk_stats[5] = {};
+  mutable std::atomic<uint64_t> tail_joins{0};
   impg::ShardCtx *shard = nullptr;
   impg::Cluster *cluster = nullptr;
   impg_gpu_index();
diff --git a/impg_amd/csrc/kernels.hip b/impg_amd/csrc/kernels.hip
--- a/impg_amd/csrc/kernels.hip
+++ b/impg_amd/csrc/kernels.hip
@@ -1196,9 +1196,10 @@
     FrontierRec f;
     f.start = f_start; f.end = f_end;
     const int32_t en_ts = (int32_t)e0.x, en_te = (int32_t)e0.y, en_qs = (int32_t)e0.z, en_qe = (int32_t)e0.w;
-    const uint32_t nops_flags = e1.z;
+    constexpr bool ON_REC = STAGED && ORIENT >= 0;
+    const uint32_t nops_flags = ON_REC ? st_pfx[ENT_CP_OFF + 2u] : e1.z;
     const uint32_t n = nops_flags & OP_LEN_MASK;
-    const bool rev = (nops_flags & EF_STRAND) != 0;
+    const bool rev = ORIENT == 1 ? false : ORIENT == 2 ? true : (nops_flags & EF_STRAND) != 0;
     PairCtx c;
     c.swp = ORIENT < 0 ? (nops_flags & EF_REVERSED) != 0 : ORIENT >= 1;
     c.flip = ORIENT < 0 ? c.swp && rev : ORIENT == 2;
@@ -1220,7 +1221,7 @@
       c.totT = st_pfx[ENT_CP_OFF + 3u];
       c.totQ = st_pfx[ENT_CP_OFF + 4u];
     }
-    c.ops = v.ops + (size_t)e1.y * TILE_WORDS;
+    c.ops = ON_REC ? nullptr : v.ops + (size_t)e1.y * TILE_WORDS;
     if (n == 0) {
       atomicOr(err_flag, 1u);
     } else {
@@ -1316,7 +1317,7 @@
             lit = (pfx_rec[(size_t)(c.m - 1u) * LSTRIDE] >> 31) != 0u;
           }
           if (IDENT && !lit) {
-            const uint32_t *idl = reinterpret_cast<const uint32_t *>(v.idp) + (size_t)e1.y * IDL_WORDS;
+            const uint32_t *idl = reinterpret_cast<const uint32_t *>(v.idp) + (size_t)(ON_REC ? st_pfx[ENT_CP_OFF + 1u] : e1.y) * IDL_WORDS;
             const uint32_t *la = idl + (size_t)lo_op.j * IDL_WORDS, *lb = idl + (size_t)hi_op.j * IDL_WORDS;
             uint4 ha = make_uint4(0u, 0u, 0u, 0u), hb = *reinterpret_cast<const uint4 *>(lb);
             u32x2_u ea = {0u, 0u}, eb = *reinterpret_cast<const u32x2_u *>(lb + IDL_E0 + hi_op.k);
@@ -1335,6 +1336,7 @@
             lineX += (ax1 != ax0 ? lo_adj : 0) + (bx1 != bx0 ? hi_adj : 0);
           }
           if (lit) {
+            if (ON_REC) c.ops = v.ops + (size_t)st_pfx[ENT_CP_OFF + 1u] * TILE_WORDS;
             res = walk_tiles<MODE>(c, orig_tile(c, kA), c.flip ? 0u : c.m - 1u, ia);
             walked = true;
           } else {
@@ -1460,9 +1462,10 @@
         }
       }
       ok = res.found && res.pqs != res.pqe && res.pts != res.pte;
-      if (ok) qid = e1.x;
-      res.pqs = qbase + (rev ? -res.pqs : res.pqs);
-      res.pqe = qbase + (rev ? -res.pqe : res.pqe);
+      if (ok) qid = ON_REC ? st_pfx[ENT_CP_OFF] : e1.x;
+      const bool rev_out = ON_REC && ORIENT == 0 ? (st_pfx[ENT_CP_OFF + 2u] & EF_STRAND) != 0 : rev;
+      res.pqs = qbase + (rev_out ? -res.pqs : res.pqs);
+      res.pqe = qbase + (rev_out ? -res.pqe : res.pqe);
     }
   }
 }
@@ -1839,12 +1842,16 @@
 constexpr uint32_t ENT_REC_STRIDE = ENT_CP_OFF + 16u;
 static_assert((ENT_RANGES & (ENT_RANGES - 1u)) == 0u && ENT_RANGES % ENT_THREADS == 0 && ENT_THREADS % 64u == 0, "whole turns of the block over its ranges");
 constexpr uint32_t ENT_REC_V4 = ENT_WAVES * ENT_REC_STRIDE / 4u, ENT_LIST_V4 = ENT_WAVES * ENT_RANGES * 2u / 16u;
+constexpr uint32_t ENT_SPARSE_OFF = (5u * ENT_THREADS + ENT_WAVES + 3u) & ~3u;
 static_assert((ENT_REC_V4 + ENT_LIST_V4) * 4u >= 5u * ENT_THREADS + ENT_WAVES, "the unstaged path's scratch overlays the waves' records and lists");
+static_assert((2u * ENT_REC_V4 + ENT_LIST_V4) * 4u >= ENT_SPARSE_OFF + ENT_RANGES + 4u, "... and, in the compact forms, so do the sparse branch's offsets");
+constexpr uint32_t ENT_ORDER = ENT_THREADS;
+static_assert(ENT_ORDER <= 256u && TILE_WORDS + 4u == STG_LINE_STRIDE && INLINE_TILES * 8u == 64u, "a byte names a span index; a record's padding holds a tail of 63 ranges");
 #ifndef IMPG_ENT_WAVES
 #define IMPG_ENT_WAVES 6
 #endif
 template <bool TRANSITIVE, int ORIENT, int MODE, int OUT>
-__device__ __forceinline__ void project_entry_chunk(const DeviceIndexView &v, uint4 e0, uint4 e1, uint4 e2, uint4 e3, uint32_t eidx, bool live,
+__device__ __forceinline__ void project_entry_chunk(const DeviceIndexView &v, uint32_t eidx, bool live,
                                                     int32_t f_start, int32_t f_end, uint32_t p, const uint32_t *rec, const HitArrays &h,
                                                     unsigned long long *__restrict__ accepted, uint32_t *__restrict__ err_flag,
                                                     uint32_t &n_ok PHASE_ARG, double min_identity, const OrderedOut &ord, uint32_t tid) {
@@ -1856,11 +1863,12 @@
     res.pqs = res.pts = res.pqe = res.pte = -1;
     uint32_t qid = HIT_NONE;
     if (ORIENT >= 0) {
-      e0 = reinterpret_cast<const uint4 *>(__builtin_assume_aligned(rec, 16))[ENT_CP_OFF / 4u + 3u];
+      const uint4 *cp = reinterpret_cast<const uint4 *>(__builtin_assume_aligned(rec, 16)) + ENT_CP_OFF / 4u;
+      uint4 e0 = cp[3];
       asm volatile("" : "+v"(e0.x), "+v"(e0.y), "+v"(e0.z), "+v"(e0.w));
-    }
-    if (ORIENT >= 0)
-      project_core<TRANSITIVE, MODE, true, ORIENT>(v, e0, e1, e2, e3, f_start, f_end, p, min_identity, err_flag, no_sl, accepted, ok, qid, res PHASE_PASS, rec);
+      const uint4 z4 = make_uint4(0u, 0u, 0u, 0u);
+      project_core<TRANSITIVE, MODE, true, ORIENT>(v, e0, z4, z4, z4, f_start, f_end, p, min_identity, err_flag, no_sl, accepted, ok, qid, res PHASE_PASS, rec);
+    }
     else
       project_pair<TRANSITIVE, MODE>(v, eidx, f_start, f_end, p, min_identity, err_flag, no_sl, accepted, ok, qid, res PHASE_PASS);
     if (OUT == OUT_ROWS) put_ordered_row(ord, p, qid, tid, ok, res.pqs, res.pqe, res.pts, res.pte);
@@ -1899,15 +1907,19 @@
     const uint32_t item = sl.work[1u + blockIdx.x];
     sblock = item >> 12; slice = (item >> 6) & 63u; n_slices = (item & 63u) + 1u;
   }
-  __shared__ uint4 st_work[ENT_REC_V4 + ENT_LIST_V4];
+  constexpr bool ordered = OUT == OUT_ROWS;
+  constexpr bool CARRY = !ordered;
+  constexpr uint32_t N_REC = CARRY ? 2u : 1u;
+  __shared__ uint4 st_work[N_REC * ENT_REC_V4 + ENT_LIST_V4];
   uint4 (*st_rec)[ENT_REC_STRIDE / 4u] = reinterpret_cast<uint4 (*)[ENT_REC_STRIDE / 4u]>(st_work);
-  uint16_t (*st_list)[ENT_RANGES] = reinterpret_cast<uint16_t (*)[ENT_RANGES]>(st_work + ENT_REC_V4);
+  uint16_t (*st_list)[ENT_RANGES] = reinterpret_cast<uint16_t (*)[ENT_RANGES]>(st_work + N_REC * ENT_REC_V4);
   __shared__ uint4 st_win[ENT_RANGES];
   __shared__ int2 st_se[ENT_RANGES];
-  __shared__ uint32_t st_off[ENT_RANGES + 4u];
-  __shared__ uint16_t st_wide[ENT_RANGES];
+  __shared__ uint32_t st_off[CARRY ? 4u : ENT_RANGES + 4u];
+  __shared__ uint16_t st_wide[CARRY ? 1u : ENT_RANGES];
   __shared__ uint32_t st_dest[OUT == OUT_ROWS ? ENT_RANGES : 1u];
-  constexpr bool ordered = OUT == OUT_ROWS;
+  __shared__ uint8_t st_order[CARRY ? ENT_ORDER : 4u];
+  __shared__ uint32_t st_ccnt[4u * ENT_WAVES];
   constexpr bool qs = OUT == OUT_QS;
   constexpr bool WIDE_LISTED = ordered;
   __shared__ uint32_t st_nwide, st_alloc, st_next;
@@ -1929,10 +1941,13 @@
   uint32_t emin = 0xFFFFFFFFu, emax = 0u;
 #pragma unroll
   for (uint32_t t = threadIdx.x; t < ENT_RANGES; t += ENT_THREADS) {
-    if (t < nr) st_off[t] = wl.pair_off[r0 + t];
-    else st_off[t + 1u] = 0xFFFFFFFFu;
-    if (t == 0) st_off[nr] = r0 + nr < wl.n_fr ? wl.pair_off[r0 + nr] : n_pairs;
+    if (!CARRY) {
+      if (t < nr) st_off[t] = wl.pair_off[r0 + t];
+      else st_off[t + 1u] = 0xFFFFFFFFu;
+      if (t == 0) st_off[nr] = r0 + nr < wl.n_fr ? wl.pair_off[r0 + nr] : n_pairs;
+    }
     uint32_t glo = 0xFFFFFFFFu, ghi = 0u;
+    if (t >= nr) st_win[t] = make_uint4(0u, 0u, 0u, 0u);
     if (t < nr) {
       const uint4 w = wl.win[r0 + t];
       st_win[t] = w;
@@ -1962,7 +1977,8 @@
     emin = (uint32_t)__builtin_amdgcn_readfirstlane((int)emin);
     emax = (uint32_t)__builtin_amdgcn_readfirstlane((int)emax);
   }
-  const uint32_t P0 = st_off[0], P1 = st_off[nr];
+  const uint32_t P0 = CARRY ? wl.pair_off[r0] : st_off[0];
+  const uint32_t P1 = CARRY ? (r0 + nr < wl.n_fr ? wl.pair_off[r0 + nr] : n_pairs) : st_off[nr];
   const bool compact = !ordered;
   uint32_t n_ok = 0;
   STG_MARK(1);
@@ -1976,17 +1992,53 @@
     }
   }
   if (sparse) {
-    n_ok = project_places<TRANSITIVE, true, false, ENT_RANGES, ENT_THREADS, MODE, OUT>(v, pair_entry, h, accepted, err_flag, wl, r0, P0, P1, emin, 0u, regroup != 0, st_off, st_win,
+    const uint32_t *offs = st_off;
+    if (CARRY) {
+      uint32_t *so = reinterpret_cast<uint32_t *>(st_work) + ENT_SPARSE_OFF;
+#pragma unroll
+      for (uint32_t t = threadIdx.x; t < ENT_RANGES; t += ENT_THREADS) {
+        if (t < nr) so[t] = wl.pair_off[r0 + t];
+        else so[t + 1u] = 0xFFFFFFFFu;
+        if (t == 0) so[nr] = P1;
+      }
+      __syncthreads();
+      offs = so;
+    }
+    n_ok = project_places<TRANSITIVE, true, false, ENT_RANGES, ENT_THREADS, MODE, OUT>(v, pair_entry, h, accepted, err_flag, wl, r0, P0, P1, emin, 0u, regroup != 0, offs, st_win,
                                                                st_se, nullptr, st_work PHASE_PASS, min_identity, st_dest);
   } else if (emin <= emax) {
     const uint4 *ents = reinterpret_cast<const uint4 *>(v.entries);
     const uint4 zero4 = make_uint4(0u, 0u, 0u, 0u);
     const uint32_t n_span = emax - emin + 1u;
+    auto entry_class = [](uint32_t w6) -> uint32_t {
+      return (w6 & OP_LEN_MASK) > INLINE_TILES * TILE_OPS ? 3u : !(w6 & EF_REVERSED) ? 0u : (w6 & EF_STRAND) ? 2u : 1u;
+    };
+    const bool carry = CARRY && wl.tail_carry != 0u;
+    const bool by_class = carry && n_span <= ENT_ORDER;
+    if (CARRY && by_class) {
+      const uint32_t t = threadIdx.x;
+      uint32_t c = 4u, rank = 0u;
+      if (t < n_span) c = entry_class(reinterpret_cast<const uint32_t *>(v.entries)[(size_t)(emin + t) * 16u + 6u]);
+#pragma unroll
+      for (uint32_t k = 0; k < 4u; k++) {
+        const unsigned long long b = __ballot(c == k);
+        if (c == k) rank = (uint32_t)__popcll(b & lanemask_lt());
+        if (l == 0) st_ccnt[k * ENT_WAVES + wv] = (uint32_t)__popcll(b);
+      }
+      __syncthreads();
+      uint32_t base = 0u;
+#pragma unroll
+      for (uint32_t k = 0; k < 4u * ENT_WAVES; k++) base += k < c * ENT_WAVES + wv ? st_ccnt[k] : 0u;
+      if (t < n_span) st_order[base + rank] = (uint8_t)t;
+      __syncthreads();
+    }
     auto take = [&]() -> uint32_t {
       uint32_t i = 0;
       if (l == 0) i = atomicAdd(&st_next, 1u);
       i = (uint32_t)__builtin_amdgcn_readfirstlane((int)i);
-      return n_slices > 1u ? min(n_span, slice + i * n_slices) : i;
+      if (n_slices > 1u) i = min(n_span, slice + i * n_slices);
+      if (CARRY && by_class && i < n_span) i = (uint32_t)__builtin_amdgcn_readfirstlane((int)st_order[i]);
+      return i;
     };
     uint32_t ic = take(), in = take();
     uint4 cq = zero4, nq = zero4, lc = zero4;
@@ -2006,32 +2058,36 @@
     cq = fetch_entry(ic);
     nq = fetch_entry(in);
     if (ic < n_span) lc = fetch_record(cq);
+    uint32_t pend = 0u, pend_p = 0u;
+    uint32_t rec_c = wv * N_REC;
+    auto tail_at = [&](uint32_t rec_i, uint32_t k) -> uint16_t * {
+      return reinterpret_cast<uint16_t *>(reinterpret_cast<uint32_t *>(&st_rec[rec_i][0]) + (k >> 3) * STG_LINE_STRIDE + TILE_WORDS) + (k & 7u);
+    };
 #pragma unroll 1
     while (ic < n_span) {
       const uint32_t eidx = emin + ic;
+      const uint32_t rec_p = rec_c ^ (N_REC - 1u);
       __builtin_amdgcn_wave_barrier();
-      st_rec[wv][(l >> 3) * (STG_LINE_STRIDE / 4u) + (l & 7u)] = lc;
-      if (l < 4u) st_rec[wv][ENT_CP_OFF / 4u + ((l + 3u) & 3u)] = cq;
-      uint4 e0, e1, e2, e3;
-      e0.x = IMPG_RDL(cq.x, 0); e0.y = IMPG_RDL(cq.y, 0); e0.z = IMPG_RDL(cq.z, 0); e0.w = IMPG_RDL(cq.w, 0);
-      e1.x = IMPG_RDL(cq.x, 1); e1.y = IMPG_RDL(cq.y, 1); e1.z = IMPG_RDL(cq.z, 1); e1.w = IMPG_RDL(cq.w, 1);
-      e2.x = IMPG_RDL(cq.x, 2); e2.y = IMPG_RDL(cq.y, 2); e2.z = IMPG_RDL(cq.z, 2); e2.w = IMPG_RDL(cq.w, 2);
-      e3.x = IMPG_RDL(cq.x, 3); e3.y = IMPG_RDL(cq.y, 3); e3.z = IMPG_RDL(cq.z, 3); e3.w = IMPG_RDL(cq.w, 3);
+      st_rec[rec_c][(l >> 3) * (STG_LINE_STRIDE / 4u) + (l & 7u)] = lc;
+      if (l < 4u) st_rec[rec_c][ENT_CP_OFF / 4u + ((l + 3u) & 3u)] = cq;
+      const uint32_t e_ts = IMPG_RDL(cq.x, 0), e_te = IMPG_RDL(cq.y, 0), e_w6 = IMPG_RDL(cq.z, 1);
       ic = in;
       cq = nq;
       lc = zero4;
+      uint32_t next_class = 4u;
       if (ic < n_span) {
         lc = fetch_record(cq);
+        next_class = entry_class(IMPG_RDL(cq.z, 1));
         in = take();
         nq = fetch_entry(in);
       }
       uint32_t cnt = 0;
-      const int32_t e_end = TRANSITIVE ? ((int32_t)e0.x < (int32_t)e0.y ? (int32_t)e0.y : (-2147483647 - 1)) : (int32_t)e0.y;
+      const int32_t e_end = TRANSITIVE ? ((int32_t)e_ts < (int32_t)e_te ? (int32_t)e_te : (-2147483647 - 1)) : (int32_t)e_te;
 #pragma unroll
       for (uint32_t q = 0; q < ENT_RANGES / 64u; q++) {
         const uint32_t r = q * 64u + l;
         bool hit = false;
-        if (r < nr) {
+        {
           const uint4 w = st_win[r];
           const uint32_t d = eidx - w.x;
           if (w.y - (w.x & ~3u) <= 64u) hit = d < 64u && (((d < 32u ? w.z >> d : w.w >> (d - 32u)) & 1u) != 0u);
@@ -2048,16 +2104,28 @@
       }
       asm volatile("s_waitcnt lgkmcnt(0)" ::: "memory");
       __builtin_amdgcn_wave_barrier();
-      const uint32_t *rec = reinterpret_cast<const uint32_t *>(&st_rec[wv][0]);
-      const int orient = (e1.z & OP_LEN_MASK) > INLINE_TILES * TILE_OPS ? -1 : !(e1.z & EF_REVERSED) ? 0 : (e1.z & EF_STRAND) ? 2 : 1;
+      const uint32_t cls = entry_class(e_w6);
       uint32_t tid = 0;
       if (ordered && cnt) tid = wl.se[r0 + (uint32_t)__builtin_amdgcn_readfirstlane((int)st_list[wv][0])].target_id;
+      const bool carry_on = CARRY && carry && cls < 3u && next_class == cls;
+      if (CARRY && wl.tail_joins && pend && cnt && l == 0) atomicAdd(wl.tail_joins, 1u);
+      uint32_t left = 0u, left_p = 0u;
 #pragma unroll 1
-      for (uint32_t k0 = 0; k0 < cnt; k0 += 64u) {
-        const bool live = k0 + l < cnt;
-        const uint32_t r = live ? (uint32_t)st_list[wv][k0 + l] : 0u;
+      for (int32_t k0 = -(int32_t)pend; k0 < (int32_t)cnt; k0 += 64) {
+        if (CARRY && carry_on && k0 >= 0 && cnt - (uint32_t)k0 < 64u) {
+          left = cnt - (uint32_t)k0;
+          left_p = run + (uint32_t)k0;
+          if (l < left) *tail_at(rec_c, l) = st_list[wv][(uint32_t)k0 + l];
+          break;
+        }
+        const int32_t k = k0 + (int32_t)l;
+        const bool tail = CARRY && k < 0;
+        const bool live = k < (int32_t)cnt;
+        uint32_t r = 0u;
+        if (tail) r = (uint32_t)*tail_at(rec_p, l);
+        else if (live) r = (uint32_t)st_list[wv][k];
         const int2 se = st_se[r];
-        uint32_t p = run + k0 + l;
+        uint32_t p = tail ? pend_p + l : run + (uint32_t)k;
         if (!compact) {
           const uint4 w = st_win[r];
           const uint32_t d = eidx - w.x;
@@ -2069,11 +2137,15 @@
           if (live) p = st_dest[r] + (uint32_t)wl.ord.vpos[p];
         } else if (qs) tid = r0 + r;
         else if (live && wl.range_out) wl.range_out[p] = wl.range_places ? r0 + r : wl.perm[r0 + r];
-        if (orient == 0) project_entry_chunk<TRANSITIVE, 0, MODE, OUT>(v, e0, e1, e2, e3, eidx, live, se.x, se.y, p, rec, h, accepted, err_flag, n_ok PHASE_PASS, min_identity, wl.ord, tid);
-        else if (orient == 1) project_entry_chunk<TRANSITIVE, 1, MODE, OUT>(v, e0, e1, e2, e3, eidx, live, se.x, se.y, p, rec, h, accepted, err_flag, n_ok PHASE_PASS, min_identity, wl.ord, tid);
-        else if (orient == 2) project_entry_chunk<TRANSITIVE, 2, MODE, OUT>(v, e0, e1, e2, e3, eidx, live, se.x, se.y, p, rec, h, accepted, err_flag, n_ok PHASE_PASS, min_identity, wl.ord, tid);
-        else project_entry_chunk<TRANSITIVE, -1, MODE, OUT>(v, e0, e1, e2, e3, eidx, live, se.x, se.y, p, rec, h, accepted, err_flag, n_ok PHASE_PASS, min_identity, wl.ord, tid);
+        const uint32_t *rec = reinterpret_cast<const uint32_t *>(st_work) + (tail ? rec_p : rec_c) * ENT_REC_STRIDE;
+        if (cls == 0u) project_entry_chunk<TRANSITIVE, 0, MODE, OUT>(v, eidx, live, se.x, se.y, p, rec, h, accepted, err_flag, n_ok PHASE_PASS, min_identity, wl.ord, tid);
+        else if (cls == 1u) project_entry_chunk<TRANSITIVE, 1, MODE, OUT>(v, eidx, live, se.x, se.y, p, rec, h, accepted, err_flag, n_ok PHASE_PASS, min_identity, wl.ord, tid);
+        else if (cls == 2u) project_entry_chunk<TRANSITIVE, 2, MODE, OUT>(v, eidx, live, se.x, se.y, p, rec, h, accepted, err_flag, n_ok PHASE_PASS, min_identity, wl.ord, tid);
+        else project_entry_chunk<TRANSITIVE, -1, MODE, OUT>(v, eidx, live, se.x, se.y, p, rec, h, accepted, err_flag, n_ok PHASE_PASS, min_identity, wl.ord, tid);
       }
+      pend = left;
+      pend_p = left_p;
+      rec_c = rec_p;
     }
 #undef IMPG_RDL
 #ifdef IMPG_PHASE_CLOCKS
@@ -2087,7 +2159,7 @@
     }
 #endif
   }
-  if (!sparse) {
+  if (WIDE_LISTED && !sparse) {
     const SliceArrays no_sl{nullptr, nullptr, nullptr, nullptr};
     const uint32_t nw = st_nwide;
 #pragma unroll 1
diff --git a/impg_amd/csrc/kernels.hpp b/impg_amd/csrc/kernels.hpp
--- a/impg_amd/csrc/kernels.hpp
+++ b/impg_amd/csrc/kernels.hpp
@@ -84,6 +84,8 @@
   uint32_t range_places;
   uint32_t *slice_work, *slice_alloc;
   uint32_t slice_cap;
+  uint32_t tail_carry;
+  uint32_t *tail_joins;
   OrderedOut ord;
 };
 bool project_is_staged(const DeviceIndexView &v, uint64_t n_pairs, bool plain);
```

Result: slower. 68.81 billion (-3.4%).
